# incredible-vision/show-and-tell

Measured on AMD Instinct MI355X. Metric: images/sec (train step), higher is better.
Workload: dtype bf16

## Files before the change

include/sat_hip.h:

```cpp
#ifndef SAT_HIP_H
#define SAT_HIP_H
#include <stdint.h>

#ifdef __cplusplus
extern "C" {
#endif

#define SAT_ABI_VERSION 18

#define SAT_OK 0
#define SAT_ERR_ARG 1001
#define SAT_ERR_WORKSPACE 1002
#define SAT_ERR_UNSUPPORTED 1003

#define SAT_F32 0
#define SAT_BF16 1

typedef void* sat_stream_t;

int sat_version(void);
const char* sat_error_string(int code);

int sat_gemm_f32(int amode, int bmode, const float* A, int64_t lda, const float* B, int64_t ldb,
                 float* C, int64_t ldc, const float* bias, const float* bias2,
                 int M, int N, int K, sat_stream_t stream);

enum {
    SAT_OP_IMAGE_PREP = 1,
    SAT_OP_CONV = 2,
    SAT_OP_BN_FINALIZE = 3,
    SAT_OP_BN_RELU = 4,
    SAT_OP_BN_ADD_RELU = 5,
    SAT_OP_BN_RELU_MAXPOOL = 6,
    SAT_OP_AVGPOOL = 7,
    SAT_OP_MAXPOOL3S2 = 10,
    SAT_OP_AVGPOOL3 = 11,
    SAT_OP_MAXPOOL2 = 9,
    SAT_OP_BN_EVAL_BATCH = 8,
    SAT_OP_GRAM = 12,
    SAT_OP_GRAM_COV = 13,
    SAT_OP_GEMM_BF16_NT = 14,
    SAT_OP_BN_FROM_GRAM = 15
};

typedef struct sat_bn_eval_item {
    const float* gamma;
    const float* beta;
    const float* running_mean;
    const float* running_var;
    float* scale_out;
    float* shift_out;
    int32_t C;
    int32_t reserved;
} sat_bn_eval_item;

typedef struct sat_bn_running_item {
    float* running_mean;
    float* running_var;
    const float* batch_mean;
    const float* batch_var;
    int32_t C;
    int32_t reserved;
} sat_bn_running_item;

typedef struct sat_op {
    int32_t kind;
    int32_t dtype;
    const void* in0;
    const void* in1;
    void* out;
    const void* w;
    const float* scale0;
    const float* shift0;
    const float* scale1;
    const float* shift1;
    float* stat_partial;
    const float* gamma;
    const float* beta;
    float* running_mean;
    float* running_var;
    float* scale_out;
    float* shift_out;
    int32_t N, Hin, Win, Cin, Hout, Wout, Cout, KH, KW, stride, pad;
    int32_t training;
    int32_t tiles_m;
    int64_t sN, sH, sW;
    int64_t count;
    float momentum, eps;
    int32_t variant;
    int32_t flags;
    void* stat_acc;
    void* stat_acc1;
    const float* gamma1;
    const float* beta1;
    float* running_mean1;
    float* running_var1;
    const void* w_packed;
    int32_t reserved1[2];
    int32_t pad_w;
    int32_t groups;
    int64_t ldc;
    void* out1;
} sat_op;
#define SAT_CONV_PADW 2
#define SAT_CONV_IN_RESIDUAL 8
#define SAT_CONV_GROUP_TABLE 4
int sat_gram_rows_per_slab(int64_t M, int P);
int sat_gram_slabs(int64_t M, int P);
int64_t sat_gram_slab_floats(int64_t M, int P);
int sat_run_ops(const sat_op* ops , int n_ops, sat_stream_t stream);
int sat_bn_running_apply(const sat_bn_running_item* items , int n_items, float momentum, sat_stream_t stream);
int sat_counter_add(int64_t* counters , int n, int64_t value, sat_stream_t stream);
int sat_run_ops_parity(const sat_op* ops , int n_ops, int parity, sat_stream_t stream);
typedef struct sat_graph sat_graph;
int sat_graph_create(const sat_op* ops , int n_ops, int parity, sat_graph** graph_out);
int sat_graph_launch(sat_graph* graph, sat_stream_t stream);
int sat_graph_destroy(sat_graph* graph);
int sat_conv_bn_relu_fwd(const sat_op* conv, const sat_op* finalize, const sat_op* bnrelu, sat_stream_t stream);
int sat_conv_tiles_m(int64_t M);
int sat_conv_autotune(sat_op* ops , int n_ops, int reps, float* scratch, int64_t scratch_bytes,
                      sat_stream_t stream);
int sat_conv_autotune_topk(sat_op* ops , int n_ops, int reps, float* scratch, int64_t scratch_bytes,
                           sat_stream_t stream, int topk, int32_t* cand );
int sat_conv_variant_signature(int variant);
int sat_conv_variant_family(int variant);
int sat_conv_num_variants(void);
int sat_conv_default_variant(const sat_op* op , int want_sig);
int sat_conv_resolved_variant(const sat_op* op );
int sat_conv_pack_weights(const void* w, void* packed, int Cout, int Cin, int taps, sat_stream_t stream);
int sat_run_ops_timed(const sat_op* ops , int n_ops, int parity, sat_stream_t stream, float* op_us );

int sat_fc_bn1d_fwd(const float* pooled , const float* w_fc , const float* b_fc ,
                    const float* gamma, const float* beta, float* running_mean, float* running_var,
                    float momentum, float eps, int training, int B, int F, int E,
                    float* feats , float* xhat , float* rstd ,
                    float* workspace, int64_t ws_bytes, sat_stream_t stream);
int64_t sat_fc_bn1d_ws_bytes(int B, int F, int E);
int sat_fc_bn1d_bwd(const float* dy , const float* pooled, const float* xhat, const float* rstd,
                    const float* gamma, int B, int F, int E,
                    float* dw_fc , float* db_fc, float* dgamma, float* dbeta,
                    float* workspace , int64_t ws_bytes, sat_stream_t stream);

int sat_embed_concat_fwd(const float* features , const float* embed ,
                         const int64_t* captions , int64_t cap_stride,
                         const int32_t* prefix , int T, int N , int B, int E, int V,
                         float* X , sat_stream_t stream);
int sat_embed_concat_bwd(const float* dX , const int64_t* captions, int64_t cap_stride,
                         const int32_t* prefix , int T, int N, int B, int E, int V,
                         float* d_embed , float* d_features , sat_stream_t stream);

int sat_validate_ids(const int64_t* ids, int64_t row_stride, int rows, int cols, int64_t lo, int64_t hi,
                     int32_t* status, sat_stream_t stream);

int sat_pack_targets(const int64_t* captions , int64_t cap_stride, const int32_t* prefix ,
                     int T, int N, int64_t* targets , sat_stream_t stream);

int sat_lstm_fwd(const float* X , const float* w_ih , const float* w_hh ,
                 const float* b_ih, const float* b_hh, const int32_t* batch_sizes , int T,
                 int In, int H, float* GA, float* CS, float* HS, float* HP, float* c_state,
                 void* workspace, int64_t ws_bytes, sat_stream_t stream);
int64_t sat_lstm_fwd_ws_bytes(int B, int H);
int64_t sat_lstm_fwd_status_offset(int B, int H);
int sat_lstm_persist_enable(int on);
int64_t sat_lstm_bwd_ws_bytes(int B, int H);
int64_t sat_lstm_bwd_ws_bytes_full(int N, int B, int In, int H);
int64_t sat_lstm_bwd_ws_bytes_max(int n_max, int B, int In, int H);
int sat_lstm_ws_release(void* workspace);
int64_t sat_lstm_bwd_status_offset(int N, int B, int In, int H);
int sat_lstm_bwd(const float* dHS , const float* X, const float* w_ih, const float* w_hh,
                 const float* GA, const float* CS, const float* HP,
                 const int32_t* batch_sizes , int T, int In, int H,
                 float* DG , float* dw_ih, float* dw_hh, float* db_ih, float* db_hh,
                 float* dX , float* workspace, int64_t ws_bytes, sat_stream_t stream);

int64_t sat_lstm_mixed_ws_bytes(int N , int In, int H);
int sat_lstm_fwd_bf16(const float* X, const float* w_ih, const float* w_hh, const float* b_ih, const float* b_hh,
                      const int32_t* batch_sizes , int T, int In, int H, float* GA, float* CS, float* HS, float* HP,
                      float* c_state, void* workspace, int64_t ws_bytes, void* mixed_ws, int64_t mixed_bytes, sat_stream_t stream);
int sat_lstm_bwd_bf16(const float* dHS, const float* X, const float* w_ih, const float* w_hh, const float* GA, const float* CS,
                      const float* HP, const int32_t* batch_sizes , int T, int In, int H, float* DG, float* dw_ih,
                      float* dw_hh, float* db_ih, float* db_hh, float* dX, float* workspace, int64_t ws_bytes, void* mixed_ws,
                      int64_t mixed_bytes, sat_stream_t stream);

int sat_vocab_logits_fwd(const float* Hs , const float* w , const float* b ,
                         int N, int H, int V, float* logits , int64_t ldl, sat_stream_t stream);
int sat_ce_rows(float* logits , int64_t ldl, const int64_t* targets , int N, int V, float inv_denom,
                int write_grad, float* row_loss , float* loss_out , sat_stream_t stream);
int64_t sat_vocab_bf16_ws_bytes(int N, int H, int V);
int sat_vocab_ce_fwd_bf16(const float* Hs , const float* w , const float* b , const int64_t* targets ,
                          int N, int H, int V, float inv_denom, float* logits , int64_t ldl, float* row_loss ,
                          float* loss_out , void* workspace , int64_t ws_bytes, sat_stream_t stream);
int sat_vocab_ce_bwd_bf16(int N, int H, int V, float* dw , float* db , float* dHs , void* workspace,
                          int64_t ws_bytes, sat_stream_t stream);
int sat_gemm_bf16_nt(const void* A, int64_t lda, const void* B, int64_t ldb, float* C, int64_t ldc, const float* bias,
                     int M, int N, int K, int ksplit, int64_t slab_stride, sat_stream_t stream);
int sat_transpose_f32_bf16(const float* in, int64_t ldi, int R, int C, void* out, int64_t ldo, sat_stream_t stream);
int sat_vocab_ce_fwd(const float* Hs , const float* w , const float* b , const int64_t* targets ,
                     int N, int H, int V, float inv_denom, float* logits , int64_t ldl,
                     float* row_loss , float* loss_out , sat_stream_t stream);
int sat_vocab_ce_bwd(const float* dlogits , int64_t ldl, const float* Hs, const float* w, int N, int H, int V,
                     float* dw, float* db, float* dHs, float* workspace, int64_t ws_bytes, sat_stream_t stream);
int64_t sat_vocab_ce_bwd_ws_bytes(int N, int H, int V);
int64_t sat_gemm_f32x3_packed_bytes(int N, int K);
int sat_gemm_f32x3_pack(const float* W, int N, int K, void* packed, sat_stream_t stream);
int sat_gemm_f32x3(const float* A, int64_t lda, const void* packed, const float* bias, float* C, int64_t ldc, int M, int N, int K,
                   sat_stream_t stream);

int sat_gemm_f32_splitk(int amode, int bmode, const float* A, int64_t lda, const float* B, int64_t ldb,
                        float* C, int64_t ldc, const float* bias, const float* bias2, int M, int N, int K,
                        int ksplit, int64_t slab_stride, sat_stream_t stream);
int sat_sum_slabs_f32(const float* in, int nslab, int64_t slab_stride, int64_t n, float* out, sat_stream_t stream);
int sat_skinny_gemm_f32(const float* A, int64_t lda, const float* W, int64_t ldw, int w_kmajor, int M, int N, int K,
                        const float* bias, float* out, int64_t ldo, float* workspace, int64_t ws_bytes, sat_stream_t stream);
int64_t sat_skinny_gemm_ws_bytes(int M, int N, int K);
int sat_skinny_gemm2_f32(const float* A, int64_t lda, const float* W, int64_t ldw, int K, const float* A2, int64_t lda2,
                         const float* W2, int64_t ldw2, int K2, int w_kmajor, int M, int N, const float* bias, float* out,
                         int64_t ldo, float* workspace, int64_t ws_bytes, sat_stream_t stream);
int sat_vocab_argmax(const float* h , const float* w, const float* b, int B, int H, int V,
                     int64_t* ids, int64_t ids_stride, float* workspace, int64_t ws_bytes, sat_stream_t stream);
int64_t sat_vocab_argmax_ws_bytes(int B, int V);
int sat_lstm_step(const float* x, const float* h_in, float* c, const float* w_ih, const float* w_hh,
                  const float* b_ih, const float* b_hh, int B, int In, int H, float* h_out, sat_stream_t stream);
int sat_embed_rows(const float* embed, const int64_t* ids, int64_t ids_stride, int B, int E, int V,
                   float* out, sat_stream_t stream);

int sat_attention_fwd(const float* ctx_enc, const float* feats, const float* proj, int64_t ld_proj, const float* w_att,
                      int rows, int P, int C, float* alpha, float* context, int64_t ld_ctx, float* workspace, int64_t ws_bytes,
                      sat_stream_t stream);
int64_t sat_attention_ws_bytes(int rows, int P);
int sat_attention_bwd(const float* ctx_enc, const float* feats, const float* proj, int64_t ld_proj, const float* w_att,
                      const float* alpha, const float* d_ctx, int64_t ld_dctx,
                      const float* d_ctx2 ,
                      int64_t ld_dctx2, int rows, int P, int C,
                      float* d_ctx_enc, float* d_proj, float* d_watt_part, float* d_feats ,
                      float* workspace, int64_t ws_bytes, sat_stream_t stream);
int64_t sat_attention_coverage_ws_bytes(int B, int P);
int sat_attention_coverage(const float* alpha , const int32_t* prefix , int T, int B, int P, float coef,
                           float* cov , float* grad , float* penalty , float* workspace,
                           int64_t ws_bytes, sat_stream_t stream);
int sat_attention_bwd_ex(const float* ctx_enc, const float* feats, const float* proj, int64_t ld_proj, const float* w_att,
                         const float* alpha, const float* d_ctx, int64_t ld_dctx, const float* d_ctx2, int64_t ld_dctx2,
                         const float* d_alpha_extra , int64_t ld_extra,
                         const float* d_alpha_scale , int rows, int P, int C,
                         float* d_ctx_enc, float* d_proj, float* d_watt_part, float* d_feats ,
                         float* workspace, int64_t ws_bytes, sat_stream_t stream);
int sat_lstmcell_fwd(const float* x , const float* h_in , float* c , const float* w_ih,
                     const float* w_hh, const float* b_ih, const float* b_hh, int B, int In, int H, float* h_out,
                     float* gates , float* c_tape , sat_stream_t stream);
int sat_rows_copy(const float* in, int64_t ldi, const int64_t* idx, int64_t idx_stride, int64_t nrows_in, int rows, int cols,
                  float* out, int64_t ldo, sat_stream_t stream);
int sat_rows_sum(const float* in, int64_t ld, int rows, int cols, float* out, int accumulate, sat_stream_t stream);
int sat_rows_add(const float* a, int64_t lda, const float* b, int64_t ldb, int rows, int cols, float* out, int64_t ldo,
                 sat_stream_t stream);
int sat_pack_tokens(const int64_t* captions, int64_t cap_stride, const int32_t* prefix , int T, int N, int col0,
                    int64_t* out, sat_stream_t stream);
int sat_scatter_rows_add(const float* rows , const int64_t* ids , int N, int E, int V, float* table,
                         sat_stream_t stream);
int sat_lstmcell_bwd_point(const float* dh_out , const float* dh_carry , int n_carry,
                           const float* gates , const float* c , const float* c_prev ,
                           float* dc_state , float* DG , int n, int H, sat_stream_t stream);

int sat_pad_nhwc_f32(const float* in, const float* relu_mask_of , int N, int H, int W, int C, int pad, float* out,
                     sat_stream_t stream);
int sat_maxpool2_bwd_f32(const float* x, const float* dy, int N, int Hin, int Win, int C, float* dx, sat_stream_t stream);
int sat_bcast_add_f32(const float* v, int B, int P, int C, float scale, float* out, sat_stream_t stream);

int sat_collate_captions(const int64_t* flat, const int64_t* offsets , const int32_t* order , int B, int Tmax,
                         int64_t* out , sat_stream_t stream);
int sat_gather_rows_f32(const float* in, const int32_t* order, int rows, int64_t cols, float* out, sat_stream_t stream);

int sat_image_augment_u8(const uint8_t* src, int Bsrc, int Hs, int Ws, const int32_t* params, const int32_t* order,
                         int B, int Hc, int Wc, const float mean[3] , const float std[3] ,
                         float* out, sat_stream_t stream);

int sat_beam_step(const float* logits , int64_t ldl, const float* scores_in ,
                  const int64_t* last_tokens , int64_t end_id, int B, int K, int V,
                  int32_t* parent , int64_t* token , float* scores_out ,
                  void* workspace, int64_t ws_bytes, sat_stream_t stream);
int64_t sat_beam_step_ws_bytes(int B, int K);
int sat_beam_gather_rows(const float* src, const int32_t* parent, int B, int K, int width, float* dst,
                         sat_stream_t stream);
int sat_beam_backtrack(const int32_t* parents, const int64_t* tokens, int T, int B, int K, int64_t* ids,
                       sat_stream_t stream);
int sat_beam_backtrack_rows(const int32_t* parents, const float* rows, int T, int B, int K, int cols, float* out,
                            sat_stream_t stream);
int64_t sat_beam_decode_ws_bytes(int B, int K, int E, int H, int V, int num_layers, int steps);
int sat_beam_decode(const float* features , const float* embed , const float* const* lstm_w , int num_layers,
                    const float* lin_w , const float* lin_b, int B, int K, int E, int H, int V, int steps, int64_t end_id,
                    int64_t* ids, float* scores, void* workspace, int64_t ws_bytes, sat_stream_t stream);
int sat_greedy_decode(const float* features, const float* embed, const float* const* lstm_w , int num_layers,
                      const float* lin_w, const float* lin_b, int B, int E, int H, int V, int steps, float* h, float* c, float* h_tmp,
                      float* x_tmp, int64_t* ids, int64_t ids_stride, float* workspace, int64_t ws_bytes, sat_stream_t stream);
typedef struct {
    const int64_t* suppress_ids;
    int n_suppress;
    int min_length;
    int no_repeat_ngram;
    int block_repeat;
    float length_penalty;
} sat_beam_constraints;
int sat_beam_step_ex(const float* logits , int64_t ldl, const float* scores_in ,
                     const int64_t* last_tokens , int64_t end_id, int B, int K, int V,
                     const sat_beam_constraints* c , const int32_t* parents, const int64_t* tokens, int i, int T,
                     int32_t* parent , int64_t* token , float* scores_out ,
                     void* workspace, int64_t ws_bytes, sat_stream_t stream);
int64_t sat_beam_step_ex_ws_bytes(int B, int K, int V, int T);
int sat_beam_rerank(const int64_t* ids, const float* scores, int B, int K, int T, int64_t end_id, float length_penalty,
                    int64_t* ids_out, float* scores_out, float* norm_out, int32_t* order_out, sat_stream_t stream);
int64_t sat_beam_decode_ex_ws_bytes(int B, int K, int E, int H, int V, int num_layers, int steps);
int sat_beam_decode_ex(const float* features , const float* embed , const float* const* lstm_w , int num_layers,
                       const float* lin_w , const float* lin_b, int B, int K, int E, int H, int V, int steps, int64_t end_id,
                       const sat_beam_constraints* c , int64_t* ids, float* scores, float* norm_scores,
                       int32_t* order, void* workspace, int64_t ws_bytes, sat_stream_t stream);
int sat_beam_step_groups(const float* logits , int64_t ldl, const float* scores_in ,
                         const int64_t* last_tokens , int64_t end_id, int B, int K, int V,
                         const sat_beam_constraints* c , const int32_t* parents, const int64_t* tokens, int i, int T,
                         int num_groups, float diversity_penalty, int32_t* parent , int64_t* token ,
                         float* scores_out , void* workspace, int64_t ws_bytes, sat_stream_t stream);
int64_t sat_beam_step_groups_ws_bytes(int B, int K, int V, int T);
int64_t sat_beam_decode_groups_ws_bytes(int B, int K, int E, int H, int V, int num_layers, int steps);
int sat_beam_decode_groups(const float* features , const float* embed , const float* const* lstm_w ,
                           int num_layers, const float* lin_w , const float* lin_b, int B, int K, int E, int H, int V, int steps,
                           int64_t end_id, const sat_beam_constraints* c , int num_groups, float diversity_penalty,
                           int64_t* ids, float* scores, float* norm_scores, int32_t* order, void* workspace, int64_t ws_bytes,
                           sat_stream_t stream);
int64_t sat_ss_decoder_fwd_ws_bytes(int B, int V);
int sat_vocab_sample(const float* h , const float* lin_w, const float* lin_b, int B, int H, int V, float* logits, int64_t ldl,
                     float ss_prob, uint64_t seed, int t, int rank, const int64_t* teacher, int64_t teacher_stride, int64_t* ids,
                     int64_t ids_stride, const float* embed, int E, float* x, float* workspace, int64_t ws_bytes, sat_stream_t stream);
int sat_ss_decoder_fwd(const float* features , const float* embed , const int64_t* captions, int64_t cap_stride,
                       const int32_t* batch_sizes , const int32_t* prefix , int T, int E, int V,
                       const float* const* lstm_w , int num_layers, int H, const float* lin_w, const float* lin_b,
                       float* const* tapes , float* X, float* logits, int64_t ldl, float ss_prob, uint64_t seed, int rank,
                       int64_t* used, int64_t used_stride, float* workspace, int64_t ws_bytes, sat_stream_t stream);
int sat_dropout_f32(const float* x, int64_t ldx, float* y, int64_t ldy, int rows, int cols, float p, uint64_t seed, int rank, int site,
                    sat_stream_t stream);
enum {
    SAT_SSA_WEIGHT_HH_W, SAT_SSA_WEIGHT_HH_B, SAT_SSA_WEIGHT_ATT, SAT_SSA_EMBEDDING, SAT_SSA_CELL_W_IH, SAT_SSA_CELL_W_HH,
    SAT_SSA_CELL_B_IH, SAT_SSA_CELL_B_HH, SAT_SSA_C2O_W, SAT_SSA_C2O_B, SAT_SSA_H2O_W, SAT_SSA_H2O_B, SAT_SSA_CLS_W, SAT_SSA_CLS_B,
    SAT_SSA_NUM_WEIGHTS
};
enum { SAT_SSA_PROJ, SAT_SSA_ALPHA, SAT_SSA_X, SAT_SSA_GATES, SAT_SSA_CS, SAT_SSA_HS, SAT_SSA_ZIN, SAT_SSA_Z, SAT_SSA_NUM_TAPES };
int64_t sat_ss_attend_fwd_ws_bytes(int B, int P, int C, int E, int H, int V);
int sat_ss_attend_fwd(const float* feats, const float* ctx_enc, const float* h0, const float* c0, const int64_t* captions,
                      int64_t cap_stride, const int32_t* batch_sizes , const int32_t* prefix , int T, int P,
                      int C, int E, int H, int V, const float* const* w , float* const* tapes , int64_t* toks,
                      float* logits, int64_t ldl, float ss_prob, uint64_t seed, int rank, int64_t* used, int64_t used_stride,
                      float* workspace, int64_t ws_bytes, sat_stream_t stream);
int sat_kept_tokens(const int64_t* ids, int64_t stride, int B, int T, int64_t end_id, int32_t* kept ,
                    sat_stream_t stream);
int64_t sat_sample_filtered_ws_bytes(int R, int V);
int sat_sample_filtered(const float* logits , int64_t ldl, int R, int V, float temperature, int top_k, float top_p,
                        uint64_t seed, int t, int rank, int64_t* ids, int64_t ids_stride, float* logp ,
                        int32_t* kept , void* workspace, int64_t ws_bytes, sat_stream_t stream);
int64_t sat_sample_decode_ws_bytes(int B, int E, int H, int V, int num_layers);
int sat_sample_decode(const float* features, const float* embed, const float* const* lstm_w , int num_layers,
                      const float* lin_w, const float* lin_b, int B, int E, int H, int V, int steps, float temperature, int top_k,
                      float top_p, uint64_t seed, int rank, float* h, float* c, float* h_tmp, float* x_tmp, int64_t* ids,
                      int64_t ids_stride, float* logp, int32_t* kept, float* logits_out, int64_t ldl, void* workspace,
                      int64_t ws_bytes, sat_stream_t stream);

typedef struct sat_cider_corpus {
    const uint64_t* table_keys;
    const int32_t* table_nodes;
    const int32_t* df;
    const int32_t* ref_tokens;
    const int32_t* ref_offsets;
    const int32_t* image_offsets;
    const double* ref_norm;
    int64_t capacity, n_tokens;
    int32_t n_nodes, n_refs, n_images;
    int32_t max_ref_tokens;
} sat_cider_corpus;
int sat_cider_table_insert(const uint64_t* keys, int n_keys, uint64_t* table_keys, int32_t* table_nodes, int64_t capacity,
                           int32_t* status, sat_stream_t stream);
int sat_cider_ref_stats(const sat_cider_corpus* corpus , double* ref_norm, sat_stream_t stream);
int sat_cider_score(const sat_cider_corpus* corpus , const int64_t* ids, int64_t stride, int B, int T,
                    const int32_t* kept , int64_t end_id, const int32_t* image_index , double sigma,
                    double* scores , double* mean , sat_stream_t stream);

typedef struct sat_ref_corpus {
    const int32_t* ref_tokens;
    const int32_t* ref_offsets;
    const int32_t* image_offsets;
    int64_t n_tokens;
    int32_t n_refs, n_images;
    int32_t max_ref_tokens;
    int32_t reserved;
} sat_ref_corpus;
int sat_bleu_comps(const sat_ref_corpus* corpus , const int64_t* ids, int64_t stride, int B, int T,
                   const int32_t* kept , int64_t end_id, const int32_t* image_index ,
                   int64_t* comps , double* sentence , double* mean ,
                   int64_t* totals , sat_stream_t stream);
int sat_bleu_finalize(const int64_t* totals , double* bleu , sat_stream_t stream);
int sat_rouge_l_score(const sat_ref_corpus* corpus , const int64_t* ids, int64_t stride, int B, int T,
                      const int32_t* kept , int64_t end_id, const int32_t* image_index , double beta,
                      double* scores , double* mean , sat_stream_t stream);

int64_t sat_rollout_decoder_fwd_ws_bytes(int B, int V);
int sat_rollout_decoder_fwd(const float* features , const float* embed , int B, int steps, int E, int V,
                            const float* const* lstm_w , int num_layers, int H, const float* lin_w, const float* lin_b,
                            float* const* tapes , float* X, float* logits, int64_t ldl, uint64_t seed, int rank, int64_t* ids,
                            int64_t ids_stride, float* workspace, int64_t ws_bytes, sat_stream_t stream);
int sat_scst_weights(const int64_t* ids, int64_t stride, int B, int T, int64_t end_id, const double* reward ,
                     const double* baseline , const double* denom , float* w ,
                     int32_t* len , double* m_out , sat_stream_t stream);
int sat_ce_rows_weighted(float* logits , int64_t ldl, const int64_t* ids, int64_t ids_stride, int B, int N, int V,
                         const float* w , int write_grad, float* row_loss , float* loss_out ,
                         sat_stream_t stream);
int64_t sat_rollout_attend_fwd_ws_bytes(int B, int P, int C, int E, int H, int V);
int sat_rollout_attend_fwd(const float* feats, const float* ctx_enc, const float* h0, const float* c0,
                           const int32_t* prefix , int B, int steps, int P, int C, int E, int H, int V,
                           const float* const* w , float* const* tapes , int64_t* toks, float* logits, int64_t ldl,
                           int greedy, int64_t start_id, uint64_t seed, int rank, int64_t* ids, int64_t ids_stride, int64_t* fed,
                           int64_t fed_stride, float* workspace, int64_t ws_bytes, sat_stream_t stream);

int sat_clamp_adam_step(float* p, float* g, float* m, float* v, int64_t n, float lr, float beta1,
                        float beta2, float eps, float clip, int step, sat_stream_t stream);
int sat_clamp_adam_step_guarded(float* p, float* g, float* m, float* v, int64_t n, float lr, float beta1,
                                float beta2, float eps, float clip, int step, const float* skip_if_nonzero,
                                sat_stream_t stream);
int sat_step_fault_flag(const void* const* status_words, int n_words, float* sticky, float* slot, sat_stream_t stream);

int sat_colsum_f32(const float* x, int64_t ld, int rows, int cols, float* out, sat_stream_t stream);
int sat_cast_f32_bf16(const float* in, void* out, int64_t n, sat_stream_t stream);
int sat_cast_bf16_f32(const void* in, float* out, int64_t n, sat_stream_t stream);

#ifdef __cplusplus
}
#endif
#endif
```

show-and-tell_amd/_lib.py:

```python
import ctypes as C
import os

_HERE = os.path.dirname(os.path.abspath(__file__))
LIB_PATH = os.environ.get("SAT_LIB") or os.path.join(_HERE, "libsat_hip.so")

ABI_VERSION = 18
SAT_F32, SAT_BF16 = 0, 1
OP_IMAGE_PREP, OP_CONV, OP_BN_FINALIZE, OP_BN_RELU, OP_BN_ADD_RELU, OP_BN_RELU_MAXPOOL, OP_AVGPOOL = 1, 2, 3, 4, 5, 6, 7

OP_BN_EVAL_BATCH = 8
OP_MAXPOOL2 = 9
OP_MAXPOOL3S2, OP_AVGPOOL3 = 10, 11
OP_GRAM, OP_GRAM_COV, OP_GEMM_BF16_NT, OP_BN_FROM_GRAM = 12, 13, 14, 15
CONV_PADW = 2
CONV_GROUP_TABLE = 4
CONV_IN_RESIDUAL = 8

_vp, _i, _i64, _f = C.c_void_p, C.c_int, C.c_int64, C.c_float


class SatBnEvalItem(C.Structure):
    _fields_ = [("gamma", _vp), ("beta", _vp), ("running_mean", _vp), ("running_var", _vp),
                ("scale_out", _vp), ("shift_out", _vp), ("C", C.c_int32), ("reserved", C.c_int32)]


class SatBnRunningItem(C.Structure):
    _fields_ = [("running_mean", _vp), ("running_var", _vp), ("batch_mean", _vp), ("batch_var", _vp),
                ("C", C.c_int32), ("reserved", C.c_int32)]


class SatCiderCorpus(C.Structure):
    _fields_ = [("table_keys", _vp), ("table_nodes", _vp), ("df", _vp), ("ref_tokens", _vp), ("ref_offsets", _vp),
                ("image_offsets", _vp), ("ref_norm", _vp), ("capacity", C.c_int64), ("n_tokens", C.c_int64),
                ("n_nodes", C.c_int32), ("n_refs", C.c_int32), ("n_images", C.c_int32), ("max_ref_tokens", C.c_int32)]


class SatRefCorpus(C.Structure):
    _fields_ = [("ref_tokens", _vp), ("ref_offsets", _vp), ("image_offsets", _vp), ("n_tokens", C.c_int64),
                ("n_refs", C.c_int32), ("n_images", C.c_int32), ("max_ref_tokens", C.c_int32), ("reserved", C.c_int32)]


class SatBeamConstraints(C.Structure):
    _fields_ = [("suppress_ids", _vp), ("n_suppress", C.c_int), ("min_length", C.c_int), ("no_repeat_ngram", C.c_int),
                ("block_repeat", C.c_int), ("length_penalty", C.c_float)]


class SatOp(C.Structure):
    __slots__ = ()
    _fields_ = [
        ("kind", C.c_int32), ("dtype", C.c_int32),
        ("in0", _vp), ("in1", _vp), ("out", _vp), ("w", _vp),
        ("scale0", _vp), ("shift0", _vp), ("scale1", _vp), ("shift1", _vp),
        ("stat_partial", _vp), ("gamma", _vp), ("beta", _vp),
        ("running_mean", _vp), ("running_var", _vp), ("scale_out", _vp), ("shift_out", _vp),
        ("N", C.c_int32), ("Hin", C.c_int32), ("Win", C.c_int32), ("Cin", C.c_int32),
        ("Hout", C.c_int32), ("Wout", C.c_int32), ("Cout", C.c_int32),
        ("KH", C.c_int32), ("KW", C.c_int32), ("stride", C.c_int32), ("pad", C.c_int32),
        ("training", C.c_int32), ("tiles_m", C.c_int32),
        ("sN", C.c_int64), ("sH", C.c_int64), ("sW", C.c_int64), ("count", C.c_int64),
        ("momentum", C.c_float), ("eps", C.c_float),
        ("variant", C.c_int32), ("flags", C.c_int32),
        ("stat_acc", _vp), ("stat_acc1", _vp), ("gamma1", _vp), ("beta1", _vp),
        ("running_mean1", _vp), ("running_var1", _vp), ("w_packed", _vp),
        ("reserved1", C.c_int32 * 2),
        ("pad_w", C.c_int32), ("groups", C.c_int32), ("ldc", C.c_int64), ("out1", C.c_void_p),
    ]


def op(kind, dtype, **fields):
    return SatOp(kind=kind, dtype=dtype, **{k: v.data_ptr() if hasattr(v, "data_ptr") else v for k, v in fields.items()})


SIGNATURES = {
    "sat_version": (_i, []),
    "sat_error_string": (C.c_char_p, [_i]),
    "sat_gemm_f32": (_i, [_i, _i, _vp, _i64, _vp, _i64, _vp, _i64, _vp, _vp, _i, _i, _i, _vp]),
    "sat_run_ops": (_i, [C.POINTER(SatOp), _i, _vp]),
    "sat_run_ops_parity": (_i, [C.POINTER(SatOp), _i, _i, _vp]),
    "sat_graph_create": (_i, [C.POINTER(SatOp), _i, _i, C.POINTER(_vp)]),
    "sat_graph_launch": (_i, [_vp, _vp]),
    "sat_graph_destroy": (_i, [_vp]),
    "sat_conv_bn_relu_fwd": (_i, [C.POINTER(SatOp), C.POINTER(SatOp), C.POINTER(SatOp), _vp]),
    "sat_conv_tiles_m": (_i, [_i64]),
    "sat_counter_add": (_i, [_vp, _i, _i64, _vp]),
    "sat_conv_variant_signature": (_i, [_i]),
    "sat_conv_variant_family": (_i, [_i]),
    "sat_gram_rows_per_slab": (_i, [_i64, _i]),
    "sat_gram_slabs": (_i, [_i64, _i]),
    "sat_gram_slab_floats": (_i64, [_i64, _i]),
    "sat_conv_num_variants": (_i, []),
    "sat_conv_default_variant": (_i, [C.POINTER(SatOp), _i]),
    "sat_conv_resolved_variant": (_i, [C.POINTER(SatOp)]),
    "sat_conv_pack_weights": (_i, [_vp, _vp, _i, _i, _i, _vp]),
    "sat_conv_autotune": (_i, [C.POINTER(SatOp), _i, _i, _vp, _i64, _vp]),
    "sat_conv_autotune_topk": (_i, [C.POINTER(SatOp), _i, _i, _vp, _i64, _vp, _i, C.POINTER(C.c_int32)]),
    "sat_run_ops_timed": (_i, [C.POINTER(SatOp), _i, _i, _vp, C.POINTER(C.c_float)]),
    "sat_validate_ids": (_i, [_vp, _i64, _i, _i, _i64, _i64, _vp, _vp]),
    "sat_fc_bn1d_fwd": (_i, [_vp, _vp, _vp, _vp, _vp, _vp, _vp, _f, _f, _i, _i, _i, _i, _vp, _vp, _vp, _vp, _i64, _vp]),
    "sat_fc_bn1d_ws_bytes": (_i64, [_i, _i, _i]),
    "sat_fc_bn1d_bwd": (_i, [_vp, _vp, _vp, _vp, _vp, _i, _i, _i, _vp, _vp, _vp, _vp, _vp, _i64, _vp]),
    "sat_embed_concat_fwd": (_i, [_vp, _vp, _vp, _i64, _vp, _i, _i, _i, _i, _i, _vp, _vp]),
    "sat_embed_concat_bwd": (_i, [_vp, _vp, _i64, _vp, _i, _i, _i, _i, _i, _vp, _vp, _vp]),
    "sat_pack_targets": (_i, [_vp, _i64, _vp, _i, _i, _vp, _vp]),
    "sat_lstm_fwd": (_i, [_vp, _vp, _vp, _vp, _vp, C.POINTER(C.c_int32), _i, _i, _i, _vp, _vp, _vp, _vp, _vp, _vp, _i64, _vp]),
    "sat_lstm_mixed_ws_bytes": (_i64, [_i, _i, _i]),
    "sat_lstm_fwd_bf16": (_i, [_vp, _vp, _vp, _vp, _vp, C.POINTER(C.c_int32), _i, _i, _i, _vp, _vp, _vp, _vp, _vp, _vp, _i64, _vp, _i64, _vp]),
    "sat_lstm_bwd_bf16": (_i, [_vp, _vp, _vp, _vp, _vp, _vp, _vp, C.POINTER(C.c_int32), _i, _i, _i,
                               _vp, _vp, _vp, _vp, _vp, _vp, _vp, _i64, _vp, _i64, _vp]),
    "sat_lstm_fwd_ws_bytes": (_i64, [_i, _i]),
    "sat_lstm_fwd_status_offset": (_i64, [_i, _i]),
    "sat_lstm_persist_enable": (_i, [_i]),
    "sat_lstm_bwd_ws_bytes": (_i64, [_i, _i]),
    "sat_lstm_bwd_ws_bytes_full": (_i64, [_i, _i, _i, _i]),
    "sat_lstm_bwd_status_offset": (_i64, [_i, _i, _i, _i]),
    "sat_lstm_bwd_ws_bytes_max": (_i64, [_i, _i, _i, _i]),
    "sat_lstm_ws_release": (_i, [_vp]),
    "sat_lstm_bwd": (_i, [_vp, _vp, _vp, _vp, _vp, _vp, _vp, C.POINTER(C.c_int32), _i, _i, _i,
                          _vp, _vp, _vp, _vp, _vp, _vp, _vp, _i64, _vp]),
    "sat_vocab_logits_fwd": (_i, [_vp, _vp, _vp, _i, _i, _i, _vp, _i64, _vp]),
    "sat_ce_rows": (_i, [_vp, _i64, _vp, _i, _i, _f, _i, _vp, _vp, _vp]),
    "sat_vocab_ce_fwd": (_i, [_vp, _vp, _vp, _vp, _i, _i, _i, _f, _vp, _i64, _vp, _vp, _vp]),
    "sat_vocab_bf16_ws_bytes": (_i64, [_i, _i, _i]),
    "sat_vocab_ce_fwd_bf16": (_i, [_vp, _vp, _vp, _vp, _i, _i, _i, _f, _vp, _i64, _vp, _vp, _vp, _i64, _vp]),
    "sat_vocab_ce_bwd_bf16": (_i, [_i, _i, _i, _vp, _vp, _vp, _vp, _i64, _vp]),
    "sat_gemm_bf16_nt": (_i, [_vp, _i64, _vp, _i64, _vp, _i64, _vp, _i, _i, _i, _i, _i64, _vp]),
    "sat_transpose_f32_bf16": (_i, [_vp, _i64, _i, _i, _vp, _i64, _vp]),
    "sat_vocab_ce_bwd": (_i, [_vp, _i64, _vp, _vp, _i, _i, _i, _vp, _vp, _vp, _vp, _i64, _vp]),
    "sat_vocab_ce_bwd_ws_bytes": (_i64, [_i, _i, _i]),
    "sat_gemm_f32_splitk": (_i, [_i, _i, _vp, _i64, _vp, _i64, _vp, _i64, _vp, _vp, _i, _i, _i, _i, _i64, _vp]),
    "sat_gemm_f32x3_packed_bytes": (_i64, [_i, _i]),
    "sat_gemm_f32x3_pack": (_i, [_vp, _i, _i, _vp, _vp]),
    "sat_gemm_f32x3": (_i, [_vp, _i64, _vp, _vp, _vp, _i64, _i, _i, _i, _vp]),
    "sat_sum_slabs_f32": (_i, [_vp, _i, _i64, _i64, _vp, _vp]),
    "sat_skinny_gemm_f32": (_i, [_vp, _i64, _vp, _i64, _i, _i, _i, _i, _vp, _vp, _i64, _vp, _i64, _vp]),
    "sat_skinny_gemm_ws_bytes": (_i64, [_i, _i, _i]),
    "sat_skinny_gemm2_f32": (_i, [_vp, _i64, _vp, _i64, _i, _vp, _i64, _vp, _i64, _i, _i, _i, _i, _vp, _vp, _i64, _vp, _i64, _vp]),
    "sat_vocab_argmax": (_i, [_vp, _vp, _vp, _i, _i, _i, _vp, _i64, _vp, _i64, _vp]),
    "sat_vocab_argmax_ws_bytes": (_i64, [_i, _i]),
    "sat_lstm_step": (_i, [_vp, _vp, _vp, _vp, _vp, _vp, _vp, _i, _i, _i, _vp, _vp]),
    "sat_embed_rows": (_i, [_vp, _vp, _i64, _i, _i, _i, _vp, _vp]),
    "sat_attention_fwd": (_i, [_vp, _vp, _vp, _i64, _vp, _i, _i, _i, _vp, _vp, _i64, _vp, _i64, _vp]),
    "sat_attention_bwd": (_i, [_vp, _vp, _vp, _i64, _vp, _vp, _vp, _i64, _vp, _i64, _i, _i, _i, _vp, _vp, _vp, _vp, _vp, _i64, _vp]),
    "sat_attention_ws_bytes": (_i64, [_i, _i]),
    "sat_attention_coverage_ws_bytes": (_i64, [_i, _i]),
    "sat_attention_coverage": (_i, [_vp, _vp, _i, _i, _i, _f, _vp, _vp, _vp, _vp, _i64, _vp]),
    "sat_attention_bwd_ex": (_i, [_vp, _vp, _vp, _i64, _vp, _vp, _vp, _i64, _vp, _i64, _vp, _i64, _vp, _i, _i, _i, _vp, _vp, _vp, _vp,
                                  _vp, _i64, _vp]),
    "sat_bn_running_apply": (_i, [_vp, _i, _f, _vp]),
    "sat_pad_nhwc_f32": (_i, [_vp, _vp, _i, _i, _i, _i, _i, _vp, _vp]),
    "sat_maxpool2_bwd_f32": (_i, [_vp, _vp, _i, _i, _i, _i, _vp, _vp]),
    "sat_bcast_add_f32": (_i, [_vp, _i, _i, _i, _f, _vp, _vp]),
    "sat_lstmcell_fwd": (_i, [_vp, _vp, _vp, _vp, _vp, _vp, _vp, _i, _i, _i, _vp, _vp, _vp, _vp]),
    "sat_rows_copy": (_i, [_vp, _i64, _vp, _i64, _i64, _i, _i, _vp, _i64, _vp]),
    "sat_rows_sum": (_i, [_vp, _i64, _i, _i, _vp, _i, _vp]),
    "sat_rows_add": (_i, [_vp, _i64, _vp, _i64, _i, _i, _vp, _i64, _vp]),
    "sat_pack_tokens": (_i, [_vp, _i64, _vp, _i, _i, _i, _vp, _vp]),
    "sat_scatter_rows_add": (_i, [_vp, _vp, _i, _i, _i, _vp, _vp]),
    "sat_lstmcell_bwd_point": (_i, [_vp, _vp, _i, _vp, _vp, _vp, _vp, _vp, _i, _i, _vp]),
    "sat_collate_captions": (_i, [_vp, _vp, _vp, _i, _i, _vp, _vp]),
    "sat_gather_rows_f32": (_i, [_vp, _vp, _i, _i64, _vp, _vp]),
    "sat_image_augment_u8": (_i, [_vp, _i, _i, _i, _vp, _vp, _i, _i, _i, C.POINTER(_f), C.POINTER(_f), _vp, _vp]),
    "sat_beam_step": (_i, [_vp, _i64, _vp, _vp, _i64, _i, _i, _i, _vp, _vp, _vp, _vp, _i64, _vp]),
    "sat_beam_step_ws_bytes": (_i64, [_i, _i]),
    "sat_beam_gather_rows": (_i, [_vp, _vp, _i, _i, _i, _vp, _vp]),
    "sat_beam_backtrack": (_i, [_vp, _vp, _i, _i, _i, _vp, _vp]),
    "sat_beam_backtrack_rows": (_i, [_vp, _vp, _i, _i, _i, _i, _vp, _vp]),
    "sat_kept_tokens": (_i, [_vp, _i64, _i, _i, _i64, _vp, _vp]),
    "sat_beam_decode_ws_bytes": (_i64, [_i, _i, _i, _i, _i, _i, _i]),
    "sat_beam_decode": (_i, [_vp, _vp, C.POINTER(_vp), _i, _vp, _vp, _i, _i, _i, _i, _i, _i, _i64, _vp, _vp, _vp, _i64, _vp]),
    "sat_beam_step_ex": (_i, [_vp, _i64, _vp, _vp, _i64, _i, _i, _i, C.POINTER(SatBeamConstraints), _vp, _vp, _i, _i, _vp, _vp, _vp, _vp,
                              _i64, _vp]),
    "sat_beam_step_ex_ws_bytes": (_i64, [_i, _i, _i, _i]),
    "sat_beam_rerank": (_i, [_vp, _vp, _i, _i, _i, _i64, _f, _vp, _vp, _vp, _vp, _vp]),
    "sat_beam_decode_ex_ws_bytes": (_i64, [_i, _i, _i, _i, _i, _i, _i]),
    "sat_beam_decode_ex": (_i, [_vp, _vp, C.POINTER(_vp), _i, _vp, _vp, _i, _i, _i, _i, _i, _i, _i64, C.POINTER(SatBeamConstraints),
                                _vp, _vp, _vp, _vp, _vp, _i64, _vp]),
    "sat_beam_step_groups": (_i, [_vp, _i64, _vp, _vp, _i64, _i, _i, _i, C.POINTER(SatBeamConstraints), _vp, _vp, _i, _i, _i, _f, _vp, _vp,
                                  _vp, _vp, _i64, _vp]),
    "sat_beam_step_groups_ws_bytes": (_i64, [_i, _i, _i, _i]),
    "sat_beam_decode_groups_ws_bytes": (_i64, [_i, _i, _i, _i, _i, _i, _i]),
    "sat_beam_decode_groups": (_i, [_vp, _vp, C.POINTER(_vp), _i, _vp, _vp, _i, _i, _i, _i, _i, _i, _i64, C.POINTER(SatBeamConstraints),
                                    _i, _f, _vp, _vp, _vp, _vp, _vp, _i64, _vp]),
    "sat_greedy_decode": (_i, [_vp, _vp, C.POINTER(_vp), _i, _vp, _vp, _i, _i, _i, _i, _i, _vp, _vp, _vp, _vp, _vp, _i64, _vp, _i64, _vp]),
    "sat_ss_decoder_fwd_ws_bytes": (_i64, [_i, _i]),
    "sat_vocab_sample": (_i, [_vp, _vp, _vp, _i, _i, _i, _vp, _i64, _f, C.c_uint64, _i, _i, _vp, _i64, _vp, _i64, _vp, _i, _vp,
                              _vp, _i64, _vp]),
    "sat_ss_decoder_fwd": (_i, [_vp, _vp, _vp, _i64, C.POINTER(C.c_int32), _vp, _i, _i, _i, C.POINTER(_vp), _i, _i, _vp, _vp,
                                C.POINTER(_vp), _vp, _vp, _i64, _f, C.c_uint64, _i, _vp, _i64, _vp, _i64, _vp]),
    "sat_ss_attend_fwd_ws_bytes": (_i64, [_i, _i, _i, _i, _i, _i]),
    "sat_ss_attend_fwd": (_i, [_vp, _vp, _vp, _vp, _vp, _i64, C.POINTER(C.c_int32), _vp, _i, _i, _i, _i, _i, _i, C.POINTER(_vp),
                               C.POINTER(_vp), _vp, _vp, _i64, _f, C.c_uint64, _i, _vp, _i64, _vp, _i64, _vp]),
    "sat_cider_table_insert": (_i, [_vp, _i, _vp, _vp, _i64, _vp, _vp]),
    "sat_cider_ref_stats": (_i, [C.POINTER(SatCiderCorpus), _vp, _vp]),
    "sat_cider_score": (_i, [C.POINTER(SatCiderCorpus), _vp, _i64, _i, _i, _vp, _i64, _vp, C.c_double, _vp, _vp, _vp]),
    "sat_bleu_comps": (_i, [C.POINTER(SatRefCorpus), _vp, _i64, _i, _i, _vp, _i64, _vp, _vp, _vp, _vp, _vp, _vp]),
    "sat_bleu_finalize": (_i, [_vp, _vp, _vp]),
    "sat_rouge_l_score": (_i, [C.POINTER(SatRefCorpus), _vp, _i64, _i, _i, _vp, _i64, _vp, C.c_double, _vp, _vp, _vp]),
    "sat_rollout_decoder_fwd_ws_bytes": (_i64, [_i, _i]),
    "sat_rollout_decoder_fwd": (_i, [_vp, _vp, _i, _i, _i, _i, C.POINTER(_vp), _i, _i, _vp, _vp, C.POINTER(_vp), _vp, _vp, _i64,
                                     C.c_uint64, _i, _vp, _i64, _vp, _i64, _vp]),
    "sat_scst_weights": (_i, [_vp, _i64, _i, _i, _i64, _vp, _vp, _vp, _vp, _vp, _vp, _vp]),
    "sat_ce_rows_weighted": (_i, [_vp, _i64, _vp, _i64, _i, _i, _i, _vp, _i, _vp, _vp, _vp]),
    "sat_rollout_attend_fwd_ws_bytes": (_i64, [_i, _i, _i, _i, _i, _i]),
    "sat_rollout_attend_fwd": (_i, [_vp, _vp, _vp, _vp, _vp, _i, _i, _i, _i, _i, _i, _i, C.POINTER(_vp), C.POINTER(_vp), _vp, _vp, _i64,
                                    _i, _i64, C.c_uint64, _i, _vp, _i64, _vp, _i64, _vp, _i64, _vp]),
    "sat_sample_filtered_ws_bytes": (_i64, [_i, _i]),
    "sat_sample_filtered": (_i, [_vp, _i64, _i, _i, _f, _i, _f, C.c_uint64, _i, _i, _vp, _i64, _vp, _vp, _vp, _i64, _vp]),
    "sat_sample_decode_ws_bytes": (_i64, [_i, _i, _i, _i, _i]),
    "sat_sample_decode": (_i, [_vp, _vp, C.POINTER(_vp), _i, _vp, _vp, _i, _i, _i, _i, _i, _f, _i, _f, C.c_uint64, _i, _vp, _vp, _vp,
                               _vp, _vp, _i64, _vp, _vp, _vp, _i64, _vp, _i64, _vp]),
    "sat_dropout_f32": (_i, [_vp, _i64, _vp, _i64, _i, _i, _f, C.c_uint64, _i, _i, _vp]),
    "sat_clamp_adam_step": (_i, [_vp, _vp, _vp, _vp, _i64, _f, _f, _f, _f, _f, _i, _vp]),
    "sat_clamp_adam_step_guarded": (_i, [_vp, _vp, _vp, _vp, _i64, _f, _f, _f, _f, _f, _i, _vp, _vp]),
    "sat_step_fault_flag": (_i, [C.POINTER(_vp), _i, _vp, _vp, _vp]),
    "sat_colsum_f32": (_i, [_vp, _i64, _i, _i, _vp, _vp]),
    "sat_cast_f32_bf16": (_i, [_vp, _vp, _i64, _vp]),
    "sat_cast_bf16_f32": (_i, [_vp, _vp, _i64, _vp]),
}

ADDED_WITHIN_ABI = ("sat_conv_resolved_variant", "sat_image_augment_u8", "sat_attention_coverage_ws_bytes", "sat_attention_coverage",
                    "sat_attention_bwd_ex", "sat_beam_backtrack_rows", "sat_cider_table_insert", "sat_cider_ref_stats", "sat_cider_score",
                    "sat_rollout_decoder_fwd_ws_bytes", "sat_rollout_decoder_fwd", "sat_scst_weights", "sat_ce_rows_weighted",
                    "sat_rollout_attend_fwd_ws_bytes", "sat_rollout_attend_fwd", "sat_bleu_comps", "sat_bleu_finalize",
                    "sat_rouge_l_score", "sat_sample_filtered_ws_bytes", "sat_sample_filtered", "sat_sample_decode_ws_bytes",
                    "sat_sample_decode", "sat_dropout_f32", "sat_beam_step_ex", "sat_beam_step_ex_ws_bytes", "sat_beam_rerank",
                    "sat_beam_decode_ex_ws_bytes", "sat_beam_decode_ex", "sat_beam_step_groups", "sat_beam_step_groups_ws_bytes",
                    "sat_beam_decode_groups_ws_bytes", "sat_beam_decode_groups")

_lib = None


def open_library(path):
    if not os.path.exists(path):
        raise RuntimeError(
            "show-and-tell_amd: %s is missing -- build it with `python -c 'import __graft_entry__ as g; g.build()'` "
            "(hipcc --offload-arch=gfx950).  There is no CPU fallback." % path)
    lib = C.CDLL(path)
    for name, (res, args) in SIGNATURES.items():
        if name in ADDED_WITHIN_ABI and not hasattr(lib, name):
            continue
        fn = getattr(lib, name)
        fn.restype = res
        fn.argtypes = args
    if lib.sat_version() != ABI_VERSION:
        raise RuntimeError("%s: ABI version mismatch" % path)
    return lib


def load():
    global _lib
    if _lib is None:
        _lib = open_library(LIB_PATH)
    return _lib


def check(rc, what=""):
    if rc != 0:
        msg = load().sat_error_string(rc)
        raise RuntimeError("libsat_hip %s failed: [%d] %s" % (what, rc, msg.decode() if msg else "?"))


def ptr(t):
    return t if t is None or isinstance(t, int) else t.data_ptr()


def rows(t, row0=0):
    return t.data_ptr() + row0 * t.shape[1] * 4


def stream():
    import torch
    return torch.cuda.current_stream().cuda_stream


def pad4(n):
    return (n + 3) // 4 * 4


def logits_buffer(N, V, device):
    import torch
    return torch.zeros(N, pad4(V), device=device) if V % 4 else torch.empty(N, V, device=device)


def pad_rows4(d):
    import torch
    V = d.shape[1]
    if V % 4 == 0:
        return d.contiguous()
    out = torch.zeros(d.shape[0], pad4(V), device=d.device)
    out[:, :V] = d
    return out


def workspace256(nbytes, device):
    import torch
    ws = torch.empty(nbytes + 256, dtype=torch.uint8, device=device)
    return ws, ws.data_ptr() + (-ws.data_ptr()) % 256


def require_gpu(t, name="tensor"):
    if not t.is_cuda:
        raise RuntimeError("show-and-tell_amd: %s must live on the MI355X (got a %s tensor); the HIP path has no CPU fallback"
                           % (name, t.device))


def counter_add(t, value=1):
    check(load().sat_counter_add(t.data_ptr(), t.numel(), value, stream()), "sat_counter_add")


_SKINNY_WS = {}
_SKINNY_ROWS = int(os.environ.get("SAT_SKINNY_ROWS", "128"))


def gemm(lib, amode, bmode, A, lda, B, ldb, Cout, ldc, M, N, K, bias=None, bias2=None):
    if amode == 0 and M <= _SKINNY_ROWS and bias2 is None and ldc == N and K % 4 == 0 and lda % 4 == 0 and (bmode == 1 or ldb % 4 == 0):
        import torch
        need = lib.sat_skinny_gemm_ws_bytes(M, N, K)
        dev = torch.cuda.current_device()
        ws = _SKINNY_WS.get(dev)
        if ws is None or ws.numel() * 4 < need:
            ws = _SKINNY_WS[dev] = torch.empty(max(need // 4, 1 << 20), dtype=torch.float32, device="cuda")
        check(lib.sat_skinny_gemm_f32(ptr(A), lda, ptr(B), ldb, bmode, M, N, K, ptr(bias), ptr(Cout), ldc,
                                      ws.data_ptr(), ws.numel() * 4, stream()), "sat_skinny_gemm_f32")
        return
    check(lib.sat_gemm_f32(amode, bmode, ptr(A), lda, ptr(B), ldb, ptr(Cout), ldc, ptr(bias), ptr(bias2), M, N, K, stream()),
          "sat_gemm_f32")
```

show-and-tell_amd/csrc/sat_elementwise.hip:

```cpp
#include "sat_bn_stats.h"
#include <stdlib.h>

namespace {

constexpr int EW_BLOCK = 256;
inline int ew_grid(long n_items) {
    long cap;
    cap = 768;
    long b = (n_items + EW_BLOCK - 1) / EW_BLOCK;
    return (int)(b < 1 ? 1 : (b > cap ? cap : b));
}

template <typename T> struct Vec;
template <> struct Vec<float> { static constexpr int N = 4; };
template <> struct Vec<bf16_t> { static constexpr int N = 8; };

template <typename T> __device__ __forceinline__ void load_chunk(const T* p, float (&v)[Vec<T>::N]);
template <> __device__ __forceinline__ void load_chunk<float>(const float* p, float (&v)[4]) {
    const f32x4 x = *(const f32x4*)p;
    v[0] = x[0]; v[1] = x[1]; v[2] = x[2]; v[3] = x[3];
}
template <> __device__ __forceinline__ void load_chunk<bf16_t>(const bf16_t* p, float (&v)[8]) {
    const bf16x8 x = *(const bf16x8*)p;
#pragma unroll
// ... 445 lines not shown
    __syncthreads();
    const int v = tok[row];
    if (v < 0) {
        for (int e = threadIdx.x; e < E; e += blockDim.x) d_features[(long)row * E + e] = dX[(long)row * E + e];
        return;
    }
    int dup = 0;
    for (int i = threadIdx.x; i < row; i += blockDim.x) dup |= (tok[i] == v);
    if (__syncthreads_or(dup)) return;
    __shared__ unsigned match_bits[1280];
    const int nwords = (Nrows + 31) >> 5;
    const bool fits = nwords <= 1280;
    int any = 0;
    if (fits) {
        for (int w = threadIdx.x; w < nwords; w += blockDim.x) {
            unsigned bits = 0u;
            const int base = w << 5;
            for (int b = 0; b < 32; ++b) {
                const int i = base + b;
                if (i > row && i < Nrows && tok[i] == v) bits |= 1u << b;
            }
            match_bits[w] = bits;
            any |= (bits != 0u);
        }
    }
    any = __syncthreads_or(any);
    for (int e = threadIdx.x; e < E; e += blockDim.x) {
        float acc = dX[(long)row * E + e];
        if (!fits) {
            for (int i = row + 1; i < Nrows; ++i)
                if (tok[i] == v) acc += dX[(long)i * E + e];
        } else if (any) {
            for (int w = row >> 5; w < nwords; ++w) {
                unsigned bits = match_bits[w];
                while (bits) {
                    const int b = __ffs(bits) - 1;
                    bits &= bits - 1;
                    acc += dX[(long)((w << 5) + b) * E + e];
                }
            }
        }
        d_embed[(long)v * E + e] = acc;
    }
}

__device__ __forceinline__ float block_reduce(float v, bool is_max, float* sh) {
    v = is_max ? wave_max(v) : wave_sum(v);
    const int w = threadIdx.x >> 6;
    __syncthreads();
    if ((threadIdx.x & 63) == 0) sh[w] = v;
    __syncthreads();
    float r = sh[0];
    for (int i = 1; i < (int)(blockDim.x >> 6); ++i) r = is_max ? fmaxf(r, sh[i]) : r + sh[i];
    return r;
}

template <bool WEIGHTED>
__global__ __launch_bounds__(256) void ce_rows_kernel(float* __restrict__ logits, long ldl, const int64_t* __restrict__ targets,
                                                      int V, float inv_denom, int write_grad, float* __restrict__ row_loss,
                                                      const float* __restrict__ w, long tstride, int B) {
    __shared__ float sh[4];
    const int row = blockIdx.x;
    float* x = logits + (long)row * ldl;
    if constexpr (WEIGHTED) inv_denom = w[row];
    const long tpos = WEIGHTED ? (long)(row % B) * tstride + row / B : (long)row;
    constexpr int RC = 12;
    const int nq = V >> 2;
    if ((ldl & 3) == 0 && nq <= RC * 256 && (((uintptr_t)logits) & 15) == 0) {
        const int tid = threadIdx.x;
        f32x4 rc[RC];
#pragma unroll
        for (int c = 0; c < RC; ++c)
            if (tid + c * 256 < nq) rc[c] = *(const f32x4*)(x + 4 * (tid + c * 256));
        const int tail = (nq << 2) + tid;
        const float xt = tail < V ? x[tail] : -INFINITY;
        float m = xt;
#pragma unroll
        for (int c = 0; c < RC; ++c)
            if (tid + c * 256 < nq) m = fmaxf(fmaxf(fmaxf(m, rc[c][0]), fmaxf(rc[c][1], rc[c][2])), rc[c][3]);
        m = block_reduce(m, true, sh);
        float s = 0.0f;
#pragma unroll
        for (int c = 0; c < RC; ++c)
            if (tid + c * 256 < nq) {
#pragma unroll
                for (int e = 0; e < 4; ++e) s += expf(rc[c][e] - m);
            }
        if (tail < V) s += expf(xt - m);
        s = block_reduce(s, false, sh);
        const float lse = m + logf(s);
        long tgt = targets[tpos];
        tgt = tgt < 0 ? 0 : (tgt >= V ? V - 1 : tgt);
        const int tq = (int)(tgt >> 2), te = (int)(tgt & 3);
#pragma unroll
        for (int c = 0; c < RC; ++c)
            if (tid + c * 256 == tq && tq < nq) row_loss[row] = lse - rc[c][te];
        if (tail == (int)tgt && tq >= nq) row_loss[row] = lse - xt;
        if (write_grad) {
#pragma unroll
            for (int c = 0; c < RC; ++c) {
                const int q = tid + c * 256;
                if (q < nq) {
                    f32x4 g;
#pragma unroll
                    for (int e = 0; e < 4; ++e)
                        g[e] = (expf(rc[c][e] - lse) - ((4 * q + e) == (int)tgt ? 1.0f : 0.0f)) * inv_denom;
                    if (WEIGHTED && inv_denom == 0.0f) g = (f32x4){0.0f, 0.0f, 0.0f, 0.0f};
                    *(f32x4*)(x + 4 * q) = g;
                }
            }
            if (tail < V) x[tail] = (WEIGHTED && inv_denom == 0.0f) ? 0.0f : (expf(xt - lse) - (tail == (int)tgt ? 1.0f : 0.0f)) * inv_denom;
        }
        return;
    }
    float m = -INFINITY;
    for (int i = threadIdx.x; i < V; i += 256) m = fmaxf(m, x[i]);
    m = block_reduce(m, true, sh);
    float s = 0.0f;
    for (int i = threadIdx.x; i < V; i += 256) s += expf(x[i] - m);
    s = block_reduce(s, false, sh);
    const float lse = m + logf(s);
    long tgt = targets[tpos];
    tgt = tgt < 0 ? 0 : (tgt >= V ? V - 1 : tgt);
    if (threadIdx.x == 0) row_loss[row] = lse - x[tgt];
    if (write_grad) {
        __syncthreads();
        for (int i = threadIdx.x; i < V; i += 256) {
            const float pr = expf(x[i] - lse);
            x[i] = (WEIGHTED && inv_denom == 0.0f) ? 0.0f : (pr - (i == (int)tgt ? 1.0f : 0.0f)) * inv_denom;
        }
    }
}

__global__ __launch_bounds__(256) void weighted_sum_kernel(const float* __restrict__ v, const float* __restrict__ w, int n, float* out) {
    __shared__ float sh[256];
    float s = 0.0f;
    for (int i = threadIdx.x; i < n; i += 256) {
        const float wi = w[i];
        if (wi != 0.0f) s += wi * v[i];
    }
    sh[threadIdx.x] = s;
    __syncthreads();
    for (int k = 128; k > 0; k >>= 1) {
        if ((int)threadIdx.x < k) sh[threadIdx.x] += sh[threadIdx.x + k];
        __syncthreads();
    }
    if (threadIdx.x == 0) out[0] = sh[0];
}

__global__ __launch_bounds__(256) void scst_weights_kernel(const int64_t* __restrict__ ids, long stride, int B, int T, int64_t end_id,
                                                           const double* __restrict__ reward, const double* __restrict__ baseline,
                                                           const double* __restrict__ denom, float* __restrict__ w,
                                                           int32_t* __restrict__ len, double* __restrict__ m_out) {
    __shared__ long long sh[256];
    const int tid = threadIdx.x;
    long long tot = 0;
    for (int b = tid; b < B; b += 256) {
        const int64_t* row = ids + (long)b * stride;
        int n = 0;
        while (n < T && row[n] != end_id) ++n;
        n = n + 1 < T ? n + 1 : T;
        len[b] = n;
        tot += n;
    }
    sh[tid] = tot;
    __syncthreads();
    for (int k = 128; k > 0; k >>= 1) {
        if (tid < k) sh[tid] += sh[tid + k];
        __syncthreads();
    }
    const double M = denom ? *denom : (double)sh[0];
    if (tid == 0) m_out[0] = M;
    for (int b = tid; b < B; b += 256) {
        const float wb = (float)((reward[b] - (baseline ? baseline[b] : 0.0)) / M);
        const int n = len[b];
        for (int t = 0; t < T; ++t) w[(long)t * B + b] = t < n ? wb : 0.0f;
    }
}

__global__ __launch_bounds__(256) void sum_scale_kernel(const float* __restrict__ v, int n, float scale, float* out) {
    __shared__ float sh[256];
    float s = 0.0f;
    for (int i = threadIdx.x; i < n; i += 256) s += v[i];
    sh[threadIdx.x] = s;
    __syncthreads();
    for (int k = 128; k > 0; k >>= 1) {
        if ((int)threadIdx.x < k) sh[threadIdx.x] += sh[threadIdx.x + k];
        __syncthreads();
    }
    if (threadIdx.x == 0) out[0] = sh[0] * scale;
}

__global__ __launch_bounds__(256) void colsum_kernel(const float* __restrict__ x, long ld, int rows, int cols,
                                                     float* __restrict__ out) {
    __shared__ float sh[8][32];
    const int cl = threadIdx.x & 31, rg = threadIdx.x >> 5;
    const int c = blockIdx.x * 32 + cl;
    float s = 0.0f;
    if (c < cols) {
        int r = rg;
        for (; r + 24 < rows; r += 32) {
            const float a0 = x[(long)r * ld + c], a1 = x[(long)(r + 8) * ld + c];
            const float a2 = x[(long)(r + 16) * ld + c], a3 = x[(long)(r + 24) * ld + c];
            s += a0; s += a1; s += a2; s += a3;
        }
        for (; r < rows; r += 8) s += x[(long)r * ld + c];
    }
    sh[rg][cl] = s;
    __syncthreads();
    if (rg == 0 && c < cols) {
        float t = 0.0f;
#pragma unroll
        for (int g = 0; g < 8; ++g) t += sh[g][cl];
        out[c] = t;
    }
}

__global__ void clamp_adam_kernel(float* __restrict__ p, float* __restrict__ g, float* __restrict__ m,
                                  float* __restrict__ v, long n, float beta1, float beta2, float eps, float clip,
                                  float step_size, float bc2_sqrt, const float* __restrict__ skip) {
    if (skip && *skip != 0.0f) return;
    const float w1 = 1.0f - beta1, w2 = 1.0f - beta2;
    const long n4 = n >> 2;
    for (long i = (long)blockIdx.x * blockDim.x + threadIdx.x; i < n4; i += (long)gridDim.x * blockDim.x) {
        f32x4 pp = ((f32x4*)p)[i], gg = ((f32x4*)g)[i], mm = ((f32x4*)m)[i], vv = ((f32x4*)v)[i];
#pragma unroll
        for (int k = 0; k < 4; ++k) {
            float gk = gg[k];
            if (clip > 0.0f) gk = fminf(fmaxf(gk, -clip), clip);
            gg[k] = gk;
            mm[k] = mm[k] + w1 * (gk - mm[k]);
            vv[k] = vv[k] * beta2 + (w2 * gk) * gk;
            const float denom = sqrtf(vv[k]) / bc2_sqrt + eps;
            pp[k] = pp[k] + (-step_size * mm[k]) / denom;
        }
        ((f32x4*)p)[i] = pp; ((f32x4*)g)[i] = gg; ((f32x4*)m)[i] = mm; ((f32x4*)v)[i] = vv;
    }
    const long base = n4 << 2;
    const long i = base + (long)blockIdx.x * blockDim.x + threadIdx.x;
    if (i < n) {
        float gk = g[i];
        if (clip > 0.0f) gk = fminf(fmaxf(gk, -clip), clip);
        g[i] = gk;
        const float mk = m[i] + w1 * (gk - m[i]);
        const float vk = v[i] * beta2 + (w2 * gk) * gk;
        m[i] = mk; v[i] = vk;
        p[i] = p[i] + (-step_size * mk) / (sqrtf(vk) / bc2_sqrt + eps);
    }
}

__global__ void cast_f32_bf16_kernel(const float* __restrict__ in, bf16_t* __restrict__ out, long n) {
    for (long i = (long)blockIdx.x * blockDim.x + threadIdx.x; i < n; i += (long)gridDim.x * blockDim.x)
        out[i] = (bf16_t)in[i];
}
__global__ void cast_bf16_f32_kernel(const bf16_t* __restrict__ in, float* __restrict__ out, long n) {
    for (long i = (long)blockIdx.x * blockDim.x + threadIdx.x; i < n; i += (long)gridDim.x * blockDim.x)
        out[i] = (float)in[i];
}

__global__ void lstm_bwd_point_kernel(const float* __restrict__ dHS, const float* __restrict__ dh_part, int nz,
                                      long slab_stride, int n_next, const float* __restrict__ GA,
                                      const float* __restrict__ CS, const float* __restrict__ CS_prev,
                                      float* __restrict__ dc_state, float* __restrict__ DG, int n, int H) {
    const long total = (long)n * H;
    for (long i = (long)blockIdx.x * blockDim.x + threadIdx.x; i < total; i += (long)gridDim.x * blockDim.x) {
        const int j = (int)(i % H);
        const int b = (int)(i / H);
        float dh = dHS[i];
        float dcn = 0.0f;
        if (b < n_next) {
            for (int z = 0; z < nz; ++z) dh += dh_part[(long)z * slab_stride + i];
            dcn = dc_state[i];
        }
        const float* ga = GA + (long)b * 4 * H;
        const float gi = ga[j], gf = ga[H + j], gg = ga[2 * H + j], go = ga[3 * H + j];
        const float tc = sat_tanh(CS[i]);
        const float c_prev = CS_prev ? CS_prev[i] : 0.0f;
        const float d_o = dh * tc;
        const float dc = dh * go * (1.0f - tc * tc) + dcn;
        float* dg = DG + (long)b * 4 * H;
        dg[j] = dc * gg * gi * (1.0f - gi);
        dg[H + j] = dc * c_prev * gf * (1.0f - gf);
        dg[2 * H + j] = dc * gi * (1.0f - gg * gg);
        dg[3 * H + j] = d_o * go * (1.0f - go);
        dc_state[i] = dc * gf;
    }
}

__global__ __launch_bounds__(256) void bn1d_fwd_kernel(const float* __restrict__ part, int nz, long slab_stride,
                                                       const float* __restrict__ b_fc, const float* __restrict__ gamma,
                                                       const float* __restrict__ beta, float* running_mean,
                                                       float* running_var, float momentum, float eps, int training,
                                                       int B, int E, float* __restrict__ zbuf, float* __restrict__ feats,
                                                       float* __restrict__ xhat, float* __restrict__ rstd_out) {
    __shared__ float sh[8][32];
    __shared__ float bc[2][32];
    const int cl = threadIdx.x & 31, rg = threadIdx.x >> 5;
    const int e = blockIdx.x * 32 + cl;
    const bool ok = e < E;
    float s = 0.0f;
    if (ok)
        for (int b = rg; b < B; b += 8) {
            float z = b_fc[e];
            for (int k = 0; k < nz; ++k) z += part[(long)k * slab_stride + (long)b * E + e];
            zbuf[(long)b * E + e] = z;
            s += z;
        }
    sh[rg][cl] = s;
    __syncthreads();
    if (rg == 0) {
        float t = 0.0f;
        for (int g = 0; g < 8; ++g) t += sh[g][cl];
        bc[0][cl] = t / (float)B;
    }
    __syncthreads();
    float mean = bc[0][cl];
    float q = 0.0f;
    if (ok)
        for (int b = rg; b < B; b += 8) {
            const float d = zbuf[(long)b * E + e] - mean;
            q += d * d;
        }
    __syncthreads();
    sh[rg][cl] = q;
    __syncthreads();
    if (rg == 0 && ok) {
        float t = 0.0f;
        for (int g = 0; g < 8; ++g) t += sh[g][cl];
        float var = t / (float)B;
        if (training) {
            const float unb = B > 1 ? t / (float)(B - 1) : var;
            running_mean[e] = (1.0f - momentum) * running_mean[e] + momentum * mean;
            running_var[e] = (1.0f - momentum) * running_var[e] + momentum * unb;
        } else {
            mean = running_mean[e];
            var = running_var[e];
        }
        const float rs = 1.0f / sqrtf(var + eps);
        bc[0][cl] = mean;
        bc[1][cl] = rs;
        rstd_out[e] = rs;
    }
    __syncthreads();
    if (ok) {
        const float mu = bc[0][cl], rs = bc[1][cl], ga = gamma[e], be = beta[e];
        for (int b = rg; b < B; b += 8) {
            const float xh = (zbuf[(long)b * E + e] - mu) * rs;
            xhat[(long)b * E + e] = xh;
            feats[(long)b * E + e] = xh * ga + be;
        }
    }
}

__global__ __launch_bounds__(256) void bn1d_bwd_kernel(const float* __restrict__ dy, const float* __restrict__ xhat,
                                                       const float* __restrict__ rstd, const float* __restrict__ gamma,
                                                       int B, int E, float* __restrict__ dz, float* __restrict__ dgamma,
                                                       float* __restrict__ dbeta, float* __restrict__ db_fc) {
    __shared__ float s1[8][32], s2[8][32];
    __shared__ float bc[2][32];
    const int cl = threadIdx.x & 31, rg = threadIdx.x >> 5;
    const int e = blockIdx.x * 32 + cl;
    const bool ok = e < E;
    float a = 0.0f, c = 0.0f;
    if (ok)
        for (int b = rg; b < B; b += 8) {
            const float d = dy[(long)b * E + e];
            a += d * xhat[(long)b * E + e];
            c += d;
        }
    s1[rg][cl] = a; s2[rg][cl] = c;
    __syncthreads();
    if (rg == 0) {
        float ta = 0.0f, tc = 0.0f;
        for (int g = 0; g < 8; ++g) { ta += s1[g][cl]; tc += s2[g][cl]; }
        bc[0][cl] = ta; bc[1][cl] = tc;
        if (ok) { dgamma[e] = ta; dbeta[e] = tc; }
    }
    __syncthreads();
    float zs = 0.0f;
    if (ok) {
        const float dga = bc[0][cl], dbe = bc[1][cl];
        const float k = gamma[e] * rstd[e] / (float)B;
        for (int b = rg; b < B; b += 8) {
            const float v = k * ((float)B * dy[(long)b * E + e] - dbe - xhat[(long)b * E + e] * dga);
            dz[(long)b * E + e] = v;
            zs += v;
        }
    }
    __syncthreads();
    s1[rg][cl] = zs;
    __syncthreads();
    if (rg == 0 && ok) {
        float t = 0.0f;
        for (int g = 0; g < 8; ++g) t += s1[g][cl];
        db_fc[e] = t;
    }
}

}

int sat_image_prep_launch(const sat_op* op, hipStream_t s) {
    if (!op->in0 || !op->out) return SAT_ERR_ARG;
    const long total = (long)op->N * op->Hin * op->Win;
    if (op->Cout != 0 && op->Cout != 4 && !(op->Cout == 8 && op->dtype == SAT_BF16)) return SAT_ERR_ARG;
    if (op->dtype == SAT_BF16 && op->Cout == 8)
        hipLaunchKernelGGL((image_prep_kernel<bf16_t, 8>), dim3(ew_grid(total)), dim3(EW_BLOCK), 0, s, (const float*)op->in0,
                           (bf16_t*)op->out, op->N, op->Hin, op->Win, op->Hout, op->Wout, op->pad);
    else if (op->dtype == SAT_BF16)
        hipLaunchKernelGGL(image_prep_kernel<bf16_t>, dim3(ew_grid(total)), dim3(EW_BLOCK), 0, s, (const float*)op->in0,
                           (bf16_t*)op->out, op->N, op->Hin, op->Win, op->Hout, op->Wout, op->pad);
    else
        hipLaunchKernelGGL(image_prep_kernel<float>, dim3(ew_grid(total)), dim3(EW_BLOCK), 0, s, (const float*)op->in0,
                           (float*)op->out, op->N, op->Hin, op->Win, op->Hout, op->Wout, op->pad);
    SAT_LAUNCH_CHECK();
    return SAT_OK;
}

extern "C" int sat_bn_running_apply(const sat_bn_running_item* items, int n_items, float momentum, sat_stream_t stream) {
    if (!items || n_items < 0 || !(momentum >= 0.0f && momentum <= 1.0f)) return SAT_ERR_ARG;
    if (n_items == 0) return SAT_OK;
    hipLaunchKernelGGL(bn_running_apply_kernel, dim3(n_items), dim3(256), 0, (hipStream_t)stream, items, momentum);
    SAT_LAUNCH_CHECK();
    return SAT_OK;
}

__global__ void counter_add_kernel(long long* p, int n, long long v) {
    const int i = blockIdx.x * blockDim.x + threadIdx.x;
    if (i < n) p[i] += v;
}
extern "C" int sat_counter_add(int64_t* counters, int n, int64_t value, sat_stream_t stream) {
    if (!counters || n < 0) return SAT_ERR_ARG;
    if (n == 0) return SAT_OK;
    hipLaunchKernelGGL(counter_add_kernel, dim3((n + 255) / 256), dim3(256), 0, (hipStream_t)stream, (long long*)counters, n, (long long)value);
    SAT_LAUNCH_CHECK();
    return SAT_OK;
}

int sat_bn_eval_batch_launch(const sat_op* op, hipStream_t s) {
    if (!op->in0 || op->count < 1 || op->count > 65535) return SAT_ERR_ARG;
    hipLaunchKernelGGL(bn_eval_batch_kernel, dim3((int)op->count), dim3(256), 0, s, (const sat_bn_eval_item*)op->in0, op->eps);
    SAT_LAUNCH_CHECK();
    return SAT_OK;
}

int sat_bn_finalize_launch(const sat_op* op, int parity, hipStream_t s) {
    if (op->stat_acc) {
        if (!op->stat_partial || op->tiles_m < 1 || op->Cout < 1) return SAT_ERR_ARG;
        long long* acc = (long long*)op->stat_acc + (long)parity * 2 * op->Cout;
        const int groups = op->groups > 1 ? op->groups : 1;
        hipLaunchKernelGGL(bn_slab_to_acc_kernel, dim3(sat_cdiv(op->Cout, 32), sat_cdiv(op->tiles_m, SLAB_TILES_PER_WG), groups),
                           dim3(1024), 0, s, op->stat_partial, op->tiles_m, op->Cout, acc);
        SAT_LAUNCH_CHECK();
        return SAT_OK;
    }
    if (op->groups > 1) return SAT_ERR_UNSUPPORTED;
    if (!op->gamma || !op->beta || !op->scale_out || !op->shift_out) return SAT_ERR_ARG;
    if (op->training && !op->stat_partial) return SAT_ERR_ARG;
    if (!op->training && (!op->running_mean || !op->running_var)) return SAT_ERR_ARG;
    hipLaunchKernelGGL(bn_finalize_kernel, dim3(sat_cdiv(op->Cout, 32)), dim3(1024), 0, s, op->stat_partial, op->tiles_m,
                       op->Cout, (double)op->count, op->gamma, op->beta, op->running_mean, op->running_var,
                       op->momentum, op->eps, op->training, op->scale_out, op->shift_out);
    SAT_LAUNCH_CHECK();
    return SAT_OK;
}

template <typename T>
static int bn_act_launch_t(const sat_op* op, bool add, int parity, hipStream_t s) {
    constexpr int V = Vec<T>::N;
    const int C = op->Cout;
    if (C % V) return SAT_ERR_ARG;
    const long n = (long)op->N * op->Hout * op->Wout * C;
    const long nch = n / V;
    BnSrc b0 = {}, b1 = {};
    b0.scale = op->scale0; b0.shift = op->shift0;
    b1.scale = op->scale1; b1.shift = op->shift1;
    int has_b1 = 0;
    size_t lds = 0;
    if (op->stat_acc) {
        if (!op->gamma || !op->beta || op->count < 1) return SAT_ERR_ARG;
        long long* base = (long long*)op->stat_acc;
        b0.acc = base + (long)parity * 2 * C;
        b0.acc_clear = base + (long)(1 - parity) * 2 * C;
        b0.gamma = op->gamma; b0.beta = op->beta; b0.running_mean = op->running_mean; b0.running_var = op->running_var;
        lds = (size_t)4 * C * sizeof(float);
    } else if (!op->scale0 || !op->shift0) {
        return SAT_ERR_ARG;
    }
    if (add) {
        if (op->stat_acc1) {
            if (!op->gamma1 || !op->beta1 || op->count < 1) return SAT_ERR_ARG;
            long long* base = (long long*)op->stat_acc1;
            b1.acc = base + (long)parity * 2 * C;
            b1.acc_clear = base + (long)(1 - parity) * 2 * C;
            b1.gamma = op->gamma1; b1.beta = op->beta1; b1.running_mean = op->running_mean1; b1.running_var = op->running_var1;
            lds = (size_t)4 * C * sizeof(float);
            has_b1 = 1;
        } else if (op->scale1) {
            if (!op->shift1) return SAT_ERR_ARG;
            has_b1 = 1;
        }
    }
    if (lds > 64 * 1024) return SAT_ERR_UNSUPPORTED;
    const int cch = C / V;
    int grid = ew_grid(nch);
    if (lds && grid > 2048) grid = 2048;
    if (op->groups > 1 && grid >= 2 * op->groups) grid /= op->groups;
    if (cch > EW_BLOCK && (cch % EW_BLOCK) == 0) {
        const int g0 = cch / EW_BLOCK;
        grid = grid / g0 * g0;
        if (grid < g0) grid = g0;
    }
    constexpr int kBnBlock = 512;
    int block = EW_BLOCK;
    if (lds && (kBnBlock % cch) == 0 && grid >= kBnBlock / EW_BLOCK) {
        block = kBnBlock;
        grid = grid / (kBnBlock / EW_BLOCK);
    }
    const int groups = op->groups > 1 ? op->groups : 1;
    if (groups > 1 && !op->stat_acc) return SAT_ERR_UNSUPPORTED;
    if (groups > 1 && ((b0.running_mean && b0.running_var != b0.running_mean + C) ||
                       (b1.running_mean && b1.running_var != b1.running_mean + C))) return SAT_ERR_ARG;
    const double count = (double)op->count;
    if (add)
        hipLaunchKernelGGL((bn_act_kernel<T, true, true>), dim3(grid, groups), dim3(block), lds, s, (const T*)op->in0, (const T*)op->in1,
                           (T*)op->out, b0, b1, has_b1, count, op->momentum, op->eps, nch, C);
    else
        hipLaunchKernelGGL((bn_act_kernel<T, false>), dim3(grid, groups), dim3(block), lds, s, (const T*)op->in0, (const T*)nullptr,
                           (T*)op->out, b0, b1, 0, count, op->momentum, op->eps, nch, C);
    SAT_LAUNCH_CHECK();
    return SAT_OK;
}

template <typename T>
static int bn_relu_strided_launch_t(const sat_op* op, int parity, hipStream_t s) {
    constexpr int V = Vec<T>::N;
    const int C = op->Cout;
    if ((C % V) || (op->ldc % V) || op->ldc < C) return SAT_ERR_ARG;
    BnSrc b = {};
    b.scale = op->scale0; b.shift = op->shift0;
    size_t lds = 0;
    if (op->stat_acc) {
        if (!op->gamma || !op->beta || op->count < 1) return SAT_ERR_ARG;
        long long* base = (long long*)op->stat_acc;
        b.acc = base + (long)parity * 2 * C;
        b.acc_clear = base + (long)(1 - parity) * 2 * C;
        b.gamma = op->gamma; b.beta = op->beta; b.running_mean = op->running_mean; b.running_var = op->running_var;
        lds = (size_t)2 * C * sizeof(float);
    } else if (!op->scale0 || !op->shift0) {
        return SAT_ERR_ARG;
    }
    const long npix = (long)op->N * op->Hout * op->Wout;
    int grid = ew_grid(npix * (C / V));
    if (lds && grid > 2048) grid = 2048;
    const int groups = op->groups > 1 ? op->groups : 1;
    if (groups > 1 && (!op->stat_acc || (b.running_mean && b.running_var != b.running_mean + C))) return SAT_ERR_ARG;
    hipLaunchKernelGGL(bn_relu_strided_kernel<T>, dim3(grid, groups), dim3(EW_BLOCK), lds, s, (const T*)op->in0, (T*)op->out, (long)op->ldc, b,
                       (double)op->count, op->momentum, op->eps, npix, C);
    SAT_LAUNCH_CHECK();
    return SAT_OK;
}

int sat_bn_act_launch(const sat_op* op, bool add, int parity, hipStream_t s) {
    if (!op->in0 || !op->out || (add && !op->in1)) return SAT_ERR_ARG;
    if (!add && op->ldc && op->ldc != op->Cout)
        return op->dtype == SAT_BF16 ? bn_relu_strided_launch_t<bf16_t>(op, parity, s) : bn_relu_strided_launch_t<float>(op, parity, s);
    return op->dtype == SAT_BF16 ? bn_act_launch_t<bf16_t>(op, add, parity, s) : bn_act_launch_t<float>(op, add, parity, s);
}

int sat_bn_relu_maxpool_launch(const sat_op* op, int parity, hipStream_t s) {
    if (!op->in0 || !op->out) return SAT_ERR_ARG;
    const int C = op->Cout;
    BnSrc b = {};
    b.scale = op->scale0; b.shift = op->shift0;
    size_t lds = 0;
    if (op->stat_acc) {
        if (!op->gamma || !op->beta || op->count < 1) return SAT_ERR_ARG;
        long long* base = (long long*)op->stat_acc;
        b.acc = base + (long)parity * 2 * C;
        b.acc_clear = base + (long)(1 - parity) * 2 * C;
        b.gamma = op->gamma; b.beta = op->beta; b.running_mean = op->running_mean; b.running_var = op->running_var;
        lds = (size_t)2 * C * sizeof(float);
        if (lds > 64 * 1024) return SAT_ERR_UNSUPPORTED;
    } else if (!op->scale0 || !op->shift0) {
        return SAT_ERR_ARG;
    }
    const double count = (double)op->count;
    const int groups = op->groups > 1 ? op->groups : 1;
    if (groups > 1 && (!op->stat_acc || (b.running_mean && b.running_var != b.running_mean + C))) return SAT_ERR_ARG;
    if (op->dtype == SAT_BF16) {
        if (C % 8) return SAT_ERR_ARG;
        const long total = (long)op->N * op->Hout * op->Wout * (C / 8);
        if (total >= (1L << 31)) return SAT_ERR_UNSUPPORTED;
        hipLaunchKernelGGL(bn_relu_maxpool_kernel<bf16_t>, dim3(ew_grid(total), groups), dim3(EW_BLOCK), lds, s, (const bf16_t*)op->in0,
                           (bf16_t*)op->out, b, count, op->momentum, op->eps, op->N, op->Hin, op->Win, C, op->Hout, op->Wout);
    } else {
        if (C % 4) return SAT_ERR_ARG;
        const long total = (long)op->N * op->Hout * op->Wout * (C / 4);
        if (total >= (1L << 31)) return SAT_ERR_UNSUPPORTED;
        if (groups > 1) return SAT_ERR_UNSUPPORTED;
        hipLaunchKernelGGL(bn_relu_maxpool_kernel<float>, dim3(ew_grid(total)), dim3(EW_BLOCK), lds, s, (const float*)op->in0,
                           (float*)op->out, b, count, op->momentum, op->eps, op->N, op->Hin, op->Win, C, op->Hout, op->Wout);
    }
    SAT_LAUNCH_CHECK();
    return SAT_OK;
}

int sat_avgpool_launch(const sat_op* op, hipStream_t s) {
    if (!op->in0 || !op->out) return SAT_ERR_ARG;
    const int C = op->Cout, HW = op->Hin * op->Win;
    if (op->dtype == SAT_BF16) {
        if (C % 8) return SAT_ERR_ARG;
        hipLaunchKernelGGL(avgpool_kernel<bf16_t>, dim3(ew_grid((long)op->N * C / 8)), dim3(EW_BLOCK), 0, s,
                           (const bf16_t*)op->in0, (float*)op->out, op->N, HW, C);
    } else {
        if (C % 4) return SAT_ERR_ARG;
        hipLaunchKernelGGL(avgpool_kernel<float>, dim3(ew_grid((long)op->N * C / 4)), dim3(EW_BLOCK), 0, s,
                           (const float*)op->in0, (float*)op->out, op->N, HW, C);
    }
    SAT_LAUNCH_CHECK();
    return SAT_OK;
}

int sat_lstm_bwd_point_launch(const float* dHS, const float* dh_part, int nz, long slab_stride, int n_next,
                              const float* GA, const float* CS, const float* CS_prev, float* dc_state, float* DG,
                              int n, int H, hipStream_t s) {
    hipLaunchKernelGGL(lstm_bwd_point_kernel, dim3(ew_grid((long)n * H)), dim3(EW_BLOCK), 0, s, dHS, dh_part, nz,
                       slab_stride, n_next, GA, CS, CS_prev, dc_state, DG, n, H);
    SAT_LAUNCH_CHECK();
    return SAT_OK;
}

int sat_bn1d_fwd_launch(const float* part, int nz, long slab_stride, const float* b_fc, const float* gamma,
                        const float* beta, float* rm, float* rv, float momentum, float eps, int training, int B, int E,
                        float* zbuf, float* feats, float* xhat, float* rstd, hipStream_t s) {
    hipLaunchKernelGGL(bn1d_fwd_kernel, dim3(sat_cdiv(E, 32)), dim3(256), 0, s, part, nz, slab_stride, b_fc, gamma, beta,
                       rm, rv, momentum, eps, training, B, E, zbuf, feats, xhat, rstd);
    SAT_LAUNCH_CHECK();
    return SAT_OK;
}

__global__ __launch_bounds__(256) void outer_wgrad_kernel(const float* __restrict__ dz, const float* __restrict__ x, int B, int E, int F,
                                                          float* __restrict__ dw) {
    const long i = (long)blockIdx.x * 256 + threadIdx.x;
    const int f4 = F >> 2;
    if (i >= (long)E * f4) return;
    const int e = (int)(i / f4), f = (int)(i - (long)e * f4) * 4;
    f32x4 acc = {0.f, 0.f, 0.f, 0.f};
    for (int b = 0; b < B; ++b) {
        const float d = dz[(long)b * E + e];
        const f32x4 v = *(const f32x4*)(x + (long)b * F + f);
#pragma unroll
        for (int k = 0; k < 4; ++k) acc[k] = fmaf(d, v[k], acc[k]);
    }
    *(f32x4*)(dw + (long)e * F + f) = acc;
}

int sat_outer_wgrad_launch(const float* dz, const float* x, int B, int E, int F, float* dw, hipStream_t s) {
    const long n = (long)E * (F >> 2);
    hipLaunchKernelGGL(outer_wgrad_kernel, dim3((unsigned)((n + 255) / 256)), dim3(256), 0, s, dz, x, B, E, F, dw);
    SAT_LAUNCH_CHECK();
    return SAT_OK;
}

int sat_bn1d_bwd_launch(const float* dy, const float* xhat, const float* rstd, const float* gamma, int B, int E,
                        float* dz, float* dgamma, float* dbeta, float* db_fc, hipStream_t s) {
    hipLaunchKernelGGL(bn1d_bwd_kernel, dim3(sat_cdiv(E, 32)), dim3(256), 0, s, dy, xhat, rstd, gamma, B, E, dz, dgamma,
                       dbeta, db_fc);
    SAT_LAUNCH_CHECK();
    return SAT_OK;
}

extern "C" int sat_embed_concat_fwd(const float* features, const float* embed, const int64_t* captions,
                                    int64_t cap_stride, const int32_t* prefix, int T, int N, int B, int E, int V,
                                    float* X, sat_stream_t stream) {
    if (!features || !embed || !prefix || !X || T < 1 || B < 1 || N < B) return SAT_ERR_ARG;
    if (T > 1 && !captions) return SAT_ERR_ARG;
    hipLaunchKernelGGL(embed_concat_fwd_kernel, dim3(N), dim3(256), 0, (hipStream_t)stream, features, embed, captions,
                       (long)cap_stride, prefix, T, E, V, X);
    SAT_LAUNCH_CHECK();
    return SAT_OK;
}

extern "C" int sat_embed_concat_bwd(const float* dX, const int64_t* captions, int64_t cap_stride,
                                    const int32_t* prefix, int T, int N, int B, int E, int V, float* d_embed,
                                    float* d_features, sat_stream_t stream) {
    if (!dX || !prefix || !d_embed || !d_features || T < 1 || B < 1 || N < B) return SAT_ERR_ARG;
    if (T > 1 && !captions) return SAT_ERR_ARG;
    const size_t dyn = (size_t)N * 4;
    if (dyn > 150 * 1024) return SAT_ERR_UNSUPPORTED;
    if (dyn > 48 * 1024) {
        hipError_t ea = hipFuncSetAttribute((const void*)embed_concat_bwd_kernel, hipFuncAttributeMaxDynamicSharedMemorySize, (int)dyn);
        if (ea != hipSuccess) return (int)ea;
    }
    hipStream_t s = (hipStream_t)stream;
    hipError_t e = hipMemsetAsync(d_embed, 0, (size_t)V * E * sizeof(float), s);
    if (e != hipSuccess) return (int)e;
    hipLaunchKernelGGL(embed_concat_bwd_kernel, dim3(N), dim3(256), (size_t)N * 4, s, dX, captions, (long)cap_stride,
                       prefix, T, B, E, V, N, d_embed, d_features);
    SAT_LAUNCH_CHECK();
    return SAT_OK;
}

extern "C" int sat_embed_rows(const float* embed, const int64_t* ids, int64_t ids_stride, int B, int E, int V,
                              float* out, sat_stream_t stream) {
    if (!embed || !ids || !out) return SAT_ERR_ARG;
    hipLaunchKernelGGL(embed_rows_kernel, dim3(B), dim3(256), 0, (hipStream_t)stream, embed, ids, (long)ids_stride, E, V, out);
    SAT_LAUNCH_CHECK();
    return SAT_OK;
}

extern "C" int sat_ce_rows(float* logits, int64_t ldl, const int64_t* targets, int N, int V, float inv_denom,
                           int write_grad, float* row_loss, float* loss_out, sat_stream_t stream) {
    if (!logits || !targets || !row_loss || N < 1 || V < 1 || ldl < V) return SAT_ERR_ARG;
    hipStream_t s = (hipStream_t)stream;
    hipLaunchKernelGGL(ce_rows_kernel<false>, dim3(N), dim3(256), 0, s, logits, (long)ldl, targets, V, inv_denom, write_grad, row_loss,
                       (const float*)nullptr, 0L, 1);
    SAT_LAUNCH_CHECK();
    if (loss_out) {
        hipLaunchKernelGGL(sum_scale_kernel, dim3(1), dim3(256), 0, s, row_loss, N, inv_denom, loss_out);
        SAT_LAUNCH_CHECK();
    }
    return SAT_OK;
}

extern "C" int sat_ce_rows_weighted(float* logits, int64_t ldl, const int64_t* ids, int64_t ids_stride, int B, int N, int V,
                                    const float* w, int write_grad, float* row_loss, float* loss_out, sat_stream_t stream) {
    if (!logits || !ids || !w || !row_loss || B < 1 || N < 1 || N % B || V < 1 || ldl < V || ids_stride < N / B) return SAT_ERR_ARG;
    hipStream_t s = (hipStream_t)stream;
    hipLaunchKernelGGL(ce_rows_kernel<true>, dim3(N), dim3(256), 0, s, logits, (long)ldl, ids, V, 0.0f, write_grad, row_loss, w,
                       (long)ids_stride, B);
    SAT_LAUNCH_CHECK();
    if (loss_out) {
        hipLaunchKernelGGL(weighted_sum_kernel, dim3(1), dim3(256), 0, s, row_loss, w, N, loss_out);
        SAT_LAUNCH_CHECK();
    }
    return SAT_OK;
}

extern "C" int sat_scst_weights(const int64_t* ids, int64_t stride, int B, int T, int64_t end_id, const double* reward,
                                const double* baseline, const double* denom, float* w, int32_t* len, double* m_out,
                                sat_stream_t stream) {
    if (!ids || !reward || !w || !len || !m_out || B < 1 || T < 1 || stride < T || (long)B * T > 0x7fffffffL) return SAT_ERR_ARG;
    hipLaunchKernelGGL(scst_weights_kernel, dim3(1), dim3(256), 0, (hipStream_t)stream, ids, (long)stride, B, T, end_id, reward,
                       baseline, denom, w, len, m_out);
    SAT_LAUNCH_CHECK();
    return SAT_OK;
}

extern "C" int sat_colsum_f32(const float* x, int64_t ld, int rows, int cols, float* out, sat_stream_t stream) {
    if (!x || !out || rows < 1 || cols < 1) return SAT_ERR_ARG;
    hipLaunchKernelGGL(colsum_kernel, dim3(sat_cdiv(cols, 32)), dim3(256), 0, (hipStream_t)stream, x, (long)ld, rows, cols, out);
    SAT_LAUNCH_CHECK();
    return SAT_OK;
}

struct FaultWords { const unsigned* w[8]; int n; };
__global__ void step_fault_flag_kernel(const FaultWords fw, float* __restrict__ sticky, float* __restrict__ slot) {
    if (threadIdx.x != 0 || blockIdx.x != 0) return;
    float f = sticky ? *sticky : 0.0f;
    for (int i = 0; i < fw.n; ++i)
        if (__hip_atomic_load(fw.w[i], __ATOMIC_RELAXED, __HIP_MEMORY_SCOPE_AGENT) != 0u) f = 1.0f;
    if (sticky) *sticky = f;
    *slot = f;
}

extern "C" int sat_step_fault_flag(const void* const* status_words, int n_words, float* sticky, float* slot, sat_stream_t stream) {
    if (!slot || n_words < 0 || n_words > 8 || (n_words > 0 && !status_words)) return SAT_ERR_ARG;
    FaultWords fw = {};
    fw.n = n_words;
    for (int i = 0; i < n_words; ++i) {
        if (!status_words[i]) return SAT_ERR_ARG;
        fw.w[i] = (const unsigned*)status_words[i];
    }
    hipLaunchKernelGGL(step_fault_flag_kernel, dim3(1), dim3(64), 0, (hipStream_t)stream, fw, sticky, slot);
    SAT_LAUNCH_CHECK();
    return SAT_OK;
}

extern "C" int sat_clamp_adam_step(float* p, float* g, float* m, float* v, int64_t n, float lr, float beta1,
                                   float beta2, float eps, float clip, int step, sat_stream_t stream) {
    return sat_clamp_adam_step_guarded(p, g, m, v, n, lr, beta1, beta2, eps, clip, step, nullptr, stream);
}

extern "C" int sat_clamp_adam_step_guarded(float* p, float* g, float* m, float* v, int64_t n, float lr, float beta1,
                                           float beta2, float eps, float clip, int step, const float* skip_if_nonzero,
                                           sat_stream_t stream) {
    if (!p || !g || !m || !v || n < 1 || step < 1) return SAT_ERR_ARG;
    if ((((uintptr_t)p | (uintptr_t)g | (uintptr_t)m | (uintptr_t)v) & 15) != 0) return SAT_ERR_ARG;
    const double bc1 = 1.0 - pow((double)beta1, (double)step);
    const double bc2 = 1.0 - pow((double)beta2, (double)step);
    const float step_size = (float)((double)lr / bc1);
    const float bc2_sqrt = (float)sqrt(bc2);
    hipLaunchKernelGGL(clamp_adam_kernel, dim3(ew_grid(n / 4 + 1)), dim3(EW_BLOCK), 0, (hipStream_t)stream, p, g, m, v,
                       (long)n, beta1, beta2, eps, clip, step_size, bc2_sqrt, skip_if_nonzero);
    SAT_LAUNCH_CHECK();
    return SAT_OK;
}

extern "C" int sat_cast_f32_bf16(const float* in, void* out, int64_t n, sat_stream_t stream) {
    if (!in || !out || n < 1) return SAT_ERR_ARG;
    hipLaunchKernelGGL(cast_f32_bf16_kernel, dim3(ew_grid(n)), dim3(EW_BLOCK), 0, (hipStream_t)stream, in, (bf16_t*)out, (long)n);
    SAT_LAUNCH_CHECK();
    return SAT_OK;
}
extern "C" int sat_cast_bf16_f32(const void* in, float* out, int64_t n, sat_stream_t stream) {
    if (!in || !out || n < 1) return SAT_ERR_ARG;
    hipLaunchKernelGGL(cast_bf16_f32_kernel, dim3(ew_grid(n)), dim3(EW_BLOCK), 0, (hipStream_t)stream, (const bf16_t*)in, out, (long)n);
    SAT_LAUNCH_CHECK();
    return SAT_OK;
}

namespace {
__global__ __launch_bounds__(256) void validate_ids_kernel(const int64_t* __restrict__ ids, long row_stride, int rows, int cols,
                                                           long lo, long hi, int* __restrict__ status) {
    const long total = (long)rows * cols;
    int bad = 0;
    for (long i = (long)blockIdx.x * blockDim.x + threadIdx.x; i < total; i += (long)gridDim.x * blockDim.x) {
        const long r = i / cols, c = i - r * cols;
        const long v = ids[r * row_stride + c];
        bad |= (v < lo || v >= hi) ? 1 : 0;
    }
    if (__syncthreads_or(bad) && threadIdx.x == 0) atomicOr(status, 1);
}
}

extern "C" int sat_validate_ids(const int64_t* ids, int64_t row_stride, int rows, int cols, int64_t lo, int64_t hi,
                                int32_t* status, sat_stream_t stream) {
    if (!ids || !status || rows < 0 || cols < 0 || row_stride < cols) return SAT_ERR_ARG;
    if (rows == 0 || cols == 0) return SAT_OK;
    const long total = (long)rows * cols;
    const int grid = (int)(total < 256L * 1024 ? (total + 255) / 256 : 1024);
    hipLaunchKernelGGL(validate_ids_kernel, dim3(grid), dim3(256), 0, (hipStream_t)stream, ids, (long)row_stride, rows, cols,
                       (long)lo, (long)hi, (int*)status);
    SAT_LAUNCH_CHECK();
    return SAT_OK;
}

namespace {
__global__ void pack_targets_kernel(const int64_t* __restrict__ captions, long cap_stride, const int* __restrict__ prefix,
                                    int T, int N, int64_t* __restrict__ out) {
    const int row = blockIdx.x * blockDim.x + threadIdx.x;
    if (row >= N) return;
    const int t = find_step(prefix, T, row);
    out[row] = captions[(long)(row - prefix[t]) * cap_stride + t + 1];
}
}

extern "C" int sat_pack_targets(const int64_t* captions, int64_t cap_stride, const int32_t* prefix, int T, int N,
                                int64_t* targets, sat_stream_t stream) {
    if (!captions || !prefix || !targets || T < 1 || N < 1) return SAT_ERR_ARG;
    hipLaunchKernelGGL(pack_targets_kernel, dim3(sat_cdiv(N, 256)), dim3(256), 0, (hipStream_t)stream, captions,
                       (long)cap_stride, prefix, T, N, targets);
    SAT_LAUNCH_CHECK();
    return SAT_OK;
}

namespace {
__global__ void sum_slabs_kernel(const float* __restrict__ in, int nslab, long slab_stride, long n4, float* __restrict__ out) {
    for (long i = (long)blockIdx.x * blockDim.x + threadIdx.x; i < n4; i += (long)gridDim.x * blockDim.x) {
        f32x4 acc = ((const f32x4*)in)[i];
        for (int z = 1; z < nslab; ++z) acc += ((const f32x4*)(in + (long)z * slab_stride))[i];
        ((f32x4*)out)[i] = acc;
    }
}
}

extern "C" int sat_sum_slabs_f32(const float* in, int nslab, int64_t slab_stride, int64_t n, float* out, sat_stream_t stream) {
    if (!in || !out || nslab < 1 || n < 1 || (n & 3) || (slab_stride & 3)) return SAT_ERR_ARG;
    hipLaunchKernelGGL(sum_slabs_kernel, dim3(ew_grid(n / 4)), dim3(EW_BLOCK), 0, (hipStream_t)stream, in, nslab,
                       (long)slab_stride, (long)(n / 4), out);
    SAT_LAUNCH_CHECK();
    return SAT_OK;
}
```

show-and-tell_amd/csrc/sat_gemm_bf16.hip:

```cpp
#include "sat_internal.h"

namespace {

__device__ u32x4 g_zero16_b;

typedef const __attribute__((address_space(1))) void* gptr_t;
typedef __attribute__((address_space(3))) void* lptr_t;

struct GemmArgs {
    const bf16_t* A;
    const bf16_t* B;
    float* C;
    const float* bias;
    const float* bias2;
    int M, N, K;
    long lda, ldb, ldc, slab;
    int tiles_n, ksteps;
};

template <int N> __device__ __forceinline__ void wait_vm() {
    static_assert(N == 0 || N == 4 || N == 6 || N == 8 || N == 12, "add the vmcnt literal");
    if constexpr (N == 0) asm volatile("s_waitcnt vmcnt(0)" ::: "memory");
    if constexpr (N == 4) asm volatile("s_waitcnt vmcnt(4)" ::: "memory");
    if constexpr (N == 6) asm volatile("s_waitcnt vmcnt(6)" ::: "memory");
    if constexpr (N == 8) asm volatile("s_waitcnt vmcnt(8)" ::: "memory");
    if constexpr (N == 12) asm volatile("s_waitcnt vmcnt(12)" ::: "memory");
}

template <int BN, int S>
__global__ __launch_bounds__(512) void gemm_bf16_nt_kernel(const GemmArgs p) {
    constexpr int BM = 128, NT = 512;
    constexpr int A_BYTES = BM * 128, B_BYTES = BN * 128, STAGE = A_BYTES + B_BYTES;
    constexpr int WGM = 2, WGN = 4, WM = BM / WGM, WN = BN / WGN, TM = WM / 32, TN = WN / 32;
    constexpr int NAI = BM / 64, NBI = BN / 64, LPW = NAI + NBI;
    constexpr int D = S - 1;
    constexpr int CROWF = BN + 4;
    static_assert(64 * CROWF * 4 <= S * STAGE, "half of the f32 output tile must fit the ring");
    __shared__ __attribute__((aligned(16))) char smem[S * STAGE];

    const int tid = threadIdx.x, lane = tid & 63;
    const int wave = __builtin_amdgcn_readfirstlane(tid >> 6);
    const int wm = wave / WGN, wn = wave % WGN;
    const int r = lane & 31, h = lane >> 5;

    const int nwg = gridDim.x, bid = blockIdx.x, z = blockIdx.y;
    const int q8 = nwg >> 3, r8 = nwg & 7, xcd = bid & 7;
    const int swz = (xcd < r8 ? xcd * (q8 + 1) : r8 * (q8 + 1) + (xcd - r8) * q8) + (bid >> 3);
    const int tile_m = swz / p.tiles_n, tile_n = swz - tile_m * p.tiles_n;
    const int m0 = tile_m * BM, n0 = tile_n * BN;
    const int k_begin = z * p.ksteps * 64;
    int nk = (p.K - k_begin) / 64;
    if (nk > p.ksteps) nk = p.ksteps;
    if (nk < 0) nk = 0;

    const bf16_t* zero = (const bf16_t*)&g_zero16_b;
    const bf16_t* a_ptr[NAI];
    const bf16_t* b_ptr[NBI];
    int a_step[NAI], b_step[NBI];
#pragma unroll
    for (int i = 0; i < NAI; ++i) {
        const int row = wave * (NAI * 8) + i * 8 + (lane >> 3);
        const int c = ((lane & 7) ^ ((row >> 1) & 7)) * 8;
        const bool ok = m0 + row < p.M;
        a_ptr[i] = ok ? p.A + ((long)(m0 + row) * p.lda + k_begin + c) : zero;
        a_step[i] = ok ? 64 : 0;
    }
#pragma unroll
    for (int i = 0; i < NBI; ++i) {
        const int row = wave * (NBI * 8) + i * 8 + (lane >> 3);
        const int c = ((lane & 7) ^ ((row >> 1) & 7)) * 8;
        const bool ok = n0 + row < p.N;
        b_ptr[i] = ok ? p.B + ((long)(n0 + row) * p.ldb + k_begin + c) : zero;
        b_step[i] = ok ? 64 : 0;
    }
    int issued = 0;
    auto issue = [&](int buf) {
        char* sA = smem + buf * STAGE;
        char* sB = sA + A_BYTES;
        const bool live = issued < nk;
        ++issued;
#pragma unroll
        for (int i = 0; i < NAI; ++i) {
            __builtin_amdgcn_global_load_lds((gptr_t)(live ? a_ptr[i] : zero), (lptr_t)(sA + (wave * (NAI * 8) + i * 8) * 128), 16, 0, 0);
            a_ptr[i] += a_step[i];
        }
#pragma unroll
        for (int i = 0; i < NBI; ++i) {
            __builtin_amdgcn_global_load_lds((gptr_t)(live ? b_ptr[i] : zero), (lptr_t)(sB + (wave * (NBI * 8) + i * 8) * 128), 16, 0, 0);
            b_ptr[i] += b_step[i];
        }
    };

    f32x16 acc[TM][TN];
#pragma unroll
    for (int i = 0; i < TM; ++i)
#pragma unroll
        for (int j = 0; j < TN; ++j)
#pragma unroll
            for (int e = 0; e < 16; ++e) acc[i][j][e] = 0.0f;

    int a_off[TM][4], b_off[TN][4];
#pragma unroll
    for (int i = 0; i < TM; ++i) {
        const int row = wm * WM + i * 32 + r;
#pragma unroll
        for (int ks = 0; ks < 4; ++ks) a_off[i][ks] = row * 128 + (((2 * ks + h) ^ ((row >> 1) & 7)) << 4);
    }
#pragma unroll
    for (int j = 0; j < TN; ++j) {
        const int row = wn * WN + j * 32 + r;
#pragma unroll
        for (int ks = 0; ks < 4; ++ks) b_off[j][ks] = A_BYTES + row * 128 + (((2 * ks + h) ^ ((row >> 1) & 7)) << 4);
    }

#pragma unroll
    for (int s = 0; s < D; ++s) issue(s);
    int buf = 0;
    for (int kt = 0; kt < nk; ++kt) {
        wait_vm<LPW*(D - 1)>();
        __builtin_amdgcn_s_barrier();
        asm volatile("" ::: "memory");
        int nbuf = buf + D;
        if (nbuf >= S) nbuf -= S;
        issue(nbuf);
        const char* st = smem + buf * STAGE;
#pragma unroll
        for (int ks = 0; ks < 4; ++ks) {
            bf16x8 af[TM], bf[TN];
#pragma unroll
            for (int i = 0; i < TM; ++i) af[i] = *(const bf16x8*)(st + a_off[i][ks]);
#pragma unroll
            for (int j = 0; j < TN; ++j) bf[j] = *(const bf16x8*)(st + b_off[j][ks]);
#pragma unroll
            for (int i = 0; i < TM; ++i)
#pragma unroll
                for (int j = 0; j < TN; ++j)
                    acc[i][j] = __builtin_amdgcn_mfma_f32_32x32x16_bf16(af[i], bf[j], acc[i][j], 0, 0, 0);
        }
        buf = (buf + 1 == S) ? 0 : buf + 1;
    }
    wait_vm<0>();
    __syncthreads();

    float* ct = (float*)smem;
    float* C = p.C + (long)z * p.slab;
    const bool add_bias = p.bias != nullptr && gridDim.y == 1;
#pragma unroll
    for (int hf = 0; hf < WGM; ++hf) {
        if (wm == hf) {
#pragma unroll
            for (int j = 0; j < TN; ++j) {
                const int col = wn * WN + j * 32 + r;
#pragma unroll
                for (int i = 0; i < TM; ++i)
#pragma unroll
                    for (int e = 0; e < 16; ++e) ct[(i * 32 + (e & 3) + 8 * (e >> 2) + 4 * h) * CROWF + col] = acc[i][j][e];
            }
        }
        __syncthreads();
        constexpr int CPR = BN / 4;
#pragma unroll
        for (int it = 0; it < 64 * CPR / NT; ++it) {
            const int q = tid + it * NT;
            const int row = q / CPR, c4 = q - row * CPR;
            const int grow = m0 + hf * 64 + row, gcol = n0 + c4 * 4;
            if (grow < p.M && gcol < p.N) {
                f32x4 v = *(const f32x4*)(ct + row * CROWF + c4 * 4);
                if (add_bias) {
                    v += *(const f32x4*)(p.bias + gcol);
                    if (p.bias2) v += *(const f32x4*)(p.bias2 + gcol);
                }
                *(f32x4*)(C + (long)grow * p.ldc + gcol) = v;
            }
        }
        __syncthreads();
    }
}

__global__ __launch_bounds__(256) void cast_rows_bf16_kernel(const float* __restrict__ in, long ldi, int R, int C, bf16_t* __restrict__ out,
                                                             long ldo) {
    const long per_row = ldo >> 3, total = (long)R * per_row;
    for (long q = (long)blockIdx.x * 256 + threadIdx.x; q < total; q += (long)gridDim.x * 256) {
        const long row = q / per_row;
        const int c0 = (int)(q - row * per_row) * 8;
        const float* src = in + row * ldi + c0;
        bf16x8 o;
        if (c0 + 8 <= C && ((((uintptr_t)src) & 15) == 0)) {
            const f32x4 a = *(const f32x4*)src, b = *(const f32x4*)(src + 4);
#pragma unroll
            for (int e = 0; e < 4; ++e) { o[e] = (bf16_t)a[e]; o[e + 4] = (bf16_t)b[e]; }
        } else {
#pragma unroll
            for (int e = 0; e < 8; ++e) o[e] = (bf16_t)(c0 + e < C ? src[e] : 0.0f);
        }
        *(bf16x8*)(out + row * ldo + c0) = o;
    }
}

template <typename T> __device__ __forceinline__ float ld_f(const T* p);
template <> __device__ __forceinline__ float ld_f<float>(const float* p) { return *p; }
template <> __device__ __forceinline__ float ld_f<bf16_t>(const bf16_t* p) { return (float)*p; }

template <typename Tin>
__global__ __launch_bounds__(256) void transpose_bf16_kernel(const Tin* __restrict__ in, long ldi, int R, int C, bf16_t* __restrict__ out,
                                                             long ldo, float* __restrict__ psum) {
    __shared__ bf16_t tile[64][66];
    const int c0 = blockIdx.x * 64, r0 = blockIdx.y * 64, t = threadIdx.x;
    {
        const int cc = (t & 15) * 4, rr = t >> 4;
#pragma unroll
        for (int pass = 0; pass < 4; ++pass) {
            const int row = rr + pass * 16;
            const long grow = r0 + row;
#pragma unroll
            for (int e = 0; e < 4; ++e) {
                const int gc = c0 + cc + e;
                tile[row][cc + e] = (bf16_t)((grow < R && gc < C) ? ld_f<Tin>(in + grow * ldi + gc) : 0.0f);
            }
        }
    }
    __syncthreads();
    if (psum && t < 64 && c0 + t < C) {
        float a = 0.0f;
#pragma unroll 8
        for (int rr2 = 0; rr2 < 64; ++rr2) a += (float)tile[rr2][t];
        psum[(long)blockIdx.y * C + c0 + t] = a;
    }
    {
        const int orr = (t & 15) * 4, oc = t >> 4;
#pragma unroll
        for (int pass = 0; pass < 4; ++pass) {
            const int c = oc + pass * 16;
            if (c0 + c < C && r0 + orr < ldo) {
                bf16x4 v;
#pragma unroll
                for (int e = 0; e < 4; ++e) v[e] = tile[orr + e][c];
                *(bf16x4*)(out + (long)(c0 + c) * ldo + r0 + orr) = v;
            }
        }
    }
}

__global__ __launch_bounds__(256) void colsum_bf16_kernel(const bf16_t* __restrict__ x, long ld, int rows, int cols, float* __restrict__ out) {
    __shared__ float sh[8][64];
    const int c2 = (threadIdx.x & 31) * 2, rg = threadIdx.x >> 5;
    const int c = blockIdx.x * 64 + c2;
    float s0 = 0.0f, s1 = 0.0f;
    if (c < cols) {
        for (int r = rg; r < rows; r += 8) {
            const unsigned u = *(const unsigned*)(x + (long)r * ld + c);
            s0 += __uint_as_float(u << 16);
            s1 += __uint_as_float(u & 0xffff0000u);
        }
    }
    sh[rg][c2] = s0;
    sh[rg][c2 + 1] = s1;
    __syncthreads();
    if (threadIdx.x < 64) {
        const int cc = blockIdx.x * 64 + threadIdx.x;
        if (cc < cols) {
            float t = 0.0f;
#pragma unroll
            for (int g = 0; g < 8; ++g) t += sh[g][threadIdx.x];
            out[cc] = t;
        }
    }
}

__device__ __forceinline__ float blk_reduce(float v, bool is_max, float* sh) {
#pragma unroll
    for (int o = 32; o > 0; o >>= 1) {
        const float w = __shfl_xor(v, o, 64);
        v = is_max ? fmaxf(v, w) : v + w;
    }
    __syncthreads();
    if ((threadIdx.x & 63) == 0) sh[threadIdx.x >> 6] = v;
    __syncthreads();
    float r = sh[0];
#pragma unroll
    for (int i = 1; i < 4; ++i) r = is_max ? fmaxf(r, sh[i]) : r + sh[i];
    return r;
}

__global__ __launch_bounds__(256) void ce_rows_bf16grad_kernel(const float* __restrict__ logits, long ldl, const int64_t* __restrict__ targets,
                                                               int V, float inv_denom, float* __restrict__ row_loss,
                                                               bf16_t* __restrict__ grad, long ldg) {
    __shared__ float sh[4];
    constexpr int RC = 12;
    const int row = blockIdx.x, tid = threadIdx.x;
    const float* x = logits + (long)row * ldl;
    const int nq = V >> 2;
    f32x4 rc[RC];
#pragma unroll
    for (int c = 0; c < RC; ++c)
        if (tid + c * 256 < nq) rc[c] = *(const f32x4*)(x + 4 * (tid + c * 256));
    float m = -INFINITY;
#pragma unroll
    for (int c = 0; c < RC; ++c)
        if (tid + c * 256 < nq) m = fmaxf(fmaxf(fmaxf(m, rc[c][0]), fmaxf(rc[c][1], rc[c][2])), rc[c][3]);
    m = blk_reduce(m, true, sh);
    float s = 0.0f;
#pragma unroll
    for (int c = 0; c < RC; ++c)
        if (tid + c * 256 < nq) {
#pragma unroll
            for (int e = 0; e < 4; ++e) s += expf(rc[c][e] - m);
        }
    s = blk_reduce(s, false, sh);
    const float lse = m + logf(s);
    long tgt = targets[row];
    tgt = tgt < 0 ? 0 : (tgt >= V ? V - 1 : tgt);
    const int tq = (int)(tgt >> 2), te = (int)(tgt & 3);
    bf16_t* g = grad + (long)row * ldg;
#pragma unroll
    for (int c = 0; c < RC; ++c) {
        const int q = tid + c * 256;
        if (q < nq) {
            if (q == tq) row_loss[row] = lse - rc[c][te];
            bf16x4 o;
#pragma unroll
            for (int e = 0; e < 4; ++e) o[e] = (bf16_t)((expf(rc[c][e] - lse) - ((4 * q + e) == (int)tgt ? 1.0f : 0.0f)) * inv_denom);
            *(bf16x4*)(g + 4 * q) = o;
        } else if (4 * q < ldg) {
            bf16x4 o = {(bf16_t)0.0f, (bf16_t)0.0f, (bf16_t)0.0f, (bf16_t)0.0f};
            *(bf16x4*)(g + 4 * q) = o;
        }
    }
}

__global__ __launch_bounds__(256) void sum_scale_b_kernel(const float* __restrict__ v, int n, float scale, float* out) {
    __shared__ float sh[4];
    float s = 0.0f;
    for (int i = threadIdx.x; i < n; i += 256) s += v[i];
    s = blk_reduce(s, false, sh);
    if (threadIdx.x == 0) out[0] = s * scale;
}

int pad64(int x) { return (x + 63) / 64 * 64; }

int launch_gemm(const bf16_t* A, long lda, const bf16_t* B, long ldb, float* C, long ldc, const float* bias, int M, int N, int K,
                int ksplit, long slab, hipStream_t s, const float* bias2 = nullptr) {
    if (!A || !B || !C || M < 1 || N < 1 || K < 64 || (K % 64) || (N % 4) || (lda % 8) || (ldb % 8) || (ldc % 4) || ksplit < 1)
        return SAT_ERR_ARG;
    GemmArgs a = {};
    a.A = A; a.B = B; a.C = C; a.bias = bias; a.bias2 = bias2; a.M = M; a.N = N; a.K = K; a.lda = lda; a.ldb = ldb; a.ldc = ldc; a.slab = slab;
    const int nk = K / 64;
    a.ksteps = sat_cdiv(nk, ksplit);
    const int tm = sat_cdiv(M, 128), tn = sat_cdiv(N, 128);
    a.tiles_n = tn;
    const dim3 grid(tm * tn, sat_cdiv(nk, a.ksteps)), block(512);
    const int S = (long)grid.x * grid.y > 256 ? 2 : 3;
    if (S == 2) hipLaunchKernelGGL((gemm_bf16_nt_kernel<128, 2>), grid, block, 0, s, a);
    else hipLaunchKernelGGL((gemm_bf16_nt_kernel<128, 3>), grid, block, 0, s, a);
    SAT_LAUNCH_CHECK();
    return SAT_OK;
}

struct VocabWs {
    int64_t hsb, wb, wtb, hstb, gb, gtb, slabs, psum, total;
    int Npad, Vpad, ks;
};
VocabWs vocab_ws(int N, int H, int V) {
    VocabWs w = {};
    w.Npad = pad64(N); w.Vpad = pad64(V);
    auto al = [](int64_t x) { return (x + 255) / 256 * 256; };
    int64_t off = 0;
    w.hsb = off;  off = al(off + (int64_t)N * H * 2);
    w.wb = off;   off = al(off + (int64_t)V * H * 2);
    w.wtb = off;  off = al(off + (int64_t)H * w.Vpad * 2);
    w.hstb = off; off = al(off + (int64_t)H * w.Npad * 2);
    w.gb = off;   off = al(off + (int64_t)N * w.Vpad * 2);
    w.gtb = off;  off = al(off + (int64_t)V * w.Npad * 2);
    const long tiles = (long)sat_cdiv(N, 128) * sat_cdiv(H, 128);
    int ks = (int)(256 / (tiles > 0 ? tiles : 1));
    const int nk = w.Vpad / 64;
    if (ks > nk / 8) ks = nk / 8;
    w.ks = ks < 1 ? 1 : (ks > 16 ? 16 : ks);
    w.slabs = off; off = al(off + (w.ks > 1 ? (int64_t)w.ks * N * H * 4 : 0));
    w.psum = off; off = al(off + (int64_t)(w.Npad / 64) * V * 4);
    w.total = off;
    return w;
}

bool vocab_bf16_ok(int N, int H, int V) { return N >= 1 && H >= 64 && (H % 64) == 0 && V >= 4 && (V % 4) == 0 && V <= 12288; }

}

extern "C" int sat_sum_slabs_f32(const float* in, int nslab, int64_t slab_stride, int64_t n, float* out, sat_stream_t stream);

extern "C" int sat_gemm_bf16_nt(const void* A, int64_t lda, const void* B, int64_t ldb, float* C, int64_t ldc, const float* bias,
                                int M, int N, int K, int ksplit, int64_t slab_stride, sat_stream_t stream) {
    return launch_gemm((const bf16_t*)A, (long)lda, (const bf16_t*)B, (long)ldb, C, (long)ldc, bias, M, N, K, ksplit, (long)slab_stride,
                       (hipStream_t)stream);
}

extern "C" int sat_transpose_f32_bf16(const float* in, int64_t ldi, int R, int C, void* out, int64_t ldo, sat_stream_t stream) {
    if (!in || !out || R < 1 || C < 1 || ldo < R || (ldo % 4) || ldi < C) return SAT_ERR_ARG;
    hipLaunchKernelGGL((transpose_bf16_kernel<float>), dim3(sat_cdiv(C, 64), sat_cdiv(ldo, 64)), dim3(256), 0, (hipStream_t)stream, in,
                       (long)ldi, R, C, (bf16_t*)out, (long)ldo, (float*)nullptr);
    SAT_LAUNCH_CHECK();
    return SAT_OK;
}

int64_t sat_gemm_mixed_scratch_bytes(int M, int N, int K) {
    const int64_t kp = pad64(K);
    return (((int64_t)M * kp * 2 + 255) / 256 * 256) + (((int64_t)N * kp * 2 + 255) / 256 * 256);
}
int sat_gemm_mixed_nt(const float* A, long lda, int a_kmajor, const float* B, long ldb, int b_kmajor, float* C, long ldc,
                      const float* bias, const float* bias2, int M, int N, int K, void* scratch, int64_t scratch_bytes, hipStream_t s) {
    if (!A || !B || !C || !scratch || M < 1 || N < 1 || K < 1) return SAT_ERR_ARG;
    if ((N % 4) || (ldc % 4)) return SAT_ERR_UNSUPPORTED;
    if (scratch_bytes < sat_gemm_mixed_scratch_bytes(M, N, K) || (((uintptr_t)scratch) & 255)) return SAT_ERR_WORKSPACE;
    const int kp = pad64(K);
    bf16_t* ab = (bf16_t*)scratch;
    bf16_t* bb = (bf16_t*)((char*)scratch + (((int64_t)M * kp * 2 + 255) / 256 * 256));
    auto prep = [&](const float* src, long ld, int kmajor, int rows, bf16_t* dst) {
        if (kmajor) {
            hipLaunchKernelGGL((transpose_bf16_kernel<float>), dim3(sat_cdiv(rows, 64), sat_cdiv(kp, 64)), dim3(256), 0, s, src, ld, K, rows,
                               dst, (long)kp, (float*)nullptr);
        } else {
            long g = ((long)rows * kp / 8 + 255) / 256;
            hipLaunchKernelGGL(cast_rows_bf16_kernel, dim3((unsigned)(g > 2048 ? 2048 : (g < 1 ? 1 : g))), dim3(256), 0, s, src, ld, rows, K,
                               dst, (long)kp);
        }
    };
    prep(A, lda, a_kmajor, M, ab);
    SAT_LAUNCH_CHECK();
    prep(B, ldb, b_kmajor, N, bb);
    SAT_LAUNCH_CHECK();
    return launch_gemm(ab, kp, bb, kp, C, ldc, bias, M, N, kp, 1, 0, s, bias2);
}

extern "C" int64_t sat_vocab_bf16_ws_bytes(int N, int H, int V) { return vocab_bf16_ok(N, H, V) ? vocab_ws(N, H, V).total : 0; }

extern "C" int sat_vocab_ce_fwd_bf16(const float* Hs, const float* w, const float* b, const int64_t* targets, int N, int H, int V,
                                     float inv_denom, float* logits, int64_t ldl, float* row_loss, float* loss_out, void* workspace,
                                     int64_t ws_bytes, sat_stream_t stream) {
    if (!Hs || !w || !b || !targets || !logits || !row_loss || !workspace || ldl < V || (ldl % 4)) return SAT_ERR_ARG;
    if (!vocab_bf16_ok(N, H, V)) return SAT_ERR_UNSUPPORTED;
    const VocabWs L = vocab_ws(N, H, V);
    if (ws_bytes < L.total) return SAT_ERR_WORKSPACE;
    if ((((uintptr_t)workspace) & 255) || (((uintptr_t)logits) & 15)) return SAT_ERR_ARG;
    hipStream_t s = (hipStream_t)stream;
    char* ws = (char*)workspace;
    bf16_t* hsb = (bf16_t*)(ws + L.hsb); bf16_t* wb = (bf16_t*)(ws + L.wb); bf16_t* wtb = (bf16_t*)(ws + L.wtb);
    bf16_t* hstb = (bf16_t*)(ws + L.hstb); bf16_t* gb = (bf16_t*)(ws + L.gb);
    auto egrid = [](long n8) { long g = (n8 + 255) / 256; return dim3((unsigned)(g > 2048 ? 2048 : (g < 1 ? 1 : g))); };
    hipLaunchKernelGGL(cast_rows_bf16_kernel, egrid((long)N * H / 8), dim3(256), 0, s, Hs, (long)H, N, H, hsb, (long)H);
    SAT_LAUNCH_CHECK();
    hipLaunchKernelGGL(cast_rows_bf16_kernel, egrid((long)V * H / 8), dim3(256), 0, s, w, (long)H, V, H, wb, (long)H);
    SAT_LAUNCH_CHECK();
    hipLaunchKernelGGL((transpose_bf16_kernel<float>), dim3(sat_cdiv(H, 64), sat_cdiv(L.Vpad, 64)), dim3(256), 0, s, w, (long)H, V, H, wtb,
                       (long)L.Vpad, (float*)nullptr);
    SAT_LAUNCH_CHECK();
    hipLaunchKernelGGL((transpose_bf16_kernel<float>), dim3(sat_cdiv(H, 64), sat_cdiv(L.Npad, 64)), dim3(256), 0, s, Hs, (long)H, N, H, hstb,
                       (long)L.Npad, (float*)nullptr);
    SAT_LAUNCH_CHECK();
    SAT_TRY(launch_gemm(hsb, H, wb, H, logits, (long)ldl, b, N, V, H, 1, 0, s));
    hipLaunchKernelGGL(ce_rows_bf16grad_kernel, dim3(N), dim3(256), 0, s, logits, (long)ldl, targets, V, inv_denom, row_loss, gb,
                       (long)L.Vpad);
    SAT_LAUNCH_CHECK();
    if (loss_out) {
        hipLaunchKernelGGL(sum_scale_b_kernel, dim3(1), dim3(256), 0, s, row_loss, N, inv_denom, loss_out);
        SAT_LAUNCH_CHECK();
    }
    return SAT_OK;
}

extern "C" int sat_vocab_ce_bwd_bf16(int N, int H, int V, float* dw, float* db, float* dHs, void* workspace, int64_t ws_bytes,
                                     sat_stream_t stream) {
    if (!dw || !db || !dHs || !workspace) return SAT_ERR_ARG;
    if (!vocab_bf16_ok(N, H, V)) return SAT_ERR_UNSUPPORTED;
    const VocabWs L = vocab_ws(N, H, V);
    if (ws_bytes < L.total) return SAT_ERR_WORKSPACE;
    hipStream_t s = (hipStream_t)stream;
    char* ws = (char*)workspace;
    bf16_t* wtb = (bf16_t*)(ws + L.wtb); bf16_t* hstb = (bf16_t*)(ws + L.hstb);
    bf16_t* gb = (bf16_t*)(ws + L.gb); bf16_t* gtb = (bf16_t*)(ws + L.gtb);
    float* slabs = (float*)(ws + L.slabs);
    float* psum = (float*)(ws + L.psum);
    const int rt = sat_cdiv(L.Npad, 64);
    hipLaunchKernelGGL((transpose_bf16_kernel<bf16_t>), dim3(sat_cdiv(V, 64), rt), dim3(256), 0, s, gb, (long)L.Vpad, N, V, gtb,
                       (long)L.Npad, psum);
    SAT_LAUNCH_CHECK();
    SAT_TRY(sat_sum_slabs_f32(psum, rt, (int64_t)V, (int64_t)V, db, stream));
    SAT_TRY(launch_gemm(gtb, L.Npad, hstb, L.Npad, dw, H, nullptr, V, H, L.Npad, 1, 0, s));
    if (L.ks == 1) return launch_gemm(gb, L.Vpad, wtb, L.Vpad, dHs, H, nullptr, N, H, L.Vpad, 1, 0, s);
    SAT_TRY(launch_gemm(gb, L.Vpad, wtb, L.Vpad, slabs, H, nullptr, N, H, L.Vpad, L.ks, (long)N * H, s));
    const int nslab = sat_cdiv(L.Vpad / 64, sat_cdiv(L.Vpad / 64, L.ks));
    return sat_sum_slabs_f32(slabs, nslab, (int64_t)N * H, (int64_t)N * H, dHs, stream);
}
```

show-and-tell_amd/csrc/sat_host.hip:

```cpp
#include "sat_internal.h"
#include <stdio.h>
#include <stdlib.h>

extern "C" int sat_version(void) { return SAT_ABI_VERSION; }

extern "C" const char* sat_error_string(int code) {
    switch (code) {
        case SAT_OK: return "ok";
        case SAT_ERR_ARG: return "sat: bad argument (null pointer, shape or alignment)";
        case SAT_ERR_WORKSPACE: return "sat: workspace too small";
        case SAT_ERR_UNSUPPORTED: return "sat: unsupported configuration";
        default: return hipGetErrorString((hipError_t)code);
    }
}

extern "C" int sat_run_ops(const sat_op* ops, int n_ops, sat_stream_t stream) {
    return sat_run_ops_parity(ops, n_ops, 0, stream);
}

extern "C" int sat_run_ops_parity(const sat_op* ops, int n_ops, int parity, sat_stream_t stream) {
    if (!ops || n_ops < 0 || (parity != 0 && parity != 1)) return SAT_ERR_ARG;
    hipStream_t s = (hipStream_t)stream;
    for (int i = 0; i < n_ops; ++i) {
        const sat_op* op = ops + i;
        int rc;
        switch (op->kind) {
            case SAT_OP_IMAGE_PREP: rc = sat_image_prep_launch(op, s); break;
            case SAT_OP_CONV: rc = sat_conv_launch(op, parity, s); break;
            case SAT_OP_BN_FINALIZE: rc = sat_bn_finalize_launch(op, parity, s); break;
            case SAT_OP_BN_RELU: rc = sat_bn_act_launch(op, false, parity, s); break;
            case SAT_OP_BN_ADD_RELU: rc = sat_bn_act_launch(op, true, parity, s); break;
            case SAT_OP_BN_RELU_MAXPOOL: rc = sat_bn_relu_maxpool_launch(op, parity, s); break;
            case SAT_OP_AVGPOOL: rc = sat_avgpool_launch(op, s); break;
            case SAT_OP_BN_EVAL_BATCH: rc = sat_bn_eval_batch_launch(op, s); break;
            case SAT_OP_MAXPOOL2: rc = sat_maxpool2_launch(op, s); break;
            case SAT_OP_MAXPOOL3S2: rc = sat_pool3_launch(op, false, s); break;
            case SAT_OP_AVGPOOL3: rc = sat_pool3_launch(op, true, s); break;
            case SAT_OP_GRAM: rc = sat_gram_launch(op, parity, s); break;
            case SAT_OP_GRAM_COV: rc = sat_gram_cov_launch(op, s); break;
            case SAT_OP_GEMM_BF16_NT: rc = sat_gemm_bf16_op_launch(op, s); break;
            case SAT_OP_BN_FROM_GRAM: rc = sat_bn_from_gram_launch(op, s); break;
            default: rc = SAT_ERR_UNSUPPORTED;
        }
        if (rc != SAT_OK) return rc;
    }
    return SAT_OK;
}

struct sat_graph {
    hipGraphExec_t exec;
};

extern "C" int sat_graph_create(const sat_op* ops, int n_ops, int parity, sat_graph** graph_out) {
    if (!ops || n_ops <= 0 || !graph_out || (parity != 0 && parity != 1)) return SAT_ERR_ARG;
    *graph_out = nullptr;
    hipStream_t cs = nullptr;
    hipError_t e = hipStreamCreateWithFlags(&cs, hipStreamNonBlocking);
    if (e != hipSuccess) return (int)e;
    e = hipStreamBeginCapture(cs, hipStreamCaptureModeThreadLocal);
    if (e != hipSuccess) {
        (void)hipStreamDestroy(cs);
        return (int)e;
    }
    const int rc = sat_run_ops_parity(ops, n_ops, parity, (sat_stream_t)cs);
    hipGraph_t g = nullptr;
    e = hipStreamEndCapture(cs, &g);
    (void)hipStreamDestroy(cs);
    if (rc != SAT_OK || e != hipSuccess || !g) {
        if (g) (void)hipGraphDestroy(g);
        (void)hipGetLastError();
        return rc != SAT_OK ? rc : (e != hipSuccess ? (int)e : SAT_ERR_UNSUPPORTED);
    }
    hipGraphExec_t exec = nullptr;
    e = hipGraphInstantiate(&exec, g, nullptr, nullptr, 0);
    (void)hipGraphDestroy(g);
    if (e != hipSuccess) return (int)e;
    sat_graph* out = new sat_graph;
    out->exec = exec;
    *graph_out = out;
    return SAT_OK;
}

extern "C" int sat_graph_launch(sat_graph* graph, sat_stream_t stream) {
    if (!graph || !graph->exec) return SAT_ERR_ARG;
    return (int)hipGraphLaunch(graph->exec, (hipStream_t)stream);
}

extern "C" int sat_graph_destroy(sat_graph* graph) {
    if (!graph) return SAT_ERR_ARG;
    hipError_t e = graph->exec ? hipGraphExecDestroy(graph->exec) : hipSuccess;
    delete graph;
    return (int)e;
}

extern "C" int sat_conv_bn_relu_fwd(const sat_op* conv, const sat_op* finalize, const sat_op* bnrelu,
                                    sat_stream_t stream) {
    if (!conv || !finalize || !bnrelu) return SAT_ERR_ARG;
    if (conv->kind != SAT_OP_CONV || finalize->kind != SAT_OP_BN_FINALIZE || bnrelu->kind != SAT_OP_BN_RELU)
        return SAT_ERR_ARG;
    if (conv->out != bnrelu->in0 || conv->Cout != finalize->Cout || conv->Cout != bnrelu->Cout) return SAT_ERR_ARG;
    hipStream_t s = (hipStream_t)stream;
    SAT_TRY(sat_conv_launch(conv, 0, s));
    SAT_TRY(sat_bn_finalize_launch(finalize, 0, s));
    return sat_bn_act_launch(bnrelu, false, 0, s);
}

void sat_conv_arm_timer(hipEvent_t start, hipEvent_t stop);

extern "C" int sat_run_ops_timed(const sat_op* ops, int n_ops, int parity, sat_stream_t stream, float* op_us) {
    if (!ops || n_ops < 0 || !op_us || (parity != 0 && parity != 1)) return SAT_ERR_ARG;
    hipStream_t s = (hipStream_t)stream;
    hipEvent_t* ev = new hipEvent_t[2 * (size_t)(n_ops > 0 ? n_ops : 1)];
    int n_ev = 0, rc = SAT_OK;
    for (int i = 0; i < n_ops && rc == SAT_OK; ++i) {
        const sat_op* op = ops + i;
        op_us[i] = 0.0f;
        const bool timed = op->kind == SAT_OP_CONV && op->dtype == SAT_BF16 && (op->Cout % 8) == 0;
        if (timed) {
            if (hipEventCreate(&ev[n_ev]) != hipSuccess) { rc = SAT_ERR_UNSUPPORTED; break; }
            if (hipEventCreate(&ev[n_ev + 1]) != hipSuccess) { (void)hipEventDestroy(ev[n_ev]); rc = SAT_ERR_UNSUPPORTED; break; }
            sat_conv_arm_timer(ev[n_ev], ev[n_ev + 1]);
            op_us[i] = -1.0f;
            n_ev += 2;
        }
        rc = sat_run_ops_parity(op, 1, parity, stream);
        sat_conv_arm_timer(nullptr, nullptr);
    }
    hipError_t e = hipStreamSynchronize(s);
    if (rc == SAT_OK && e != hipSuccess) rc = (int)e;
    int k = 0;
    for (int i = 0; i < n_ops; ++i) {
        if (op_us[i] >= 0.0f) continue;
        if (k + 2 > n_ev) { op_us[i] = 0.0f; continue; }
        float ms = 0.0f;
        if (rc == SAT_OK && hipEventElapsedTime(&ms, ev[k], ev[k + 1]) == hipSuccess) op_us[i] = ms * 1e3f;
        else op_us[i] = 0.0f;
        k += 2;
    }
    for (int j = 0; j < n_ev; ++j) (void)hipEventDestroy(ev[j]);
    delete[] ev;
    return rc;
}

static int fc_split(int F) { return F >= 1024 ? 8 : (F >= 256 ? 4 : 1); }

extern "C" int64_t sat_fc_bn1d_ws_bytes(int B, int F, int E) {
    return (int64_t)(fc_split(F) + 1) * B * E * sizeof(float);
}

extern "C" int sat_fc_bn1d_fwd(const float* pooled, const float* w_fc, const float* b_fc, const float* gamma,
                               const float* beta, float* running_mean, float* running_var, float momentum, float eps,
                               int training, int B, int F, int E, float* feats, float* xhat, float* rstd,
                               float* workspace, int64_t ws_bytes, sat_stream_t stream) {
    if (!pooled || !w_fc || !b_fc || !gamma || !beta || !running_mean || !running_var || !feats || !xhat || !rstd ||
        !workspace)
        return SAT_ERR_ARG;
    if (ws_bytes < sat_fc_bn1d_ws_bytes(B, F, E)) return SAT_ERR_WORKSPACE;
    hipStream_t s = (hipStream_t)stream;
    const int nz = fc_split(F);
    float* part = workspace;
    float* zbuf = workspace + (long)nz * B * E;
    SAT_TRY(sat_skinny_store(pooled, F, w_fc, F, 0, B, E, F, nz, part, E, (long)B * E, nullptr, s));
    return sat_bn1d_fwd_launch(part, nz, (long)B * E, b_fc, gamma, beta, running_mean, running_var, momentum, eps,
                               training, B, E, zbuf, feats, xhat, rstd, s);
}

extern "C" int sat_fc_bn1d_bwd(const float* dy, const float* pooled, const float* xhat, const float* rstd,
                               const float* gamma, int B, int F, int E, float* dw_fc, float* db_fc, float* dgamma,
                               float* dbeta, float* workspace, int64_t ws_bytes, sat_stream_t stream) {
    if (!dy || !pooled || !xhat || !rstd || !gamma || !dw_fc || !db_fc || !dgamma || !dbeta || !workspace)
        return SAT_ERR_ARG;
    if (ws_bytes < (int64_t)B * E * (int64_t)sizeof(float)) return SAT_ERR_WORKSPACE;
    if ((E & 3) || (F & 3)) return SAT_ERR_UNSUPPORTED;
    hipStream_t s = (hipStream_t)stream;
    float* dz = workspace;
    SAT_TRY(sat_bn1d_bwd_launch(dy, xhat, rstd, gamma, B, E, dz, dgamma, dbeta, db_fc, s));
    if (B <= 1024) return sat_outer_wgrad_launch(dz, pooled, B, E, F, dw_fc, s);
    return sat_gemm_f32(2, 1, dz, E, pooled, F, dw_fc, F, nullptr, nullptr, E, F, B, stream);
}

bool sat_lstm_persist_ok(int B, int H, int T, int n_cu);
int sat_lstm_persist_rows(int B, int H, int T, int n_cu);
int sat_lstm_persist_launch(float* GA, const float* W, float* CS, float* HS, float* HP, const int32_t* batch_sizes, int T,
                            int H, int rows, void* workspace, int64_t ws_bytes, hipStream_t s);
int64_t sat_lstm_persist_bwd_ws_bytes(int B, int H);
int sat_lstm_persist_bwd_launch(const float* dHS, const float* GA, const float* CS, const float* W, float* DG,
                                const int32_t* batch_sizes, int T, int H, void* xch, unsigned* err, hipStream_t s);

static int device_cu_count() {
    static int n = -1;
    if (n < 0) {
        int dev = 0, v = 0;
        if (hipGetDevice(&dev) == hipSuccess && hipDeviceGetAttribute(&v, hipDeviceAttributeMultiprocessorCount, dev) == hipSuccess) n = v;
        else n = 0;
    }
    return n;
}

static int lstm_fwd_impl(const float* X, const float* w_ih, const float* w_hh, const float* b_ih,
                         const float* b_hh, const int32_t* batch_sizes, int T, int In, int H, float* GA,
                         float* CS, float* HS, float* HP, float* c_state, void* workspace, int64_t ws_bytes,
                         void* mixed, int64_t mixed_bytes, sat_stream_t stream) {
    if (!X || !w_ih || !w_hh || !b_ih || !b_hh || !batch_sizes || !GA || !CS || !HS || !HP || !c_state || T < 1)
        return SAT_ERR_ARG;
    if ((In & 3) || (H & 3)) return SAT_ERR_UNSUPPORTED;
    hipStream_t s = (hipStream_t)stream;
    const int B = batch_sizes[0];
    long N = 0;
    for (int t = 0; t < T; ++t) {
        if (batch_sizes[t] < 1 || (t > 0 && batch_sizes[t] > batch_sizes[t - 1])) return SAT_ERR_ARG;
        N += batch_sizes[t];
    }
    if (mixed && mixed_bytes >= sat_gemm_mixed_scratch_bytes((int)N, 4 * H, In))
        SAT_TRY(sat_gemm_mixed_nt(X, In, 0, w_ih, In, 0, GA, 4L * H, b_ih, b_hh, (int)N, 4 * H, In, mixed, mixed_bytes, s));
    else
        SAT_TRY(sat_gemm_f32(0, 0, X, In, w_ih, In, GA, 4L * H, b_ih, b_hh, (int)N, 4 * H, In, stream));
    hipError_t e = hipMemsetAsync(HP, 0, (size_t)B * H * sizeof(float), s);
    if (e != hipSuccess) return (int)e;
    static const int persist_env = getenv("SAT_LSTM_PERSIST") ? atoi(getenv("SAT_LSTM_PERSIST")) : 1;
    const int prow = (persist_env && workspace && ws_bytes >= sat_lstm_fwd_ws_bytes(B, H)) ? sat_lstm_persist_rows(B, H, T, device_cu_count()) : 0;
    if (prow) return sat_lstm_persist_launch(GA, w_hh, CS, HS, HP, batch_sizes, T, H, prow, workspace, ws_bytes, s);
    const int64_t soff = sat_lstm_fwd_status_offset(B, H);
    if (workspace && soff >= 0 && ws_bytes >= soff + 64) {
        e = hipMemsetAsync((char*)workspace + soff, 0, 64, s);
        if (e != hipSuccess) return (int)e;
    }
    e = hipMemsetAsync(c_state, 0, (size_t)B * H * sizeof(float), s);
    if (e != hipSuccess) return (int)e;
    long off = 0;
    for (int t = 0; t < T; ++t) {
        const int n = batch_sizes[t];
        const int n_next = (t + 1 < T) ? batch_sizes[t + 1] : 0;
        float* ga = GA + off * 4 * H;
        SAT_TRY(sat_skinny_lstm(HP + off * H, w_hh, nullptr, nullptr, 0, nullptr, nullptr, ga, 4L * H, n, H, c_state,
                                ga, 4L * H, CS + off * H, HS + off * H, n_next ? HP + (off + n) * H : nullptr, n_next, s));
        off += n;
    }
    return SAT_OK;
}

extern "C" int sat_lstm_fwd(const float* X, const float* w_ih, const float* w_hh, const float* b_ih,
                            const float* b_hh, const int32_t* batch_sizes, int T, int In, int H, float* GA,
                            float* CS, float* HS, float* HP, float* c_state, void* workspace, int64_t ws_bytes,
                            sat_stream_t stream) {
    return lstm_fwd_impl(X, w_ih, w_hh, b_ih, b_hh, batch_sizes, T, In, H, GA, CS, HS, HP, c_state, workspace, ws_bytes, nullptr, 0, stream);
}

extern "C" int64_t sat_lstm_mixed_ws_bytes(int N, int In, int H) {
    int64_t m = sat_gemm_mixed_scratch_bytes(N, 4 * H, In);
    const int64_t c[3] = {sat_gemm_mixed_scratch_bytes(4 * H, In, N), sat_gemm_mixed_scratch_bytes(4 * H, H, N),
                          sat_gemm_mixed_scratch_bytes(N, In, 4 * H)};
    for (int i = 0; i < 3; ++i) m = c[i] > m ? c[i] : m;
    return m;
}

extern "C" int sat_lstm_fwd_bf16(const float* X, const float* w_ih, const float* w_hh, const float* b_ih,
                                 const float* b_hh, const int32_t* batch_sizes, int T, int In, int H, float* GA,
                                 float* CS, float* HS, float* HP, float* c_state, void* workspace, int64_t ws_bytes,
                                 void* mixed_ws, int64_t mixed_bytes, sat_stream_t stream) {
    if (!mixed_ws) return SAT_ERR_ARG;
    return lstm_fwd_impl(X, w_ih, w_hh, b_ih, b_hh, batch_sizes, T, In, H, GA, CS, HS, HP, c_state, workspace, ws_bytes, mixed_ws,
                         mixed_bytes, stream);
}

static int lstm_bwd_split(int H) {
    const int ncg = sat_cdiv(H, 16);
    int nz = 256 / (ncg > 0 ? ncg : 1);
    return nz < 1 ? 1 : (nz > 16 ? 16 : nz);
}

extern "C" int64_t sat_lstm_bwd_ws_bytes(int B, int H) {
    return (int64_t)(lstm_bwd_split(H) + 1) * B * H * sizeof(float);
}

static int fill_split(long M, long Nn, long K) {
    const long tiles = (long)sat_cdiv(M, 64) * sat_cdiv(Nn, 64);
    if (tiles >= 192 || K < 256) return 1;
    long ks = 384 / (tiles > 0 ? tiles : 1);
    const long max_by_k = K / 128;
    if (ks > max_by_k) ks = max_by_k;
    return (int)(ks < 1 ? 1 : (ks > 8 ? 8 : ks));
}

static int64_t lstm_bwd_xb(int B, int H) {
    const int64_t xb = sat_lstm_persist_bwd_ws_bytes(B, H);
    return xb >= 64 ? xb : 64;
}
static int64_t lstm_bwd_head_bytes(int B, int H) { return (lstm_bwd_xb(B, H) + 255) / 256 * 256; }
static int64_t lstm_bwd_slab_bytes(int N, int B, int In, int H) {
    const int64_t base = sat_lstm_bwd_ws_bytes(B, H);
    const int64_t dx = (int64_t)fill_split(N, In, 4L * H) * N * In * sizeof(float);
    const int64_t dw = (int64_t)fill_split(4L * H, In, N) * 4 * H * In * sizeof(float);
    int64_t m = dx > dw ? dx : dw;
    if (base > m) m = base;
    return (m + 255) / 256 * 256;
}

extern "C" int64_t sat_lstm_bwd_ws_bytes_full(int N, int B, int In, int H) {
    return lstm_bwd_head_bytes(B, H) + lstm_bwd_slab_bytes(N, B, In, H);
}
extern "C" int64_t sat_lstm_bwd_ws_bytes_max(int n_max, int B, int In, int H) {
    int64_t m = sat_lstm_bwd_ws_bytes(B, H);
    const int64_t dx = 8LL * n_max * In * sizeof(float), dw = 8LL * 4 * H * In * sizeof(float);
    if (dx > m) m = dx;
    if (dw > m) m = dw;
    return lstm_bwd_head_bytes(B, H) + (m + 255) / 256 * 256;
}

extern "C" int64_t sat_lstm_bwd_status_offset(int N, int B, int In, int H) {
    (void)N; (void)In;
    return lstm_bwd_xb(B, H) - 64;
}

static int lstm_bwd_impl(const float* dHS, const float* X, const float* w_ih, const float* w_hh, const float* GA,
                         const float* CS, const float* HP, const int32_t* batch_sizes, int T, int In, int H,
                         float* DG, float* dw_ih, float* dw_hh, float* db_ih, float* db_hh, float* dX,
                         float* workspace, int64_t ws_bytes, void* mixed, int64_t mixed_bytes, sat_stream_t stream) {
    if (!dHS || !X || !w_ih || !w_hh || !GA || !CS || !HP || !batch_sizes || !DG || !dw_ih || !dw_hh || !db_ih ||
        !db_hh || !workspace || T < 1)
        return SAT_ERR_ARG;
    if ((In & 3) || (H & 3)) return SAT_ERR_UNSUPPORTED;
    hipStream_t s = (hipStream_t)stream;
    const int B = batch_sizes[0];
    if (ws_bytes < sat_lstm_bwd_ws_bytes(B, H)) return SAT_ERR_WORKSPACE;
    long N = 0;
    for (int t = 0; t < T; ++t) N += batch_sizes[t];
    const int nz = lstm_bwd_split(H);
    const long slab = (long)B * H;
    const int64_t full = sat_lstm_bwd_ws_bytes_full((int)N, B, In, H);
    const bool roomy = ws_bytes >= full;
    char* const ws0 = (char*)workspace;
    if (roomy) workspace = (float*)(ws0 + lstm_bwd_head_bytes(B, H));
    float* dc_state = workspace + nz * slab;
    hipError_t e = hipMemsetAsync(dc_state, 0, (size_t)slab * sizeof(float), s);
    if (e != hipSuccess) return (int)e;
    static const int persist_bwd = getenv("SAT_LSTM_PERSIST_BWD") ? atoi(getenv("SAT_LSTM_PERSIST_BWD")) : 1;
    bool recurrence_done = false;
    if (roomy) {
        unsigned* status = (unsigned*)(ws0 + sat_lstm_bwd_status_offset((int)N, B, In, H));
        if (persist_bwd && sat_lstm_persist_bwd_ws_bytes(B, H) > 0 && sat_lstm_persist_ok(B, H, T, device_cu_count())) {
            SAT_TRY(sat_lstm_persist_bwd_launch(dHS, GA, CS, w_hh, DG, batch_sizes, T, H, ws0, status, s));
            recurrence_done = true;
        } else {
            e = hipMemsetAsync(status, 0, 64, s);
            if (e != hipSuccess) return (int)e;
        }
    }
    long off = N;
    for (int t = T - 1; t >= 0 && !recurrence_done; --t) {
        const int n = batch_sizes[t];
        off -= n;
        const int n_next = (t + 1 < T) ? batch_sizes[t + 1] : 0;
        const float* cs_prev = (t > 0) ? CS + (off - batch_sizes[t - 1]) * H : nullptr;
        SAT_TRY(sat_lstm_bwd_step(dHS + off * H, n_next ? DG + (off + n) * 4 * H : nullptr, n_next, w_hh, GA + off * 4 * H,
                                  CS + off * H, cs_prev, dc_state, DG + off * 4 * H, n, H, s));
    }
    if (mixed && mixed_bytes >= sat_lstm_mixed_ws_bytes((int)N, In, H)) {
        SAT_TRY(sat_gemm_mixed_nt(DG, 4L * H, 1, X, In, 1, dw_ih, In, nullptr, nullptr, 4 * H, In, (int)N, mixed, mixed_bytes, s));
        SAT_TRY(sat_gemm_mixed_nt(DG, 4L * H, 1, HP, H, 1, dw_hh, H, nullptr, nullptr, 4 * H, H, (int)N, mixed, mixed_bytes, s));
        SAT_TRY(sat_colsum_f32(DG, 4L * H, (int)N, 4 * H, db_ih, stream));
        e = hipMemcpyAsync(db_hh, db_ih, (size_t)4 * H * sizeof(float), hipMemcpyDeviceToDevice, s);
        if (e != hipSuccess) return (int)e;
        if (dX) SAT_TRY(sat_gemm_mixed_nt(DG, 4L * H, 0, w_ih, In, 1, dX, In, nullptr, nullptr, (int)N, In, 4 * H, mixed, mixed_bytes, s));
        return SAT_OK;
    }
    const int ks_dw = roomy ? fill_split(4L * H, In, N) : 1;
    if (ks_dw > 1) {
        SAT_TRY(sat_gemm_f32_splitk(2, 1, DG, 4L * H, X, In, workspace, In, nullptr, nullptr, 4 * H, In, (int)N, ks_dw,
                                    (int64_t)4 * H * In, stream));
        SAT_TRY(sat_sum_slabs_f32(workspace, ks_dw, (int64_t)4 * H * In, (int64_t)4 * H * In, dw_ih, stream));
    } else {
        SAT_TRY(sat_gemm_f32(2, 1, DG, 4L * H, X, In, dw_ih, In, nullptr, nullptr, 4 * H, In, (int)N, stream));
    }
    SAT_TRY(sat_gemm_f32(2, 1, DG, 4L * H, HP, H, dw_hh, H, nullptr, nullptr, 4 * H, H, (int)N, stream));
    SAT_TRY(sat_colsum_f32(DG, 4L * H, (int)N, 4 * H, db_ih, stream));
    e = hipMemcpyAsync(db_hh, db_ih, (size_t)4 * H * sizeof(float), hipMemcpyDeviceToDevice, s);
    if (e != hipSuccess) return (int)e;
    if (dX) {
        const int ks_dx = roomy ? fill_split(N, In, 4L * H) : 1;
        if (ks_dx > 1) {
            SAT_TRY(sat_gemm_f32_splitk(0, 1, DG, 4L * H, w_ih, In, workspace, In, nullptr, nullptr, (int)N, In, 4 * H, ks_dx,
                                        (int64_t)N * In, stream));
            SAT_TRY(sat_sum_slabs_f32(workspace, ks_dx, (int64_t)N * In, (int64_t)N * In, dX, stream));
        } else {
            SAT_TRY(sat_gemm_f32(0, 1, DG, 4L * H, w_ih, In, dX, In, nullptr, nullptr, (int)N, In, 4 * H, stream));
        }
    }
    return SAT_OK;
}

extern "C" int sat_lstm_bwd(const float* dHS, const float* X, const float* w_ih, const float* w_hh, const float* GA,
                            const float* CS, const float* HP, const int32_t* batch_sizes, int T, int In, int H,
                            float* DG, float* dw_ih, float* dw_hh, float* db_ih, float* db_hh, float* dX,
                            float* workspace, int64_t ws_bytes, sat_stream_t stream) {
    return lstm_bwd_impl(dHS, X, w_ih, w_hh, GA, CS, HP, batch_sizes, T, In, H, DG, dw_ih, dw_hh, db_ih, db_hh, dX, workspace, ws_bytes,
                         nullptr, 0, stream);
}

extern "C" int sat_lstm_bwd_bf16(const float* dHS, const float* X, const float* w_ih, const float* w_hh, const float* GA,
                                 const float* CS, const float* HP, const int32_t* batch_sizes, int T, int In, int H,
                                 float* DG, float* dw_ih, float* dw_hh, float* db_ih, float* db_hh, float* dX,
                                 float* workspace, int64_t ws_bytes, void* mixed_ws, int64_t mixed_bytes, sat_stream_t stream) {
    if (!mixed_ws) return SAT_ERR_ARG;
    return lstm_bwd_impl(dHS, X, w_ih, w_hh, GA, CS, HP, batch_sizes, T, In, H, DG, dw_ih, dw_hh, db_ih, db_hh, dX, workspace, ws_bytes,
                         mixed_ws, mixed_bytes, stream);
}

extern "C" int sat_vocab_logits_fwd(const float* Hs, const float* w, const float* b, int N, int H, int V,
                                    float* logits, int64_t ldl, sat_stream_t stream) {
    if (!Hs || !w || !b || !logits || ldl < V) return SAT_ERR_ARG;
    return sat_gemm_f32(0, 0, Hs, H, w, H, logits, ldl, b, nullptr, N, V, H, stream);
}

static int vocab_bwd_split(int N, int H, int V) {
    const long tiles = (long)sat_cdiv(N, 64) * sat_cdiv(H, 64);
    int ks = (int)(512 / (tiles > 0 ? tiles : 1));
    const int nk = sat_cdiv(V, 32);
    if (ks > nk / 8) ks = nk / 8;
    return ks < 1 ? 1 : (ks > 16 ? 16 : ks);
}

extern "C" int64_t sat_vocab_ce_bwd_ws_bytes(int N, int H, int V) {
    const int ks = vocab_bwd_split(N, H, V);
    return ks > 1 ? (int64_t)ks * N * H * sizeof(float) : 0;
}

extern "C" int sat_sum_slabs_f32(const float* in, int nslab, int64_t slab_stride, int64_t n, float* out, sat_stream_t stream);
extern "C" int sat_gemm_f32_splitk(int amode, int bmode, const float* A, int64_t lda, const float* B, int64_t ldb,
                                   float* C, int64_t ldc, const float* bias, const float* bias2, int M, int N, int K,
                                   int ksplit, int64_t slab_stride, sat_stream_t stream);

extern "C" int sat_vocab_ce_bwd(const float* dlogits, int64_t ldl, const float* Hs, const float* w, int N, int H, int V,
                                float* dw, float* db, float* dHs, float* workspace, int64_t ws_bytes,
                                sat_stream_t stream) {
    if (!dlogits || !Hs || !w || !dw || !db || !dHs) return SAT_ERR_ARG;
    if ((H & 3) || (ldl & 3) || ldl < ((V + 3) & ~3)) return SAT_ERR_UNSUPPORTED;
    const int ks = vocab_bwd_split(N, H, V);
    if (ks > 1 && (!workspace || ws_bytes < sat_vocab_ce_bwd_ws_bytes(N, H, V))) return SAT_ERR_WORKSPACE;
    SAT_TRY(sat_gemm_f32(2, 1, dlogits, ldl, Hs, H, dw, H, nullptr, nullptr, V, H, N, stream));
    SAT_TRY(sat_colsum_f32(dlogits, ldl, N, V, db, stream));
    if (ks == 1) return sat_gemm_f32(0, 1, dlogits, ldl, w, H, dHs, H, nullptr, nullptr, N, H, V, stream);
    SAT_TRY(sat_gemm_f32_splitk(0, 1, dlogits, ldl, w, H, workspace, H, nullptr, nullptr, N, H, V, ks, (int64_t)N * H, stream));
    if (((long)N * H) & 3) return SAT_ERR_UNSUPPORTED;
    return sat_sum_slabs_f32(workspace, ks, (int64_t)N * H, (int64_t)N * H, dHs, stream);
}
```

show-and-tell_amd/csrc/sat_internal.h:

```cpp
#pragma once
#include "sat_common.h"
#include "../../include/sat_hip.h"

int sat_conv_launch(const sat_op* op, int parity, hipStream_t s);
int sat_conv_check_args(const sat_op* op);
int sat_image_prep_launch(const sat_op* op, hipStream_t s);
int sat_bn_finalize_launch(const sat_op* op, int parity, hipStream_t s);
int sat_bn_eval_batch_launch(const sat_op* op, hipStream_t s);
int sat_bn_act_launch(const sat_op* op, bool add, int parity, hipStream_t s);
int sat_bn_relu_maxpool_launch(const sat_op* op, int parity, hipStream_t s);
int sat_avgpool_launch(const sat_op* op, hipStream_t s);
int sat_maxpool2_launch(const sat_op* op, hipStream_t s);
int sat_pool3_launch(const sat_op* op, bool avg, hipStream_t s);
int sat_gram_launch(const sat_op* op, int parity, hipStream_t s);
int sat_gram_cov_launch(const sat_op* op, hipStream_t s);
int sat_gemm_bf16_op_launch(const sat_op* op, hipStream_t s);
int sat_bn_from_gram_launch(const sat_op* op, hipStream_t s);

int64_t sat_gemm_mixed_scratch_bytes(int M, int N, int K);
int sat_gemm_mixed_nt(const float* A, long lda, int a_kmajor, const float* B, long ldb, int b_kmajor, float* C, long ldc,
                      const float* bias, const float* bias2, int M, int N, int K, void* scratch, int64_t scratch_bytes, hipStream_t s);

int sat_skinny_store(const float* A, long lda, const float* W, long ldw, int wkm, int M, int N, int K, int nz,
                     float* out, long ldo, long slab_stride, const float* bias, hipStream_t s);
int sat_skinny_lstm(const float* h_prev, const float* w_hh, const float* x, const float* w_ih, int In,
                    const float* bias, const float* bias2, const float* xg, long ldxg, int M, int H,
                    float* c_state, float* ga, long ldga, float* cs, float* h_out, float* h_out2, int m2,
                    hipStream_t s);
int sat_lstm_bwd_step(const float* dHS, const float* DG_next, int n_next, const float* w_hh, const float* GA, const float* CS,
                      const float* CS_prev, float* dc_state, float* DG, int n, int H, hipStream_t s);
int sat_lstm_bwd_point_launch(const float* dHS, const float* dh_part, int nz, long slab_stride, int n_next,
                              const float* GA, const float* CS, const float* CS_prev, float* dc_state, float* DG,
                              int n, int H, hipStream_t s);
int sat_bn1d_fwd_launch(const float* part, int nz, long slab_stride, const float* b_fc, const float* gamma,
                        const float* beta, float* rm, float* rv, float momentum, float eps, int training, int B, int E,
                        float* zbuf, float* feats, float* xhat, float* rstd, hipStream_t s);
int sat_outer_wgrad_launch(const float* dz, const float* x, int B, int E, int F, float* dw, hipStream_t s);
int sat_bn1d_bwd_launch(const float* dy, const float* xhat, const float* rstd, const float* gamma, int B, int E,
                        float* dz, float* dgamma, float* dbeta, float* db_fc, hipStream_t s);

inline int64_t al256(int64_t n) { return (n + 255) / 256 * 256; }

#define SAT_STAT_SCALE 4194304.0

#define SAT_TRY(expr)                 \
    do {                              \
        int rc__ = (expr);            \
        if (rc__ != SAT_OK) return rc__; \
    } while (0)
```

Before: 19500.

## Read f32 and k-major operands directly in bf16 GEMM, skipping transpose copies

Extends the bf16 MFMA GEMM so it can load operands directly as f32 (converted to bf16 in registers) or as k-major layouts (using LDS transpose reads). With operand copies off by default, the LSTM input and weight-gradient GEMMs and the vocab CE backward skip their separate cast and transpose kernels and their scratch traffic. The bn1d partial-sum loop and the outer wgrad loop are also unrolled by 8 to expose more loads in flight. The risks are more register pressure and uncoalesced k-major f32 loads inside the GEMM main loop.

```diff
diff --git a/include/sat_hip.h b/include/sat_hip.h
--- a/include/sat_hip.h
+++ b/include/sat_hip.h
@@ -194,6 +194,15 @@
                           int64_t ws_bytes, sat_stream_t stream);
 int sat_gemm_bf16_nt(const void* A, int64_t lda, const void* B, int64_t ldb, float* C, int64_t ldc, const float* bias,
                      int M, int N, int K, int ksplit, int64_t slab_stride, sat_stream_t stream);
+#define SAT_GEMM_OP_KMAJOR 1
+#define SAT_GEMM_OP_F32 2
+int sat_gemm_bf16_ex(const void* A, int64_t lda, int a_layout, const void* B, int64_t ldb, int b_layout, float* C, int64_t ldc,
+                     const float* bias, int M, int N, int K, int ksplit, int64_t slab_stride, sat_stream_t stream);
+int64_t sat_gemm_mixed_f32_ws_bytes(int M, int N, int K);
+int sat_gemm_mixed_f32_nt(const float* A, int64_t lda, int a_kmajor, const float* B, int64_t ldb, int b_kmajor, float* C, int64_t ldc,
+                          const float* bias, const float* bias2, int M, int N, int K, void* scratch, int64_t scratch_bytes,
+                          sat_stream_t stream);
+int sat_gemm_operand_copies(int on);
 int sat_transpose_f32_bf16(const float* in, int64_t ldi, int R, int C, void* out, int64_t ldo, sat_stream_t stream);
 int sat_vocab_ce_fwd(const float* Hs , const float* w , const float* b , const int64_t* targets ,
                      int N, int H, int V, float inv_denom, float* logits , int64_t ldl,
diff --git a/show-and-tell_amd/_lib.py b/show-and-tell_amd/_lib.py
--- a/show-and-tell_amd/_lib.py
+++ b/show-and-tell_amd/_lib.py
@@ -125,6 +125,10 @@
     "sat_vocab_ce_bwd_bf16": (_i, [_i, _i, _i, _vp, _vp, _vp, _vp, _i64, _vp]),
     "sat_gemm_bf16_nt": (_i, [_vp, _i64, _vp, _i64, _vp, _i64, _vp, _i, _i, _i, _i, _i64, _vp]),
     "sat_transpose_f32_bf16": (_i, [_vp, _i64, _i, _i, _vp, _i64, _vp]),
+    "sat_gemm_bf16_ex": (_i, [_vp, _i64, _i, _vp, _i64, _i, _vp, _i64, _vp, _i, _i, _i, _i, _i64, _vp]),
+    "sat_gemm_operand_copies": (_i, [_i]),
+    "sat_gemm_mixed_f32_ws_bytes": (_i64, [_i, _i, _i]),
+    "sat_gemm_mixed_f32_nt": (_i, [_vp, _i64, _i, _vp, _i64, _i, _vp, _i64, _vp, _vp, _i, _i, _i, _vp, _i64, _vp]),
     "sat_vocab_ce_bwd": (_i, [_vp, _i64, _vp, _vp, _i, _i, _i, _vp, _vp, _vp, _vp, _i64, _vp]),
     "sat_vocab_ce_bwd_ws_bytes": (_i64, [_i, _i, _i]),
     "sat_gemm_f32_splitk": (_i, [_i, _i, _vp, _i64, _vp, _i64, _vp, _i64, _vp, _vp, _i, _i, _i, _i, _i64, _vp]),
diff --git a/show-and-tell_amd/csrc/sat_elementwise.hip b/show-and-tell_amd/csrc/sat_elementwise.hip
--- a/show-and-tell_amd/csrc/sat_elementwise.hip
+++ b/show-and-tell_amd/csrc/sat_elementwise.hip
@@ -771,7 +771,14 @@
     if (ok)
         for (int b = rg; b < B; b += 8) {
             float z = b_fc[e];
-            for (int k = 0; k < nz; ++k) z += part[(long)k * slab_stride + (long)b * E + e];
+            const float* p0 = part + (long)b * E + e;
+            for (int k0 = 0; k0 < nz; k0 += 8) {
+                float v[8];
+#pragma unroll
+                for (int u = 0; u < 8; ++u) v[u] = p0[(long)(k0 + u < nz ? k0 + u : nz - 1) * slab_stride];
+#pragma unroll
+                for (int u = 0; u < 8; ++u) z = k0 + u < nz ? z + v[u] : z;
+            }
             zbuf[(long)b * E + e] = z;
             s += z;
         }
@@ -1115,6 +1122,45 @@
     if (i >= (long)E * f4) return;
     const int e = (int)(i / f4), f = (int)(i - (long)e * f4) * 4;
     f32x4 acc = {0.f, 0.f, 0.f, 0.f};
+    int b = 0;
+    for (; b + 8 <= B; b += 8) {
+        float d[8];
+        f32x4 v[8];
+#pragma unroll
+        for (int u = 0; u < 8; ++u) {
+            d[u] = dz[(long)(b + u) * E + e];
+            v[u] = *(const f32x4*)(x + (long)(b + u) * F + f);
+        }
+#pragma unroll
+        for (int u = 0; u < 8; ++u)
+#pragma unroll
+            for (int k = 0; k < 4; ++k) acc[k] = fmaf(d[u], v[u][k], acc[k]);
+    }
+    for (; b < B; ++b) {
+        const float d = dz[(long)b * E + e];
+        const f32x4 v = *(const f32x4*)(x + (long)b * F + f);
+#pragma unroll
+        for (int k = 0; k < 4; ++k) acc[k] = fmaf(d, v[k], acc[k]);
+    }
+    *(f32x4*)(dw + (long)e * F + f) = acc;
+}
+
+int sat_outer_wgrad_launch(const float* dz, const float* x, int B, int E, int F, float* dw, hipStream_t s) {
+    const long n = (long)E * (F >> 2);
+    hipLaunchKernelGGL(outer_wgrad_kernel, dim3((unsigned)((n + 255) / 256)), dim3(256), 0, s, dz, x, B, E, F, dw);
+    SAT_LAUNCH_CHECK();
+    return SAT_OK;
+}
+
+#ifdef SAT_TESTHOOKS
+namespace {
+__global__ __launch_bounds__(256) void outer_wgrad_ref_kernel(const float* __restrict__ dz, const float* __restrict__ x, int B, int E, int F,
+                                                              float* __restrict__ dw) {
+    const long i = (long)blockIdx.x * 256 + threadIdx.x;
+    const int f4 = F >> 2;
+    if (i >= (long)E * f4) return;
+    const int e = (int)(i / f4), f = (int)(i - (long)e * f4) * 4;
+    f32x4 acc = {0.f, 0.f, 0.f, 0.f};
     for (int b = 0; b < B; ++b) {
         const float d = dz[(long)b * E + e];
         const f32x4 v = *(const f32x4*)(x + (long)b * F + f);
@@ -1124,12 +1170,94 @@
     *(f32x4*)(dw + (long)e * F + f) = acc;
 }
 
-int sat_outer_wgrad_launch(const float* dz, const float* x, int B, int E, int F, float* dw, hipStream_t s) {
+__global__ __launch_bounds__(256) void bn1d_fwd_ref_kernel(const float* __restrict__ part, int nz, long slab_stride,
+                                                           const float* __restrict__ b_fc, const float* __restrict__ gamma,
+                                                           const float* __restrict__ beta, float* running_mean,
+                                                           float* running_var, float momentum, float eps, int training,
+                                                           int B, int E, float* __restrict__ zbuf, float* __restrict__ feats,
+                                                           float* __restrict__ xhat, float* __restrict__ rstd_out) {
+    __shared__ float sh[8][32];
+    __shared__ float bc[2][32];
+    const int cl = threadIdx.x & 31, rg = threadIdx.x >> 5;
+    const int e = blockIdx.x * 32 + cl;
+    const bool ok = e < E;
+    float s = 0.0f;
+    if (ok)
+        for (int b = rg; b < B; b += 8) {
+            float z = b_fc[e];
+            for (int k = 0; k < nz; ++k) z += part[(long)k * slab_stride + (long)b * E + e];
+            zbuf[(long)b * E + e] = z;
+            s += z;
+        }
+    sh[rg][cl] = s;
+    __syncthreads();
+    if (rg == 0) {
+        float t = 0.0f;
+        for (int g = 0; g < 8; ++g) t += sh[g][cl];
+        bc[0][cl] = t / (float)B;
+    }
+    __syncthreads();
+    float mean = bc[0][cl];
+    float q = 0.0f;
+    if (ok)
+        for (int b = rg; b < B; b += 8) {
+            const float d = zbuf[(long)b * E + e] - mean;
+            q += d * d;
+        }
+    __syncthreads();
+    sh[rg][cl] = q;
+    __syncthreads();
+    if (rg == 0 && ok) {
+        float t = 0.0f;
+        for (int g = 0; g < 8; ++g) t += sh[g][cl];
+        float var = t / (float)B;
+        if (training) {
+            const float unb = B > 1 ? t / (float)(B - 1) : var;
+            running_mean[e] = (1.0f - momentum) * running_mean[e] + momentum * mean;
+            running_var[e] = (1.0f - momentum) * running_var[e] + momentum * unb;
+        } else {
+            mean = running_mean[e];
+            var = running_var[e];
+        }
+        const float rs = 1.0f / sqrtf(var + eps);
+        bc[0][cl] = mean;
+        bc[1][cl] = rs;
+        rstd_out[e] = rs;
+    }
+    __syncthreads();
+    if (ok) {
+        const float mu = bc[0][cl], rs = bc[1][cl], ga = gamma[e], be = beta[e];
+        for (int b = rg; b < B; b += 8) {
+            const float xh = (zbuf[(long)b * E + e] - mu) * rs;
+            xhat[(long)b * E + e] = xh;
+            feats[(long)b * E + e] = xh * ga + be;
+        }
+    }
+}
+}
+
+extern "C" int sat_test_outer_wgrad(int ref, const float* dz, const float* x, int B, int E, int F, float* dw, sat_stream_t stream) {
+    if (!dz || !x || !dw || B < 1 || E < 1 || F < 4 || (F & 3)) return SAT_ERR_ARG;
+    if (!ref) return sat_outer_wgrad_launch(dz, x, B, E, F, dw, (hipStream_t)stream);
     const long n = (long)E * (F >> 2);
-    hipLaunchKernelGGL(outer_wgrad_kernel, dim3((unsigned)((n + 255) / 256)), dim3(256), 0, s, dz, x, B, E, F, dw);
-    SAT_LAUNCH_CHECK();
-    return SAT_OK;
-}
+    hipLaunchKernelGGL(outer_wgrad_ref_kernel, dim3((unsigned)((n + 255) / 256)), dim3(256), 0, (hipStream_t)stream, dz, x, B, E, F, dw);
+    SAT_LAUNCH_CHECK();
+    return SAT_OK;
+}
+
+extern "C" int sat_test_bn1d_fwd(int ref, const float* part, int nz, int64_t slab_stride, const float* b_fc, const float* gamma,
+                                 const float* beta, float* rm, float* rv, float momentum, float eps, int training, int B, int E,
+                                 float* zbuf, float* feats, float* xhat, float* rstd, sat_stream_t stream) {
+    if (!part || !b_fc || !gamma || !beta || !rm || !rv || !zbuf || !feats || !xhat || !rstd || nz < 1 || B < 1 || E < 1) return SAT_ERR_ARG;
+    if (!ref)
+        return sat_bn1d_fwd_launch(part, nz, (long)slab_stride, b_fc, gamma, beta, rm, rv, momentum, eps, training, B, E, zbuf, feats, xhat,
+                                   rstd, (hipStream_t)stream);
+    hipLaunchKernelGGL(bn1d_fwd_ref_kernel, dim3(sat_cdiv(E, 32)), dim3(256), 0, (hipStream_t)stream, part, nz, (long)slab_stride, b_fc,
+                       gamma, beta, rm, rv, momentum, eps, training, B, E, zbuf, feats, xhat, rstd);
+    SAT_LAUNCH_CHECK();
+    return SAT_OK;
+}
+#endif
 
 int sat_bn1d_bwd_launch(const float* dy, const float* xhat, const float* rstd, const float* gamma, int B, int E,
                         float* dz, float* dgamma, float* dbeta, float* db_fc, hipStream_t s) {
diff --git a/show-and-tell_amd/csrc/sat_gemm_bf16.hip b/show-and-tell_amd/csrc/sat_gemm_bf16.hip
--- a/show-and-tell_amd/csrc/sat_gemm_bf16.hip
+++ b/show-and-tell_amd/csrc/sat_gemm_bf16.hip
@@ -7,9 +7,11 @@
 typedef const __attribute__((address_space(1))) void* gptr_t;
 typedef __attribute__((address_space(3))) void* lptr_t;
 
+enum : int { OP_KC16 = 0, OP_KM16 = 1, OP_KC32 = 2, OP_KM32 = 3 };
+
 struct GemmArgs {
-    const bf16_t* A;
-    const bf16_t* B;
+    const void* A;
+    const void* B;
     float* C;
     const float* bias;
     const float* bias2;
@@ -18,21 +20,173 @@
     int tiles_n, ksteps;
 };
 
+__device__ __forceinline__ int km_swz(int row) { return ((row & 3) << 2) | ((row >> 2) & 3); }
+__device__ __forceinline__ int km_off(int krow, int chunk) { return 256 * krow + 16 * (chunk ^ km_swz(krow)); }
+
+typedef float f32x4_u __attribute__((ext_vector_type(4), aligned(4)));
+typedef short s16x4 __attribute__((ext_vector_type(4)));
+typedef short s16x8 __attribute__((ext_vector_type(8)));
+typedef __attribute__((address_space(3))) s16x4* lds_s16x4_t;
+
+constexpr int kRegSets = 3;
+template <int L>
+struct OperandStage {
+    static constexpr bool KM = (L & 1) != 0, F32 = (L & 2) != 0;
+    const bf16_t* dptr[2];
+    long dstep[2];
+    int dk[2];
+    const float* fptr[2];
+    long fstep;
+    const float* fbase;
+    int fk[2], fvalid[2], fdst[2];
+    f32x4 reg[kRegSets][2][2];
+    unsigned fok[kRegSets];
+
+    __device__ __forceinline__ void init(const void* base, long ld, int rows, int r0, int k_begin, int tid, int wave, int lane,
+                                         const bf16_t* zero) {
+        if constexpr (!F32) {
+#pragma unroll
+            for (int i = 0; i < 2; ++i) {
+                if constexpr (!KM) {
+                    const int row = wave * 16 + i * 8 + (lane >> 3);
+                    const int c = ((lane & 7) ^ ((row >> 1) & 7)) * 8;
+                    const bool ok = r0 + row < rows;
+                    dptr[i] = ok ? (const bf16_t*)base + ((long)(r0 + row) * ld + k_begin + c) : zero;
+                    dstep[i] = ok ? 64 : 0;
+                    dk[i] = 0;
+                } else {
+                    const int krow = (wave * 2 + i) * 4 + (lane >> 4);
+                    const int col = r0 + ((lane & 15) ^ km_swz(krow)) * 8;
+                    const bool ok = col < rows;
+                    dptr[i] = ok ? (const bf16_t*)base + ((long)(k_begin + krow) * ld + col) : zero;
+                    dstep[i] = ok ? 64 * ld : 0;
+                    dk[i] = k_begin + krow;
+                }
+            }
+        } else {
+            fbase = (const float*)base;
+#pragma unroll
+            for (int u = 0; u < kRegSets; ++u) fok[u] = 0u;
+#pragma unroll
+            for (int j = 0; j < 2; ++j) {
+                if constexpr (!KM) {
+                    const int c = tid & 7, row = (tid >> 3) + 64 * j;
+                    fptr[j] = (const float*)base + ((long)(r0 + row) * ld + k_begin + c * 8);
+                    fk[j] = k_begin + c * 8;
+                    fvalid[j] = r0 + row < rows ? 8 : 0;
+                    fdst[j] = row * 128 + ((c ^ ((row >> 1) & 7)) << 4);
+                    fstep = 64;
+                } else {
+                    const int lc = tid & 15, krow = (tid >> 4) + 32 * j;
+                    const int left = rows - (r0 + lc * 8);
+                    fptr[j] = (const float*)base + ((long)(k_begin + krow) * ld + r0 + lc * 8);
+                    fk[j] = k_begin + krow;
+                    fvalid[j] = left < 0 ? 0 : (left > 8 ? 8 : left);
+                    fdst[j] = km_off(krow, lc);
+                    fstep = 64 * ld;
+                }
+            }
+        }
+    }
+    template <bool TAIL>
+    __device__ __forceinline__ void load(int set, bool live, int K) {
+        if constexpr (F32) {
+#pragma unroll
+            for (int j = 0; j < 2; ++j) {
+                int n = 0;
+                if (live) {
+                    if constexpr (!KM) { n = K - fk[j]; n = n < fvalid[j] ? n : fvalid[j]; }
+                    else n = fk[j] < K ? fvalid[j] : 0;
+                }
+                if constexpr (!TAIL) {
+                    const bool ok = n >= 8;
+                    const float* src = ok ? fptr[j] : fbase;
+                    reg[set][j][0] = *(const f32x4_u*)src;
+                    reg[set][j][1] = *(const f32x4_u*)(src + 4);
+                    fok[set] = (fok[set] & ~(1u << j)) | ((ok ? 1u : 0u) << j);
+                } else {
+                    const float* src = fptr[j];
+#pragma unroll
+                    for (int e = 0; e < 8; ++e) reg[set][j][e >> 2][e & 3] = e < n ? src[e] : 0.0f;
+                    fok[set] |= 1u << j;
+                }
+                fptr[j] += fstep;
+                fk[j] += 64;
+            }
+        }
+    }
+    __device__ __forceinline__ void dma(bool live, int K, char* img, int wave, const bf16_t* zero) {
+        if constexpr (!F32) {
+#pragma unroll
+            for (int i = 0; i < 2; ++i) {
+                bool in = live;
+                if constexpr (KM) in = live && dk[i] < K;
+                __builtin_amdgcn_global_load_lds((gptr_t)(in ? dptr[i] : zero), (lptr_t)(img + (wave * 16 + i * 8) * 128), 16, 0, 0);
+                dptr[i] += dstep[i];
+                dk[i] += 64;
+            }
+        }
+    }
+    __device__ __forceinline__ void store(int set, char* img) {
+        if constexpr (F32) {
+#pragma unroll
+            for (int j = 0; j < 2; ++j) {
+                bf16x8 o;
+                const bool ok = (fok[set] >> j) & 1u;
+#pragma unroll
+                for (int e = 0; e < 4; ++e) {
+                    o[e] = (bf16_t)(ok ? reg[set][j][0][e] : 0.0f);
+                    o[e + 4] = (bf16_t)(ok ? reg[set][j][1][e] : 0.0f);
+                }
+                *(bf16x8*)(img + fdst[j]) = o;
+            }
+        }
+    }
+};
+
+template <int L>
+__device__ __forceinline__ void frag_offsets(int blk, int lane, int (&off)[4]) {
+    if constexpr ((L & 1) == 0) {
+        const int row = blk * 32 + (lane & 31), h = lane >> 5;
+#pragma unroll
+        for (int ks = 0; ks < 4; ++ks) off[ks] = row * 128 + (((2 * ks + h) ^ ((row >> 1) & 7)) << 4);
+    } else {
+        const int g16 = lane >> 4, sub = g16 & 1, h = g16 >> 1, q = (lane & 15) >> 2, pp = lane & 3;
+#pragma unroll
+        for (int e = 0; e < 2; ++e) off[e] = km_off(8 * h + 4 * e + q, blk * 4 + 2 * sub + (pp >> 1)) + 8 * (pp & 1);
+        off[2] = off[3] = 0;
+    }
+}
+template <int L>
+__device__ __forceinline__ bf16x8 frag_read(const char* img, const int (&off)[4], int ks) {
+    if constexpr ((L & 1) == 0) {
+        return *(const bf16x8*)(img + off[ks]);
+    } else {
+        const s16x4 lo = __builtin_amdgcn_ds_read_tr16_b64_v4i16((lds_s16x4_t)(img + ks * 4096 + off[0]));
+        const s16x4 hi = __builtin_amdgcn_ds_read_tr16_b64_v4i16((lds_s16x4_t)(img + ks * 4096 + off[1]));
+        const s16x8 v = {lo[0], lo[1], lo[2], lo[3], hi[0], hi[1], hi[2], hi[3]};
+        return __builtin_bit_cast(bf16x8, v);
+    }
+}
+
 template <int N> __device__ __forceinline__ void wait_vm() {
-    static_assert(N == 0 || N == 4 || N == 6 || N == 8 || N == 12, "add the vmcnt literal");
+    static_assert(N == 0 || N == 2 || N == 4 || N == 6 || N == 8 || N == 12, "add the vmcnt literal");
     if constexpr (N == 0) asm volatile("s_waitcnt vmcnt(0)" ::: "memory");
+    if constexpr (N == 2) asm volatile("s_waitcnt vmcnt(2)" ::: "memory");
     if constexpr (N == 4) asm volatile("s_waitcnt vmcnt(4)" ::: "memory");
     if constexpr (N == 6) asm volatile("s_waitcnt vmcnt(6)" ::: "memory");
     if constexpr (N == 8) asm volatile("s_waitcnt vmcnt(8)" ::: "memory");
     if constexpr (N == 12) asm volatile("s_waitcnt vmcnt(12)" ::: "memory");
 }
 
-template <int BN, int S>
+template <int BN, int S, int AL, int BL, bool TAIL>
 __global__ __launch_bounds__(512) void gemm_bf16_nt_kernel(const GemmArgs p) {
+    static_assert(BN == 128, "the operand stages are 128 rows");
     constexpr int BM = 128, NT = 512;
     constexpr int A_BYTES = BM * 128, B_BYTES = BN * 128, STAGE = A_BYTES + B_BYTES;
     constexpr int WGM = 2, WGN = 4, WM = BM / WGM, WN = BN / WGN, TM = WM / 32, TN = WN / 32;
-    constexpr int NAI = BM / 64, NBI = BN / 64, LPW = NAI + NBI;
+    constexpr bool A_F32 = (AL & 2) != 0, B_F32 = (BL & 2) != 0, ANY_F32 = A_F32 || B_F32;
+    constexpr int LPW = (A_F32 ? 0 : 2) + (B_F32 ? 0 : 2);
     constexpr int D = S - 1;
     constexpr int CROWF = BN + 4;
     static_assert(64 * CROWF * 4 <= S * STAGE, "half of the f32 output tile must fit the ring");
@@ -49,47 +203,33 @@
     const int tile_m = swz / p.tiles_n, tile_n = swz - tile_m * p.tiles_n;
     const int m0 = tile_m * BM, n0 = tile_n * BN;
     const int k_begin = z * p.ksteps * 64;
-    int nk = (p.K - k_begin) / 64;
+    int nk = (p.K - k_begin + 63) / 64;
     if (nk > p.ksteps) nk = p.ksteps;
     if (nk < 0) nk = 0;
 
     const bf16_t* zero = (const bf16_t*)&g_zero16_b;
-    const bf16_t* a_ptr[NAI];
-    const bf16_t* b_ptr[NBI];
-    int a_step[NAI], b_step[NBI];
-#pragma unroll
-    for (int i = 0; i < NAI; ++i) {
-        const int row = wave * (NAI * 8) + i * 8 + (lane >> 3);
-        const int c = ((lane & 7) ^ ((row >> 1) & 7)) * 8;
-        const bool ok = m0 + row < p.M;
-        a_ptr[i] = ok ? p.A + ((long)(m0 + row) * p.lda + k_begin + c) : zero;
-        a_step[i] = ok ? 64 : 0;
-    }
-#pragma unroll
-    for (int i = 0; i < NBI; ++i) {
-        const int row = wave * (NBI * 8) + i * 8 + (lane >> 3);
-        const int c = ((lane & 7) ^ ((row >> 1) & 7)) * 8;
-        const bool ok = n0 + row < p.N;
-        b_ptr[i] = ok ? p.B + ((long)(n0 + row) * p.ldb + k_begin + c) : zero;
-        b_step[i] = ok ? 64 : 0;
-    }
-    int issued = 0;
+    OperandStage<AL> opa;
+    OperandStage<BL> opb;
+    opa.init(p.A, p.lda, p.M, m0, k_begin, tid, wave, lane, zero);
+    opb.init(p.B, p.ldb, p.N, n0, k_begin, tid, wave, lane, zero);
+    int issued = 0, asked = 0;
     auto issue = [&](int buf) {
         char* sA = smem + buf * STAGE;
-        char* sB = sA + A_BYTES;
         const bool live = issued < nk;
         ++issued;
-#pragma unroll
-        for (int i = 0; i < NAI; ++i) {
-            __builtin_amdgcn_global_load_lds((gptr_t)(live ? a_ptr[i] : zero), (lptr_t)(sA + (wave * (NAI * 8) + i * 8) * 128), 16, 0, 0);
-            a_ptr[i] += a_step[i];
-        }
-#pragma unroll
-        for (int i = 0; i < NBI; ++i) {
-            __builtin_amdgcn_global_load_lds((gptr_t)(live ? b_ptr[i] : zero), (lptr_t)(sB + (wave * (NBI * 8) + i * 8) * 128), 16, 0, 0);
-            b_ptr[i] += b_step[i];
-        }
+        opa.dma(live, p.K, sA, wave, zero);
+        opb.dma(live, p.K, sA + A_BYTES, wave, zero);
     };
+    auto ask = [&](int set) {
+        const bool live = asked < nk;
+        ++asked;
+        opa.template load<TAIL>(set, live, p.K);
+        opb.template load<TAIL>(set, live, p.K);
+    };
+    auto stash = [&](int set, int buf) {
+        opa.store(set, smem + buf * STAGE);
+        opb.store(set, smem + buf * STAGE + A_BYTES);
+    };
 
     f32x16 acc[TM][TN];
 #pragma unroll
@@ -101,36 +241,43 @@
 
     int a_off[TM][4], b_off[TN][4];
 #pragma unroll
-    for (int i = 0; i < TM; ++i) {
-        const int row = wm * WM + i * 32 + r;
-#pragma unroll
-        for (int ks = 0; ks < 4; ++ks) a_off[i][ks] = row * 128 + (((2 * ks + h) ^ ((row >> 1) & 7)) << 4);
-    }
-#pragma unroll
-    for (int j = 0; j < TN; ++j) {
-        const int row = wn * WN + j * 32 + r;
-#pragma unroll
-        for (int ks = 0; ks < 4; ++ks) b_off[j][ks] = A_BYTES + row * 128 + (((2 * ks + h) ^ ((row >> 1) & 7)) << 4);
-    }
+    for (int i = 0; i < TM; ++i) frag_offsets<AL>((wm * WM) / 32 + i, lane, a_off[i]);
+#pragma unroll
+    for (int j = 0; j < TN; ++j) frag_offsets<BL>((wn * WN) / 32 + j, lane, b_off[j]);
 
 #pragma unroll
     for (int s = 0; s < D; ++s) issue(s);
+    if constexpr (ANY_F32) {
+        ask(0);
+        stash(0, 0);
+#pragma unroll
+        for (int j = 1; j <= kRegSets; ++j) ask(j % kRegSets);
+    }
     int buf = 0;
-    for (int kt = 0; kt < nk; ++kt) {
-        wait_vm<LPW*(D - 1)>();
+    for (int kt0 = 0; kt0 < nk; kt0 += kRegSets) {
+#pragma unroll
+    for (int u = 0; u < kRegSets; ++u) {
+        const int kt = kt0 + u;
+        if (kt >= nk) break;
+        if constexpr (LPW > 0) wait_vm<ANY_F32 ? 0 : LPW*(D - 1)>();
+        if constexpr (ANY_F32) asm volatile("s_waitcnt lgkmcnt(0)" ::: "memory");
         __builtin_amdgcn_s_barrier();
         asm volatile("" ::: "memory");
         int nbuf = buf + D;
         if (nbuf >= S) nbuf -= S;
         issue(nbuf);
+        if constexpr (ANY_F32) {
+            stash((u + 1) % kRegSets, buf + 1 == S ? 0 : buf + 1);
+            ask((u + 1) % kRegSets);
+        }
         const char* st = smem + buf * STAGE;
 #pragma unroll
         for (int ks = 0; ks < 4; ++ks) {
             bf16x8 af[TM], bf[TN];
 #pragma unroll
-            for (int i = 0; i < TM; ++i) af[i] = *(const bf16x8*)(st + a_off[i][ks]);
-#pragma unroll
-            for (int j = 0; j < TN; ++j) bf[j] = *(const bf16x8*)(st + b_off[j][ks]);
+            for (int i = 0; i < TM; ++i) af[i] = frag_read<AL>(st, a_off[i], ks);
+#pragma unroll
+            for (int j = 0; j < TN; ++j) bf[j] = frag_read<BL>(st + A_BYTES, b_off[j], ks);
 #pragma unroll
             for (int i = 0; i < TM; ++i)
 #pragma unroll
@@ -138,6 +285,7 @@
                     acc[i][j] = __builtin_amdgcn_mfma_f32_32x32x16_bf16(af[i], bf[j], acc[i][j], 0, 0, 0);
         }
         buf = (buf + 1 == S) ? 0 : buf + 1;
+    }
     }
     wait_vm<0>();
     __syncthreads();
@@ -241,6 +389,27 @@
     }
 }
 
+__global__ __launch_bounds__(64) void colsum64_bf16_kernel(const bf16_t* __restrict__ x, long ld, int R, int C, float* __restrict__ psum) {
+    const int c = (blockIdx.x * 64 + threadIdx.x) * 2, r0 = blockIdx.y * 64;
+    if (c >= C) return;
+    unsigned u[64];
+#pragma unroll
+    for (int i = 0; i < 64; ++i) {
+        const int row = r0 + i < R ? r0 + i : R - 1;
+        u[i] = *(const unsigned*)(x + (long)row * ld + c);
+    }
+    float s0 = 0.0f, s1 = 0.0f;
+#pragma unroll
+    for (int i = 0; i < 64; ++i) {
+        const bool in = r0 + i < R;
+        s0 += in ? __uint_as_float(u[i] << 16) : 0.0f;
+        s1 += in ? __uint_as_float(u[i] & 0xffff0000u) : 0.0f;
+    }
+    float* o = psum + (long)blockIdx.y * C + c;
+    o[0] = s0;
+    if (c + 1 < C) o[1] = s1;
+}
+
 __global__ __launch_bounds__(256) void colsum_bf16_kernel(const bf16_t* __restrict__ x, long ld, int rows, int cols, float* __restrict__ out) {
     __shared__ float sh[8][64];
     const int c2 = (threadIdx.x & 31) * 2, rg = threadIdx.x >> 5;
@@ -337,6 +506,63 @@
 }
 
 int pad64(int x) { return (x + 63) / 64 * 64; }
+
+template <int S, int AL, int BL>
+void launch_tail(bool tail, dim3 grid, hipStream_t s, const GemmArgs& a) {
+    if constexpr (((AL | BL) & 2) != 0) {
+        if (tail) { hipLaunchKernelGGL((gemm_bf16_nt_kernel<128, S, AL, BL, true>), grid, dim3(512), 0, s, a); return; }
+    }
+    hipLaunchKernelGGL((gemm_bf16_nt_kernel<128, S, AL, BL, false>), grid, dim3(512), 0, s, a);
+}
+template <int S, int AL>
+void launch_layouts_b(int bl, bool tail, dim3 grid, hipStream_t s, const GemmArgs& a) {
+    switch (bl) {
+        case OP_KC16: launch_tail<S, AL, OP_KC16>(tail, grid, s, a); break;
+        case OP_KM16: launch_tail<S, AL, OP_KM16>(tail, grid, s, a); break;
+        case OP_KC32: launch_tail<S, AL, OP_KC32>(tail, grid, s, a); break;
+        default:      launch_tail<S, AL, OP_KM32>(tail, grid, s, a); break;
+    }
+}
+template <int S>
+void launch_layouts(int al, int bl, bool tail, dim3 grid, hipStream_t s, const GemmArgs& a) {
+    switch (al) {
+        case OP_KC16: launch_layouts_b<S, OP_KC16>(bl, tail, grid, s, a); break;
+        case OP_KM16: launch_layouts_b<S, OP_KM16>(bl, tail, grid, s, a); break;
+        case OP_KC32: launch_layouts_b<S, OP_KC32>(bl, tail, grid, s, a); break;
+        default:      launch_layouts_b<S, OP_KM32>(bl, tail, grid, s, a); break;
+    }
+}
+
+bool operand_tail(int layout, int rows, int K) {
+    if (!(layout & 2)) return false;
+    return (((layout & 1) ? rows : K) % 8) != 0 || (long)rows * K < 8;
+}
+
+bool operand_ok(const void* ptr, long ld, int layout, int rows, int K) {
+    if (!ptr || layout < OP_KC16 || layout > OP_KM32) return false;
+    const long extent = (layout & 1) ? rows : K;
+    if (layout & 2) return ld >= extent;
+    if ((ld % 8) || (((uintptr_t)ptr) & 15)) return false;
+    return ld >= ((layout & 1) ? (extent + 7) / 8 * 8 : (extent + 63) / 64 * 64);
+}
+
+int launch_gemm_ex(const void* A, long lda, int al, const void* B, long ldb, int bl, float* C, long ldc, const float* bias, int M, int N,
+                   int K, int ksplit, long slab, hipStream_t s, const float* bias2 = nullptr) {
+    if (!C || M < 1 || N < 1 || K < 1 || (N % 4) || (ldc % 4) || ldc < N || ksplit < 1) return SAT_ERR_ARG;
+    if (!operand_ok(A, lda, al, M, K) || !operand_ok(B, ldb, bl, N, K)) return SAT_ERR_ARG;
+    GemmArgs a = {};
+    a.A = A; a.B = B; a.C = C; a.bias = bias; a.bias2 = bias2; a.M = M; a.N = N; a.K = K; a.lda = lda; a.ldb = ldb; a.ldc = ldc; a.slab = slab;
+    const int nk = sat_cdiv(K, 64);
+    a.ksteps = sat_cdiv(nk, ksplit);
+    const int tm = sat_cdiv(M, 128), tn = sat_cdiv(N, 128);
+    a.tiles_n = tn;
+    const dim3 grid(tm * tn, sat_cdiv(nk, a.ksteps));
+    const bool tail = operand_tail(al, M, K) || operand_tail(bl, N, K);
+    if ((long)grid.x * grid.y > 256) launch_layouts<2>(al, bl, tail, grid, s, a);
+    else launch_layouts<3>(al, bl, tail, grid, s, a);
+    SAT_LAUNCH_CHECK();
+    return SAT_OK;
+}
 
 int launch_gemm(const bf16_t* A, long lda, const bf16_t* B, long ldb, float* C, long ldc, const float* bias, int M, int N, int K,
                 int ksplit, long slab, hipStream_t s, const float* bias2 = nullptr) {
@@ -350,8 +576,8 @@
     a.tiles_n = tn;
     const dim3 grid(tm * tn, sat_cdiv(nk, a.ksteps)), block(512);
     const int S = (long)grid.x * grid.y > 256 ? 2 : 3;
-    if (S == 2) hipLaunchKernelGGL((gemm_bf16_nt_kernel<128, 2>), grid, block, 0, s, a);
-    else hipLaunchKernelGGL((gemm_bf16_nt_kernel<128, 3>), grid, block, 0, s, a);
+    if (S == 2) hipLaunchKernelGGL((gemm_bf16_nt_kernel<128, 2, OP_KC16, OP_KC16, false>), grid, block, 0, s, a);
+    else hipLaunchKernelGGL((gemm_bf16_nt_kernel<128, 3, OP_KC16, OP_KC16, false>), grid, block, 0, s, a);
     SAT_LAUNCH_CHECK();
     return SAT_OK;
 }
@@ -394,6 +620,25 @@
                        (hipStream_t)stream);
 }
 
+extern "C" int sat_gemm_bf16_ex(const void* A, int64_t lda, int a_layout, const void* B, int64_t ldb, int b_layout, float* C, int64_t ldc,
+                                const float* bias, int M, int N, int K, int ksplit, int64_t slab_stride, sat_stream_t stream) {
+    return launch_gemm_ex(A, (long)lda, a_layout, B, (long)ldb, b_layout, C, (long)ldc, bias, M, N, K, ksplit, (long)slab_stride,
+                          (hipStream_t)stream);
+}
+
+int sat_gemm_operands_nt(const void* A, long lda, int a_layout, const void* B, long ldb, int b_layout, float* C, long ldc,
+                         const float* bias, const float* bias2, int M, int N, int K, hipStream_t s) {
+    return launch_gemm_ex(A, lda, a_layout, B, ldb, b_layout, C, ldc, bias, M, N, K, 1, 0, s, bias2);
+}
+
+static int g_operand_copies = 0;
+extern "C" int sat_gemm_operand_copies(int on) {
+    const int was = g_operand_copies;
+    g_operand_copies = on ? 1 : 0;
+    return was;
+}
+int sat_gemm_operand_copies_on() { return g_operand_copies; }
+
 extern "C" int sat_transpose_f32_bf16(const float* in, int64_t ldi, int R, int C, void* out, int64_t ldo, sat_stream_t stream) {
     if (!in || !out || R < 1 || C < 1 || ldo < R || (ldo % 4) || ldi < C) return SAT_ERR_ARG;
     hipLaunchKernelGGL((transpose_bf16_kernel<float>), dim3(sat_cdiv(C, 64), sat_cdiv(ldo, 64)), dim3(256), 0, (hipStream_t)stream, in,
@@ -431,6 +676,14 @@
     return launch_gemm(ab, kp, bb, kp, C, ldc, bias, M, N, kp, 1, 0, s, bias2);
 }
 
+extern "C" int64_t sat_gemm_mixed_f32_ws_bytes(int M, int N, int K) { return sat_gemm_mixed_scratch_bytes(M, N, K); }
+extern "C" int sat_gemm_mixed_f32_nt(const float* A, int64_t lda, int a_kmajor, const float* B, int64_t ldb, int b_kmajor, float* C,
+                                     int64_t ldc, const float* bias, const float* bias2, int M, int N, int K, void* scratch,
+                                     int64_t scratch_bytes, sat_stream_t stream) {
+    return sat_gemm_mixed_nt(A, (long)lda, a_kmajor, B, (long)ldb, b_kmajor, C, (long)ldc, bias, bias2, M, N, K, scratch, scratch_bytes,
+                             (hipStream_t)stream);
+}
+
 extern "C" int64_t sat_vocab_bf16_ws_bytes(int N, int H, int V) { return vocab_bf16_ok(N, H, V) ? vocab_ws(N, H, V).total : 0; }
 
 extern "C" int sat_vocab_ce_fwd_bf16(const float* Hs, const float* w, const float* b, const int64_t* targets, int N, int H, int V,
@@ -450,12 +703,14 @@
     SAT_LAUNCH_CHECK();
     hipLaunchKernelGGL(cast_rows_bf16_kernel, egrid((long)V * H / 8), dim3(256), 0, s, w, (long)H, V, H, wb, (long)H);
     SAT_LAUNCH_CHECK();
-    hipLaunchKernelGGL((transpose_bf16_kernel<float>), dim3(sat_cdiv(H, 64), sat_cdiv(L.Vpad, 64)), dim3(256), 0, s, w, (long)H, V, H, wtb,
-                       (long)L.Vpad, (float*)nullptr);
-    SAT_LAUNCH_CHECK();
-    hipLaunchKernelGGL((transpose_bf16_kernel<float>), dim3(sat_cdiv(H, 64), sat_cdiv(L.Npad, 64)), dim3(256), 0, s, Hs, (long)H, N, H, hstb,
-                       (long)L.Npad, (float*)nullptr);
-    SAT_LAUNCH_CHECK();
+    if (g_operand_copies) {
+        hipLaunchKernelGGL((transpose_bf16_kernel<float>), dim3(sat_cdiv(H, 64), sat_cdiv(L.Vpad, 64)), dim3(256), 0, s, w, (long)H, V, H, wtb,
+                           (long)L.Vpad, (float*)nullptr);
+        SAT_LAUNCH_CHECK();
+        hipLaunchKernelGGL((transpose_bf16_kernel<float>), dim3(sat_cdiv(H, 64), sat_cdiv(L.Npad, 64)), dim3(256), 0, s, Hs, (long)H, N, H,
+                           hstb, (long)L.Npad, (float*)nullptr);
+        SAT_LAUNCH_CHECK();
+    }
     SAT_TRY(launch_gemm(hsb, H, wb, H, logits, (long)ldl, b, N, V, H, 1, 0, s));
     hipLaunchKernelGGL(ce_rows_bf16grad_kernel, dim3(N), dim3(256), 0, s, logits, (long)ldl, targets, V, inv_denom, row_loss, gb,
                        (long)L.Vpad);
@@ -478,6 +733,20 @@
     bf16_t* wtb = (bf16_t*)(ws + L.wtb); bf16_t* hstb = (bf16_t*)(ws + L.hstb);
     bf16_t* gb = (bf16_t*)(ws + L.gb); bf16_t* gtb = (bf16_t*)(ws + L.gtb);
     float* slabs = (float*)(ws + L.slabs);
+    if (!g_operand_copies) {
+        const bf16_t* hsb = (const bf16_t*)(ws + L.hsb);
+        const bf16_t* wb = (const bf16_t*)(ws + L.wb);
+        float* psum = (float*)(ws + L.psum);
+        const int rt = sat_cdiv(N, 64);
+        hipLaunchKernelGGL(colsum64_bf16_kernel, dim3(sat_cdiv(V, 128), rt), dim3(64), 0, s, gb, (long)L.Vpad, N, V, psum);
+        SAT_LAUNCH_CHECK();
+        SAT_TRY(sat_sum_slabs_f32(psum, rt, (int64_t)V, (int64_t)V, db, stream));
+        SAT_TRY(launch_gemm_ex(gb, L.Vpad, OP_KM16, hsb, H, OP_KM16, dw, H, nullptr, V, H, N, 1, 0, s));
+        if (L.ks == 1) return launch_gemm_ex(gb, L.Vpad, OP_KC16, wb, H, OP_KM16, dHs, H, nullptr, N, H, V, 1, 0, s);
+        SAT_TRY(launch_gemm_ex(gb, L.Vpad, OP_KC16, wb, H, OP_KM16, slabs, H, nullptr, N, H, V, L.ks, (long)N * H, s));
+        const int nslab = sat_cdiv(L.Vpad / 64, sat_cdiv(L.Vpad / 64, L.ks));
+        return sat_sum_slabs_f32(slabs, nslab, (int64_t)N * H, (int64_t)N * H, dHs, stream);
+    }
     float* psum = (float*)(ws + L.psum);
     const int rt = sat_cdiv(L.Npad, 64);
     hipLaunchKernelGGL((transpose_bf16_kernel<bf16_t>), dim3(sat_cdiv(V, 64), rt), dim3(256), 0, s, gb, (long)L.Vpad, N, V, gtb,
diff --git a/show-and-tell_amd/csrc/sat_host.hip b/show-and-tell_amd/csrc/sat_host.hip
--- a/show-and-tell_amd/csrc/sat_host.hip
+++ b/show-and-tell_amd/csrc/sat_host.hip
@@ -211,9 +211,12 @@
         if (batch_sizes[t] < 1 || (t > 0 && batch_sizes[t] > batch_sizes[t - 1])) return SAT_ERR_ARG;
         N += batch_sizes[t];
     }
-    if (mixed && mixed_bytes >= sat_gemm_mixed_scratch_bytes((int)N, 4 * H, In))
-        SAT_TRY(sat_gemm_mixed_nt(X, In, 0, w_ih, In, 0, GA, 4L * H, b_ih, b_hh, (int)N, 4 * H, In, mixed, mixed_bytes, s));
-    else
+    if (mixed && mixed_bytes >= sat_gemm_mixed_scratch_bytes((int)N, 4 * H, In)) {
+        if (sat_gemm_operand_copies_on())
+            SAT_TRY(sat_gemm_mixed_nt(X, In, 0, w_ih, In, 0, GA, 4L * H, b_ih, b_hh, (int)N, 4 * H, In, mixed, mixed_bytes, s));
+        else
+            SAT_TRY(sat_gemm_operands_nt(X, In, SAT_GEMM_OP_F32, w_ih, In, SAT_GEMM_OP_F32, GA, 4L * H, b_ih, b_hh, (int)N, 4 * H, In, s));
+    } else
         SAT_TRY(sat_gemm_f32(0, 0, X, In, w_ih, In, GA, 4L * H, b_ih, b_hh, (int)N, 4 * H, In, stream));
     hipError_t e = hipMemsetAsync(HP, 0, (size_t)B * H * sizeof(float), s);
     if (e != hipSuccess) return (int)e;
@@ -356,11 +359,19 @@
                                   CS + off * H, cs_prev, dc_state, DG + off * 4 * H, n, H, s));
     }
     if (mixed && mixed_bytes >= sat_lstm_mixed_ws_bytes((int)N, In, H)) {
-        SAT_TRY(sat_gemm_mixed_nt(DG, 4L * H, 1, X, In, 1, dw_ih, In, nullptr, nullptr, 4 * H, In, (int)N, mixed, mixed_bytes, s));
-        SAT_TRY(sat_gemm_mixed_nt(DG, 4L * H, 1, HP, H, 1, dw_hh, H, nullptr, nullptr, 4 * H, H, (int)N, mixed, mixed_bytes, s));
+        const bool copies = sat_gemm_operand_copies_on() != 0;
+        const int KC = SAT_GEMM_OP_F32, KM = SAT_GEMM_OP_F32 | SAT_GEMM_OP_KMAJOR;
+        if (copies) {
+            SAT_TRY(sat_gemm_mixed_nt(DG, 4L * H, 1, X, In, 1, dw_ih, In, nullptr, nullptr, 4 * H, In, (int)N, mixed, mixed_bytes, s));
+            SAT_TRY(sat_gemm_mixed_nt(DG, 4L * H, 1, HP, H, 1, dw_hh, H, nullptr, nullptr, 4 * H, H, (int)N, mixed, mixed_bytes, s));
+        } else {
+            SAT_TRY(sat_gemm_operands_nt(DG, 4L * H, KM, X, In, KM, dw_ih, In, nullptr, nullptr, 4 * H, In, (int)N, s));
+            SAT_TRY(sat_gemm_operands_nt(DG, 4L * H, KM, HP, H, KM, dw_hh, H, nullptr, nullptr, 4 * H, H, (int)N, s));
+        }
         SAT_TRY(sat_colsum_f32(DG, 4L * H, (int)N, 4 * H, db_ih, stream));
         e = hipMemcpyAsync(db_hh, db_ih, (size_t)4 * H * sizeof(float), hipMemcpyDeviceToDevice, s);
         if (e != hipSuccess) return (int)e;
+        (void)KC;
         if (dX) SAT_TRY(sat_gemm_mixed_nt(DG, 4L * H, 0, w_ih, In, 1, dX, In, nullptr, nullptr, (int)N, In, 4 * H, mixed, mixed_bytes, s));
         return SAT_OK;
     }
diff --git a/show-and-tell_amd/csrc/sat_internal.h b/show-and-tell_amd/csrc/sat_internal.h
--- a/show-and-tell_amd/csrc/sat_internal.h
+++ b/show-and-tell_amd/csrc/sat_internal.h
@@ -20,6 +20,10 @@
 int64_t sat_gemm_mixed_scratch_bytes(int M, int N, int K);
 int sat_gemm_mixed_nt(const float* A, long lda, int a_kmajor, const float* B, long ldb, int b_kmajor, float* C, long ldc,
                       const float* bias, const float* bias2, int M, int N, int K, void* scratch, int64_t scratch_bytes, hipStream_t s);
+
+int sat_gemm_operands_nt(const void* A, long lda, int a_layout, const void* B, long ldb, int b_layout, float* C, long ldc,
+                         const float* bias, const float* bias2, int M, int N, int K, hipStream_t s);
+int sat_gemm_operand_copies_on();
 
 int sat_skinny_store(const float* A, long lda, const float* W, long ldw, int wkm, int M, int N, int K, int nz,
                      float* out, long ldo, long slab_stride, const float* bias, hipStream_t s);
```

Measured after the change: 19440. Within noise of the previous version (-0.3%).
